# lyndonchan/wsss-analysis

Hardware: AMD Instinct MI355X
Metric: images/sec CAM+CRF pseudo-labels, VOC2012 321x321 (higher is better)
Workload: dtype f16x3; 1 GPU; resnet50 CAM + dense-CRF (M=21, 10 mean-field iters), 321x321, batch 32 images (=64 samples) per GPU, image-sharded; batch_images=32, num_classes=20, parallelism=image-sharded x1, no collective, steps_per_rank=243

## Files before the change

### include/wsscam.h

```cpp
#ifndef WSSCAM_H
#define WSSCAM_H

#include <stddef.h>
#include <stdint.h>

#ifdef __cplusplus
extern "C" {
#endif

#define WSC_VERSION 100

typedef enum wsc_status {
    WSC_OK = 0,
    WSC_ERR_INVALID = -1,
    WSC_ERR_NO_DEVICE = -2,
    WSC_ERR_HIP = -3,
    WSC_ERR_MISSING_KEY = -4,
    WSC_ERR_SHAPE = -5,
    WSC_ERR_NOMEM = -6,
    WSC_ERR_KEY_RANGE = -7,
    WSC_ERR_CAPACITY = -8,
    WSC_ERR_RANGE = -9
} wsc_status;

typedef enum wsc_arch {
    WSC_ARCH_RESNET50_CAM = 0,
    WSC_ARCH_VGG16_CAM = 1,
    WSC_ARCH_M7_CAM = 2,
    WSC_ARCH_RESNET50_IRN = 3,
    WSC_ARCH_VGG16_IRN = 4,
    WSC_ARCH_M7_IRN = 5
} wsc_arch;

typedef enum wsc_precision {
    WSC_PREC_BF16 = 0,
    WSC_PREC_BF16X3 = 1,
    WSC_PREC_F16 = 2,
    WSC_PREC_F16X3 = 3,
    WSC_PREC_F32 = 4
} wsc_precision;

typedef struct wsc_ctx wsc_ctx;
typedef struct wsc_net wsc_net;
typedef enum {
    WSC_OPT_CRF_GAUSS_ON_CHIP = 0,
    WSC_OPT_CRF_FUSED_BLUR = 1,
    WSC_OPT_CRF_BLUR_ON_CHIP = 2,
    WSC_OPT_CRF_RANK_BALLOT = 3,
    WSC_OPT_CRF_EMBED_FULL = 4,
    WSC_OPT_RW_TILED = 5,
    WSC_OPT_STEM_POOL_FUSED = 6,
    WSC_OPT_CONV_WINDOW = 7,
    WSC_OPT_CAM_HEAD_STREAM = 8,
    WSC_OPT_CRF_MSG_IN_UPDATE = 9,
    WSC_OPT_COUNT = 10
} wsc_option;

typedef struct wsc_crf wsc_crf;
typedef struct wsc_crf_v wsc_crf_v;

typedef struct wsc_tensor_desc {
    const char *name;
    const float *data;
    int32_t ndim;
    int64_t shape[4];
} wsc_tensor_desc;


int wsc_version(void);
const char *wsc_last_error(void);

int wsc_ctx_create(int device, void *stream, wsc_ctx **out);
void wsc_ctx_destroy(wsc_ctx *ctx);
int wsc_ctx_set_option(wsc_ctx *ctx, int option, int value);
int wsc_sync(wsc_ctx *ctx);
int wsc_ctx_range_status(wsc_ctx *ctx, int *flag_out, int clear);
int wsc_ctx_wait(wsc_ctx *ctx, wsc_ctx *other);
int wsc_ctx_mark(wsc_ctx *ctx, int slot);
int wsc_ctx_wait_mark(wsc_ctx *ctx, int slot);
int wsc_ctx_wait_for_mark(wsc_ctx *ctx, wsc_ctx *other, int slot);
int wsc_device_info(wsc_ctx *ctx, char *arch_name, size_t arch_name_len, int *num_cus);

int wsc_malloc(wsc_ctx *ctx, size_t bytes, void **dptr_out);
int wsc_free(wsc_ctx *ctx, void *dptr);
int wsc_memcpy_h2d(wsc_ctx *ctx, void *dst_dev, const void *src_host, size_t bytes);
int wsc_memcpy_d2h(wsc_ctx *ctx, void *dst_host, const void *src_dev, size_t bytes);
int wsc_memset(wsc_ctx *ctx, void *dst_dev, int value, size_t bytes);
int wsc_host_alloc(wsc_ctx *ctx, size_t bytes, void **host_out);
int wsc_host_free(wsc_ctx *ctx, void *host);
int wsc_host_write_segments(const char *path, int n, const void *const *ptrs, const size_t *sizes);
int wsc_memcpy_h2d_async(wsc_ctx *ctx, void *dst_dev, const void *src_pinned_host, size_t bytes);
int wsc_memcpy_d2h_async(wsc_ctx *ctx, void *dst_pinned_host, const void *src_dev, size_t bytes);

int wsc_timer_begin(wsc_ctx *ctx);
int wsc_timer_end(wsc_ctx *ctx, float *ms_out);

int wsc_profile_begin(wsc_ctx *ctx);
int wsc_profile_end(wsc_ctx *ctx, int max_classes, int32_t *calls_out, float *total_ms_out, double *work_out,
                    int *n_classes_out);
const char *wsc_profile_class_name(int cls);


int wsc_net_create(wsc_ctx *ctx, int arch, const wsc_tensor_desc *weights, int n_weights,
                   int num_classes, int precision, wsc_net **out);
void wsc_net_destroy(wsc_net *net);
int wsc_net_cam_size(const wsc_net *net, int S, int *h_out);
int wsc_net_feat_channels(const wsc_net *net, int *f_out);

int wsc_net_forward_cam(wsc_ctx *ctx, const wsc_net *net, const float *x_dev, int B, int S,
                        float *cam_dev, float *score_dev);
int wsc_net_cam_size_hw(const wsc_net *net, int H, int W, int *h_out, int *w_out);
int wsc_net_forward_cam_hw(wsc_ctx *ctx, const wsc_net *net, const float *x_dev, int B, int H, int W, float *cam_dev,
                           float *score_dev);

int wsc_net_forward_features(wsc_ctx *ctx, const wsc_net *net, const float *x_dev ,
                             int N, int S, float *feat_dev);

int wsc_net_forward_edge(wsc_ctx *ctx, const wsc_net *net, const float *x_dev, int B, int S, int feat_h, int feat_w,
                         float *edge_dev, float *dp_dev);

int wsc_rw_propagate(wsc_ctx *ctx, const float *x_dev, const float *edge_dev, int K, int h, int w,
                     const int32_t *dirs_host, const int32_t *path_start_host, const int32_t *path_yx_host, int D,
                     float beta, int n_steps, float *rw_dev);
int wsc_rw_propagate_batch(wsc_ctx *ctx, int n_img, const int32_t *K_host, const int32_t *h_host,
                           const int32_t *w_host, const float *x_dev, const float *edge_dev,
                           const int32_t *dirs_host, const int32_t *path_start_host, const int32_t *path_yx_host,
                           int D, float beta, int n_steps, float *rw_dev);

int wsc_net_forward_gradcam(wsc_ctx *ctx, const wsc_net *net, const float *x_dev, int N, int S, int relu,
                            float *cams_dev, float *score_dev);

#define WSC_CONV_GENERIC 0x100
int wsc_conv2d_nchw(wsc_ctx *ctx, const float *x_dev, int N, int Cin, int H, int W, const float *w_host,
                    int Cout, int kh, int kw, int stride, int pad, const float *scale_host,
                    const float *shift_host, const float *residual_dev, int relu, int precision,
                    float *y_dev);


int wsc_cam_postprocess(wsc_ctx *ctx, const float *cam_dev, int B, int C, int h, int w,
                        const int32_t *size_hw_host , const int32_t *keys_host,
                        const int32_t *key_off_host , const int64_t *strided_off_host ,
                        const int64_t *highres_off_host , float *strided_dev, float *highres_dev);

int wsc_cam_eval_confusion(wsc_ctx *ctx, const float *highres_dev, int B, const int32_t *size_hw_host,
                           const int32_t *keys_host, const int32_t *key_off_host,
                           const int64_t *highres_off_host, float bg_thres, const uint8_t *gt_dev, int n_class,
                           int ignore_label, uint8_t *pred_dev, int64_t *confusion_dev);

int wsc_unary_from_maps(wsc_ctx *ctx, const float *maps_dev, int B, int C, int N, float bg_value,
                        float *unary_dev);

int wsc_cam_eval_confusion_nn(wsc_ctx *ctx, const float *maps_dev, int B, const int32_t *src_hw_host ,
                              const int32_t *out_hw_host , const int32_t *keys_host, const int32_t *key_off_host ,
                              const int64_t *maps_off_host , const uint8_t *gt_dev, int n_class, int ignore_label,
                              uint8_t *pred_dev, int64_t *confusion_dev);

int wsc_label_confusion_nn(wsc_ctx *ctx, const int32_t *labels_dev, int B, const int32_t *src_hw_host ,
                           const int32_t *out_hw_host , const int64_t *labels_off_host , const uint8_t *gt_dev,
                           int n_class, int ignore_label, uint8_t *pred_dev, int64_t *confusion_dev);

int wsc_sem_seg_finish(wsc_ctx *ctx, const float *rw_dev, int B, const int64_t *rw_off_host , const int32_t *khw_host ,
                       const int32_t *up_hw_host , const int32_t *out_hw_host , const int32_t *keys_host,
                       const int32_t *key_off_host , int has_bg, float bg_thres, uint8_t *label_dev);

int wsc_cam_unary(wsc_ctx *ctx, const float *cam_dev, int B, int C, int h, int w, int H0, int W0, float bg_value,
                  float *unary_dev);
int wsc_cam_unary_pm(wsc_ctx *ctx, const float *cam_dev, int B, int C, int h, int w, int H0, int W0, float bg_value,
                     float *unary_pm_dev);

int wsc_cam_sum_scales(wsc_ctx *ctx, const float *cam_dev, int n_images, int n_scales, long long map_elems, float *out_dev);

int wsc_msf_input_u8(wsc_ctx *ctx, const uint8_t *images_dev, int B, const int32_t *size_hw_host,
                     const int64_t *offset_host, int S, const float *mean3_host, const float *std3_host,
                     int pre_div255, int pair, float *x_dev);

int wsc_resize_u8(wsc_ctx *ctx, const uint8_t *images_dev, int B, const int32_t *size_hw_host, const int64_t *offset_host,
                  int OH, int OW, uint8_t *out_dev);

int wsc_bilinear_resize(wsc_ctx *ctx, const float *src_dev, int C, int h, int w, float *dst_dev, int H,
                        int W);


int wsc_label_unary_from_cam(wsc_ctx *ctx, const float *highres_dev, int B, int K, int N, float thres, float gt_prob,
                             float *unary_dev, int32_t *labels_dev);
int wsc_ir_label_combine(wsc_ctx *ctx, const int32_t *fg_pred_dev, const int32_t *bg_pred_dev, const int32_t *keys_host,
                         int B, int M, int N, uint8_t *conf_dev);


int wsc_hsn_gradcam_post(wsc_ctx *ctx, const float *cams_nhwc_dev, int B, int h, int w, int C, int S,
                         const float *gate_dev, float *out_dev, int out_channels, int out_first);
int wsc_hsn_voc_background(wsc_ctx *ctx, const float *Hbg_dev, int B, int Cb, int N, float *y_dev, int Ctot);
int wsc_hsn_class_mass(wsc_ctx *ctx, const float *maps_dev, int n_maps, int N, uint32_t *mass_dev);
int wsc_hsn_background(wsc_ctx *ctx, const uint8_t *rgb_dev, int B, int H, int W, int Ho, int Wo, double *bg_dev);
int wsc_cam_adp_modify(wsc_ctx *ctx, const float *cam_dev, int B, int n_sc, int C, int hw, const double *bg_dev, int mode,
                       const int32_t *use_host, int n_use, const int32_t *adipose_host, int n_adip, const int32_t *exc_host,
                       int n_exc, float *out_dev);
int wsc_hsn_cs_gradcam(wsc_ctx *ctx, const float *H_dev, int B, int C_all, int N, const double *bg_dev,
                       const int32_t *src_of_valid_host, int Cv, int bg_ind, int other_ind,
                       const int32_t *exception_inds_host, int n_exc, const int32_t *adipose_src_host, int n_adip,
                       float *cs_dev, float *y_dev, uint32_t *mass_dev);
int wsc_hsn_gather_unary(wsc_ctx *ctx, const float *maps_dev, const int64_t *chan_off_host, int n_chan, int N,
                         float *unary_dev);


int wsc_crf_create(wsc_ctx *ctx, const uint8_t *rgb_dev, int B, int H, int W, float g_sxy,
                   float bi_sxy, float bi_srgb, wsc_crf **out);
void wsc_crf_destroy(wsc_crf *crf);
int wsc_crf_lattice_sizes(wsc_ctx *ctx, const wsc_crf *crf, int32_t *v_gauss_host,
                          int32_t *v_bilat_host);
int wsc_crf_gaussian_on_chip(const wsc_crf *crf, int M);

int wsc_crf_inference(wsc_ctx *ctx, wsc_crf *crf, const float *unary_dev, int M, float g_compat,
                      float bi_compat, int n_iters, float *q_dev, int32_t *argmax_dev);
int wsc_crf_inference_pm(wsc_ctx *ctx, wsc_crf *crf, const float *unary_pm_dev, int M, float g_compat,
                         float bi_compat, int n_iters, float *q_dev, int32_t *argmax_dev);

int wsc_crf_v_create(wsc_ctx *ctx, const uint8_t *const *rgb_dev, const int32_t *hw_host , int B, float g_sxy,
                     float bi_sxy, float bi_srgb, wsc_crf_v **out);
void wsc_crf_v_destroy(wsc_crf_v *crf);
int wsc_crf_v_num_groups(const wsc_crf_v *crf);
int wsc_crf_v_inference(wsc_ctx *ctx, wsc_crf_v *crf, const float *const *unary_dev, const int32_t *M_host, float g_compat,
                        float bi_compat, int n_iters, float *const *q_dev, int32_t *const *argmax_dev);

#ifdef __cplusplus
}
#endif
#endif
```

### wsss-analysis_amd/csrc/common.h

```cpp
#pragma once
#include <hip/hip_runtime.h>
#include <stdint.h>
#include <map>
#include <string>
#include <unordered_map>
#include <vector>

#include "../../include/wsscam.h"

typedef uint16_t bf16_t;

typedef __bf16 bf16x8_t __attribute__((ext_vector_type(8)));
typedef _Float16 f16x8_t __attribute__((ext_vector_type(8)));
typedef float f32x16_t __attribute__((ext_vector_type(16)));
typedef float f32x4_t __attribute__((ext_vector_type(4)));

__host__ __device__ inline bf16_t f32_to_bf16(float f) {
    union { float f; uint32_t u; } v;
    v.f = f;
    uint32_t u = v.u;
    if ((u & 0x7fffffffu) > 0x7f800000u) return (bf16_t)((u >> 16) | 0x40);
    u += 0x7fffu + ((u >> 16) & 1u);
    return (bf16_t)(u >> 16);
}
__host__ __device__ inline float bf16_to_f32(bf16_t h) {
    union { float f; uint32_t u; } v;
    v.u = ((uint32_t)h) << 16;
    return v.f;
}

__host__ __device__ inline uint16_t f32_to_f16(float f) {
#if defined(__HIP_DEVICE_COMPILE__)
    const _Float16 h = (_Float16)fminf(fmaxf(f, -65504.f), 65504.f);
    return __builtin_bit_cast(uint16_t, h);
#else
    union { float f; uint32_t u; } v, magic;
    v.f = f;
    const uint32_t sign = v.u & 0x80000000u;
    v.u ^= sign;
    uint16_t o;
    if (v.u >= ((127u + 16u) << 23)) {
        o = v.u > (255u << 23) ? 0x7e00 : 0x7bff;
    } else if (v.u < (113u << 23)) {
        magic.u = ((127u - 15u) + (23u - 10u) + 1u) << 23;
        v.f += magic.f;
        o = (uint16_t)(v.u - magic.u);
    } else {
        const uint32_t mant_odd = (v.u >> 13) & 1u;
        v.u += ((15u - 127u) << 23) + 0xfffu;
        v.u += mant_odd;
        o = (uint16_t)(v.u >> 13);
        if (o >= 0x7c00) o = 0x7bff;
    }
    return (uint16_t)(o | (sign >> 16));
#endif
}
__host__ __device__ inline float f16_to_f32(uint16_t h) {
#if defined(__HIP_DEVICE_COMPILE__)
    return (float)__builtin_bit_cast(_Float16, h);
#else
    union { float f; uint32_t u; } o, magic;
    magic.u = 113u << 23;
    const uint32_t shifted_exp = 0x7c00u << 13;
    o.u = ((uint32_t)h & 0x7fffu) << 13;
    const uint32_t exp = shifted_exp & o.u;
    o.u += (127u - 15u) << 23;
    if (exp == shifted_exp) o.u += (128u - 16u) << 23;
    else if (exp == 0) { o.u += 1u << 23; o.f -= magic.f; }
    o.u |= ((uint32_t)h & 0x8000u) << 16;
    return o.f;
#endif
}
__host__ __device__ inline uint16_t f32_to_h16(float f, int fmt) { return fmt ? f32_to_f16(f) : f32_to_bf16(f); }
__host__ __device__ inline float h16_to_f32(uint16_t h, int fmt) { return fmt ? f16_to_f32(h) : bf16_to_f32(h); }

void wsc_set_error(const char *fmt, ...);
#define WSC_HIP(expr)                                                                          \
    do {                                                                                       \
        hipError_t _e = (expr);                                                                \
        if (_e != hipSuccess) {                                                                \
            wsc_set_error("%s:%d: %s failed: %s", __FILE__, __LINE__, #expr,                   \
                          hipGetErrorString(_e));                                              \
            return WSC_ERR_HIP;                                                                \
        }                                                                                      \
    } while (0)
#define WSC_CHECK(cond, code, ...)                                                             \
    do {                                                                                       \
        if (!(cond)) {                                                                         \
            wsc_set_error(__VA_ARGS__);                                                        \
            return (code);                                                                     \
        }                                                                                      \
    } while (0)
#define WSC_TRY(expr)                                                                          \
    do {                                                                                       \
        int _s = (expr);                                                                       \
        if (_s != WSC_OK) return _s;                                                           \
    } while (0)

enum WscKernelClass {
    WSC_K_CONV256 = 0,
    WSC_K_CONV128,
    WSC_K_CONV64,
    WSC_K_CONV_SMALLCIN,
    WSC_K_POOL_MISC,
    WSC_K_CAM_TAIL,
    WSC_K_CRF_BUILD,
    WSC_K_GAUSS_MSG,
    WSC_K_BLUR,
    WSC_K_SLICE_UPDATE,
    WSC_K_CRF_MISC,
    WSC_K_COUNT
};
struct WscProfRecord {
    int cls;
    double work;
    hipEvent_t e0, e1;
};

struct WscGaussCache;
void wsc_gauss_cache_destroy(WscGaussCache *cache);
struct wsc_ctx {
    int device = 0;
    hipStream_t stream = nullptr;
    bool own_stream = false;
    int num_cus = 0;
    std::string arch;
    void *ws = nullptr;
    size_t ws_bytes = 0;
    static constexpr int PIN_SLOTS = 8;
    struct PinSlot {
        void *p = nullptr;
        size_t bytes = 0;
        hipEvent_t ev = nullptr;
        bool busy = false;
    };
    PinSlot pin_ring[PIN_SLOTS];
    int pin_next = 0;
    int opt[WSC_OPT_COUNT] = {1, 1, 1, 0, 0, -1, 1, 1, 1, 1};
    void *zero_page = nullptr;
    unsigned *range_host = nullptr, *range_dev = nullptr;
    hipEvent_t ev0 = nullptr, ev1 = nullptr;
    hipEvent_t join_ev = nullptr;
    hipEvent_t marks[8] = {};
    bool mark_set[8] = {};
    hipStream_t aux_stream = nullptr;
    hipEvent_t fork_ev = nullptr, aux_done_ev = nullptr;
    bool profiling = false;
    std::vector<WscProfRecord> prof;
    std::vector<hipEvent_t> prof_pool;
    std::multimap<size_t, void *> free_blocks;
    std::unordered_map<void *, size_t> live_blocks;
    WscGaussCache *gauss_cache = nullptr;
};
int wsc_ctx_workspace(wsc_ctx *ctx, size_t bytes, void **out);
int wsc_ctx_range_check(wsc_ctx *ctx);
__device__ __forceinline__ unsigned half2_at_ceiling(unsigned hw) { return (hw & 0x7fff7fffu) + 0x04010401u; }
struct WscKernelTimer {
    wsc_ctx *ctx;
    int idx = -1;
    WscKernelTimer(wsc_ctx *c, int cls, double work);
    ~WscKernelTimer();
};
int wsc_ctx_cached_alloc(wsc_ctx *ctx, size_t bytes, void **out);
void wsc_ctx_cached_free(wsc_ctx *ctx, void *p);
struct WscCachedGuard {
    wsc_ctx *ctx;
    void *p;
    WscCachedGuard(wsc_ctx *c, void *q) : ctx(c), p(q) {}
    WscCachedGuard(const WscCachedGuard &) = delete;
    WscCachedGuard &operator=(const WscCachedGuard &) = delete;
    void free_now() {
        if (p) wsc_ctx_cached_free(ctx, p);
        p = nullptr;
    }
    ~WscCachedGuard() { free_now(); }
};
int wsc_ctx_upload_small(wsc_ctx *ctx, void *dst_dev, const void *src_host, size_t bytes);
int wsc_set_max_dynamic_lds(wsc_ctx *ctx, const void *fn, int bytes);

constexpr int CONV_FMT_F32 = 2;
inline int conv_fmt(wsc_precision prec) {
    if (prec == WSC_PREC_F32) return CONV_FMT_F32;
    return (prec == WSC_PREC_F16 || prec == WSC_PREC_F16X3) ? 1 : 0;
}
inline size_t conv_elem_bytes(wsc_precision prec) { return prec == WSC_PREC_F32 ? sizeof(float) : sizeof(bf16_t); }
inline int conv_split(wsc_precision prec) { return prec == WSC_PREC_BF16X3 ? 1 : (prec == WSC_PREC_F16X3 ? 2 : 0); }

enum ConvForm {
    CONV_FORM_GENERIC = 0,
    CONV_FORM_SMALL2,
    CONV_FORM_SMALL4,
    CONV_FORM_STEM_ROWS
};
inline bool conv_form_dma(ConvForm f) { return f == CONV_FORM_GENERIC || f == CONV_FORM_STEM_ROWS; }

struct ConvKLayout {
    ConvForm form;
    int kh, kw;
    int kw_steps;
    int kstep;
    int ck;
    bool interleaved;
    int cchunks;
    int ksteps_base;
    int Kbase;
    int Kw;
    int nk;
    int lo_at;
    int index(int ci, int r, int s) const {
        if (form == CONV_FORM_STEM_ROWS) return r * 64 + s * 4 + ci;
        if (form == CONV_FORM_GENERIC) return (((ci / ck) * kh + r) * kw + s) * kstep + ci % ck;
        return r * (form == CONV_FORM_SMALL2 ? 4 : 8) * 4 + s * 4 + ci;
    }
};
inline ConvKLayout conv_k_layout(int kh, int kw, int Cin, ConvForm form, wsc_precision prec) {
    ConvKLayout L;
    const int split = conv_split(prec);
    L.form = form; L.kh = kh; L.kw = kw;
    L.interleaved = split == 2 && conv_form_dma(form);
    L.kstep = prec == WSC_PREC_F32 ? 32 : 64;
    L.ck = (L.interleaved || prec == WSC_PREC_F32) ? 32 : 64;
    L.kw_steps = form == CONV_FORM_STEM_ROWS ? 1 : kw;
    L.cchunks = form == CONV_FORM_GENERIC ? Cin / L.ck : 1;
    if (form == CONV_FORM_GENERIC) L.ksteps_base = kh * kw * L.cchunks;
    else if (form == CONV_FORM_STEM_ROWS) L.ksteps_base = kh;
    else L.ksteps_base = (kh * (form == CONV_FORM_SMALL2 ? 4 : 8) * 4 + L.kstep - 1) / L.kstep;
    L.Kbase = L.ksteps_base * L.kstep;
    const bool segments = split != 0 && !L.interleaved;
    L.Kw = L.Kbase * (segments ? 2 : 1);
    L.nk = L.ksteps_base * (segments ? 3 : 1);
    L.lo_at = L.interleaved ? 32 : L.Kbase;
    return L;
}
inline int conv_cout_pad(int Cout) { return Cout <= 64 ? 64 : ((Cout + 127) / 128) * 128; }
inline int conv_tile_bn(int CoutPad) { return CoutPad % 128 == 0 ? 128 : 64; }
inline void conv_stem_rows_input_dims(int Ho, int Wo, int stride, int kh, int *Hp, int *Wp) {
    *Hp = (Ho - 1) * stride + kh;
    *Wp = (Wo - 1) * stride + 8;
}

struct ConvLaunch {
    const bf16_t *x, *x_lo;
    const bf16_t *w;
    const float *s1, *b1;
    const float *s2, *b2;
    const bf16_t *res, *res_lo;
    bf16_t *y, *y_lo;
    float *y_f32;
    int N, H, W, Cin, Ho, Wo, Cout, CoutPad;
    int kh, kw, stride, pad;
    int relu;
    ConvForm form;
    wsc_precision prec;
    int generic;
    int ldy;
    const bf16_t *x2, *x2_lo;
    int H2, W2, C2, stride2;
};
int conv_igemm_launch(wsc_ctx *ctx, const ConvLaunch &p);
int conv_f32_launch(wsc_ctx *ctx, const ConvLaunch &p);
int launch_cam_head(wsc_ctx *ctx, const bf16_t *x, const bf16_t *x_lo, int M, int K, const bf16_t *w, int Kw, int CoutPad,
                    const float *s1, const float *b1, int C, int relu, float *y);

int launch_nchw_to_nhwc4(wsc_ctx *ctx, const float *x, int N, int H, int W, bf16_t *y, bf16_t *y_lo, int fmt);
void stem_pool_input_dims(int H, int W, int *Hp, int *Wp);
int launch_stem_pool(wsc_ctx *ctx, const bf16_t *x, const bf16_t *x_lo, int N, int H, int W, const bf16_t *w, int Kw, const float *s1,
                     const float *b1, int relu, bf16_t *y, bf16_t *y_lo);
int launch_gather_strided(wsc_ctx *ctx, const bf16_t *x, const bf16_t *x_lo, int N, int H, int W, int C, int stride, int Ho, int Wo,
                          bf16_t *y, bf16_t *y_lo, int ldy);
int launch_nchw_to_nhwc4_pad(wsc_ctx *ctx, const float *x, int N, int H, int W, int Hp, int Wp, int pad, bf16_t *y, bf16_t *y_lo,
                             int fmt);
int launch_maxpool(wsc_ctx *ctx, const bf16_t *x, const bf16_t *x_lo, int N, int H, int W, int C, int k,
                   int stride, int pad, int Ho, int Wo, bf16_t *y, bf16_t *y_lo, int fmt);
int launch_flip_add(wsc_ctx *ctx, const float *head, int B, int h, int w, int C, int Cs, float *cam);
int launch_gap_linear_sigmoid(wsc_ctx *ctx, const bf16_t *feat, const bf16_t *feat_lo, int B, int hw, int F,
                              const float *Wc, const float *bias, int C, float *score, int fmt,
                              int sample_stride);
int launch_bf16_to_f32(wsc_ctx *ctx, const bf16_t *x, const bf16_t *x_lo, size_t n, float *y, int fmt);
int launch_nchw_to_nhwc(wsc_ctx *ctx, const float *x, int N, int C, int HW, bf16_t *y, bf16_t *y_lo, int fmt);
int launch_nhwc_to_nchw(wsc_ctx *ctx, const bf16_t *x, const bf16_t *x_lo, int N, int C, int HW, float *y, int fmt);

int launch_group_norm_stats(wsc_ctx *ctx, const float *x, int N, int H, int W, int C, int G, float eps, void *partial,
                            void *stats);
size_t group_norm_partial_bytes(int N, int H, int W, int G);
int launch_group_norm_apply(wsc_ctx *ctx, const float *x, const void *stats, const float *gamma, const float *beta,
                            int N, int H, int W, int C, int G, int up, int relu, bf16_t *y, bf16_t *y_lo, int Hd, int Wd,
                            int Ctot, int coff, int fmt);
int launch_edge_finish(wsc_ctx *ctx, const float *e, int He, int We, const float *d, int Hd, int Wd, int B, int fh, int fw,
                       float ms0, float ms1, float *edge, float *dp);
```

### wsss-analysis_amd/csrc/crf.hip

```cpp
#include "common.h"

#include <atomic>
#include <cmath>
#include <cstring>
#include <memory>

namespace {

constexpr unsigned long long EMPTY_KEY = 0xFFFFFFFFFFFFFFFFull;
typedef float f32x2_t __attribute__((ext_vector_type(2)));

struct LatticeDev {
    int d = 0;
    int rep = 1;
    int rows = 0;
    int32_t *offset = nullptr;
    float *bary = nullptr;
    float *norm = nullptr;
    int2 *nbr = nullptr;
    int32_t *tslot_start = nullptr;
    int2 *slot_desc = nullptr;
    float *tent_w = nullptr;
    uint8_t *tent_p = nullptr;
    int32_t *row_slot_start = nullptr;
    int n_tiles = 0, n_slots = 0;
    bool sorted_dest = false;
    long long n_pix = 0;
    int M_cur = 0;
    float alpha = 0.f;
    int32_t *tile_rows = nullptr;
    int2 *tile_pstart = nullptr;
    int32_t *tile_list = nullptr;
    int n_tiles_occ = 0;
    int4 *gt_cnt = nullptr;
    int2 *gt_rows = nullptr;
    uint4 *gt_nbr = nullptr;
    uint4 *gt_pix = nullptr;
    int gt_stride = 0;
    std::vector<int32_t> v_per_image;
    int32_t *img_row = nullptr;
    int max_img_rows = 0;
    uint32_t *part_row = nullptr;
    bool bl_ok = false;
    int2 *bl_blk = nullptr;
    int bl_cap = 0;
    mutable std::vector<int2> bl_blk_host;
    mutable int bl_M = -1, bl_nblk = 0;
    mutable size_t bl_lds = 0;
};

constexpr int TILE_W = 16, TILE_H = 16, TILE_PIX = TILE_W * TILE_H;
static_assert(TILE_PIX <= 256, "an entry's pixel index is stored in one byte");
constexpr int SLOT_ENT = 32;
constexpr int SORT_MAX = 2048;
static_assert(TILE_PIX * 6 <= SORT_MAX && SORT_MAX <= 65535, "tile too large for the in-LDS grouping");

struct TileGeom {
    int H, W, ntx, nty, tpi;
};
__host__ __device__ inline TileGeom make_geom(int H, int W) {
    TileGeom g;
    g.H = H; g.W = W;
    g.ntx = (W + TILE_W - 1) / TILE_W;
    g.nty = (H + TILE_H - 1) / TILE_H;
    g.tpi = g.ntx * g.nty;
    return g;
}
struct TileBox {
    int x0, y0, cw, ch;
    int ebase;
};
__host__ __device__ inline TileBox tile_box(const TileGeom &g, int j) {
    const unsigned ty = (unsigned)j / (unsigned)g.ntx, tx = (unsigned)j - ty * (unsigned)g.ntx;
    TileBox b;
    b.x0 = (int)(tx * (unsigned)g.W / (unsigned)g.ntx);
    b.y0 = (int)(ty * (unsigned)g.H / (unsigned)g.nty);
    b.cw = (int)((tx + 1) * (unsigned)g.W / (unsigned)g.ntx) - b.x0;
    b.ch = (int)((ty + 1) * (unsigned)g.H / (unsigned)g.nty) - b.y0;
    b.ebase = b.y0 * g.W + b.x0 * b.ch;
    return b;
}
static_assert(TILE_W <= 26 && TILE_PIX <= 4096, "tile_div_magic range");
__host__ __device__ inline unsigned tile_div_magic(int cw) { return (65536u + (unsigned)cw - 1u) / (unsigned)cw; }

struct CtxBlocks {
    wsc_ctx *ctx;
    std::vector<void *> ptrs;
    explicit CtxBlocks(wsc_ctx *c) : ctx(c) {}
    CtxBlocks(CtxBlocks &&o) noexcept : ctx(o.ctx), ptrs(std::move(o.ptrs)) { o.ptrs.clear(); }
    ~CtxBlocks() { release(); }
    template <class T>
    int alloc(size_t bytes, T **out) {
        void *p = nullptr;
        WSC_TRY(wsc_ctx_cached_alloc(ctx, bytes, &p));
        ptrs.push_back(p);
        *out = static_cast<T *>(p);
        return WSC_OK;
    }
    void take(CtxBlocks &&o) {
        ptrs.insert(ptrs.end(), o.ptrs.begin(), o.ptrs.end());
        o.ptrs.clear();
    }
    void release() {
        for (void *p : ptrs) wsc_ctx_cached_free(ctx, p);
        ptrs.clear();
    }
};

struct GaussEntry {
    int H, W;
    float sxy;
    LatticeDev L;
    CtxBlocks blocks;
    int users = 0;
    unsigned long long last_use = 0;
    bool fuse_pending = true;
};
constexpr int GAUSS_CACHE_MAX = 64;
std::atomic<unsigned long long> g_gauss_use_clock{0};

}

struct wsc_crf {
    wsc_ctx *ctx = nullptr;
    int B = 0, H = 0, W = 0, N = 0;
    LatticeDev lat[2];
    uint4 *pix_rec = nullptr;
    uint32_t *pix_rec_b = nullptr;
    CtxBlocks blocks;
    GaussEntry *gauss = nullptr;
    hipEvent_t use_ev = nullptr;
    bool used_elsewhere = false;
    explicit wsc_crf(wsc_ctx *c) : ctx(c), blocks(c) {}
};

struct WscGaussCache {
    std::vector<std::unique_ptr<GaussEntry>> entries;
};
void wsc_gauss_cache_destroy(WscGaussCache *cache) { delete cache; }

namespace {

__device__ __forceinline__ unsigned long long mix64(unsigned long long x) {
    x ^= x >> 30; x *= 0xbf58476d1ce4e5b9ull;
    x ^= x >> 27; x *= 0x94d049bb133111ebull;
    x ^= x >> 31;
    return x;
}

template <int D>
__device__ __forceinline__ bool pack_key(const int *key, unsigned long long &out) {
    if (D == 2) {
        out = ((unsigned long long)(unsigned)(key[0] + 0x40000000) << 32) | (unsigned)(key[1] + 0x40000000);
        return true;
    }
    unsigned long long k = 0;
    bool ok = true;
#pragma unroll
    for (int i = 0; i < D; ++i) {
        const int v = key[i] + 2048;
        ok = ok && v >= 0 && v < 4096;
        k = (k << 12) | (unsigned long long)(v & 4095);
    }
    out = k;
    return ok;
}
template <int D>
__device__ __forceinline__ void unpack_key(unsigned long long k, int *key) {
    if (D == 2) {
        key[0] = (int)(unsigned)(k >> 32) - 0x40000000;
        key[1] = (int)(unsigned)(k & 0xffffffffu) - 0x40000000;
        return;
    }
#pragma unroll
    for (int i = D - 1; i >= 0; --i) {
        key[i] = (int)(k & 4095) - 2048;
        k >>= 12;
    }
}

constexpr int HASH_MAX_PROBE = 256;
__device__ __forceinline__ int hash_insert(unsigned long long *table, unsigned mask, unsigned long long key) {
    unsigned slot = (unsigned)mix64(key) & mask;
    for (int probe = 0; probe < HASH_MAX_PROBE; ++probe) {
        const unsigned long long prev = atomicCAS(&table[slot], EMPTY_KEY, key);
        if (prev == EMPTY_KEY || prev == key) return (int)slot;
        slot = (slot + 1) & mask;
    }
    return -1;
}
__device__ __forceinline__ int hash_lookup(const unsigned long long *table, unsigned mask, unsigned long long key) {
    unsigned slot = (unsigned)mix64(key) & mask;
    for (;;) {
        const unsigned long long cur = table[slot];
        if (cur == key) return (int)slot;
        if (cur == EMPTY_KEY) return -1;
        slot = (slot + 1) & mask;
    }
}

__device__ __forceinline__ void xcd_range(long long total, long long &begin, long long &end) {
    const int nb = gridDim.x, bid = blockIdx.x;
    const int xcd = bid & 7, q = nb >> 3, r = nb & 7;
    const long long lb = (xcd < r ? (long long)xcd * (q + 1) : (long long)r * (q + 1) + (long long)(xcd - r) * q) + (bid >> 3);
    const long long per = (total + nb - 1) / nb;
    begin = lb * per;
    end = begin + per < total ? begin + per : total;
}

__device__ __forceinline__ int xcd_block_id() {
    const int nb = gridDim.x, bid = blockIdx.x;
    const int xcd = bid & 7, q = nb >> 3, r = nb & 7;
    return (xcd < r ? xcd * (q + 1) : r * (q + 1) + (xcd - r) * q) + (bid >> 3);
}

__device__ __forceinline__ void xcd_range_rep(long long n_local, int rep, int &k, long long &begin, long long &end) {
    const int nb = gridDim.x, bid = blockIdx.x;
    const int xcd = bid & 7, q = nb >> 3, r = nb & 7;
    const int lb = (xcd < r ? xcd * (q + 1) : r * (q + 1) + (xcd - r) * q) + (bid >> 3);
    const int bpr = nb / rep;
    k = lb / bpr;
    const int j = lb - k * bpr;
    const long long per = (n_local + bpr - 1) / bpr;
    begin = (long long)j * per;
    end = begin + per < n_local ? begin + per : n_local;
}

struct EmbedArgs {
    const uint8_t *rgb;
    int B, H, W, N;
    float inv_sxy_den, inv_srgb_den;
    float scale[5];
    unsigned long long *table;
    unsigned cap_mask;
    long long cap;
    float *bary;
    int32_t *first;
    int *err;
};

template <int D>
__device__ __forceinline__ bool embed_pixel(const EmbedArgs &a, long long gp, int x, int y, unsigned long long *pk_out,
                                            float *bary_out) {

    float f[D];
    f[0] = (float)x / a.inv_sxy_den;
    f[1] = (float)y / a.inv_sxy_den;
    if (D == 5) {
        const uint8_t *px = a.rgb + gp * 3;
        f[2] = (float)(int)px[0] / a.inv_srgb_den;
        f[3] = (float)(int)px[1] / a.inv_srgb_den;
        f[4] = (float)(int)px[2] / a.inv_srgb_den;
    }
    float elevated[D + 1], rem0[D + 1];
    int rank[D + 1];
    float sm = 0.f;
#pragma unroll
    for (int j = D; j > 0; --j) {
        const float cf = f[j - 1] * a.scale[j - 1];
        elevated[j] = sm - (float)j * cf;
        sm += cf;
    }
    elevated[0] = sm;

    const float down_factor = 1.0f / (float)(D + 1);
    const float up_factor = (float)(D + 1);
    int sum = 0;
#pragma unroll
    for (int i = 0; i <= D; ++i) {
        const float v = down_factor * elevated[i];
        const float up = ceilf(v) * up_factor;
        const float down = floorf(v) * up_factor;
        int rd2;
        if (up - elevated[i] < elevated[i] - down) rd2 = (int)(short)up;
        else rd2 = (int)(short)down;
        rem0[i] = (float)rd2;
        sum = (int)((float)sum + (float)rd2 * down_factor);
    }
#pragma unroll
    for (int i = 0; i <= D; ++i) rank[i] = 0;
#pragma unroll
    for (int i = 0; i < D; ++i) {
        const float di = elevated[i] - rem0[i];
#pragma unroll
        for (int j = i + 1; j <= D; ++j) {
            if (di < elevated[j] - rem0[j]) rank[i]++;
            else rank[j]++;
        }
    }
#pragma unroll
    for (int i = 0; i <= D; ++i) {
        rank[i] += sum;
        if (rank[i] < 0) {
            rank[i] += D + 1;
            rem0[i] += (float)(D + 1);
        } else if (rank[i] > D) {
            rank[i] -= D + 1;
            rem0[i] -= (float)(D + 1);
        }
    }
    float bary[D + 2];
#pragma unroll
    for (int i = 0; i <= D + 1; ++i) bary[i] = 0.f;
#pragma unroll
    for (int i = 0; i <= D; ++i) {
        const float v = (elevated[i] - rem0[i]) * down_factor;
#pragma unroll
        for (int s = 0; s <= D + 1; ++s) {
            if (s == D - rank[i]) bary[s] += v;
            if (s == D - rank[i] + 1) bary[s] -= v;
        }
    }
    bary[0] = (float)((double)bary[0] + (1.0 + (double)bary[D + 1]));

    bool ok = true;
#pragma unroll
    for (int r = 0; r <= D; ++r) {
        int key[D];
#pragma unroll
        for (int i = 0; i < D; ++i) {
            const int can = rank[i] <= D - r ? r : r - (D + 1);
            key[i] = (int)(short)(rem0[i] + (float)can);
        }
        ok = pack_key<D>(key, pk_out[r]) && ok;
        bary_out[r] = bary[r];
    }
    return ok;
}

__global__ void first_bits_kernel(const int32_t *__restrict__ first, long long cap, int per_img, unsigned *__restrict__ bitmap) {
    const int b = blockIdx.y;
    const int32_t *fi = first + (long long)b * cap;
    for (long long sl = (long long)blockIdx.x * blockDim.x + threadIdx.x; sl < cap; sl += (long long)gridDim.x * blockDim.x) {
        const int f = fi[sl];
        if (f != 0x7fffffff) {
            const long long g = (long long)b * per_img + f;
            atomicOr(&bitmap[g >> 5], 1u << (unsigned)(g & 31));
        }
    }
}
__global__ void popc_words_kernel(const unsigned *__restrict__ bitmap, long long nw, unsigned *__restrict__ cnt) {
    for (long long w = (long long)blockIdx.x * blockDim.x + threadIdx.x; w < nw; w += (long long)gridDim.x * blockDim.x)
        cnt[w] = (unsigned)__popc(bitmap[w]);
}
__device__ __forceinline__ unsigned first_rank(const unsigned *bitmap, const unsigned *wprefix, long long g) {
    return wprefix[g >> 5] + (unsigned)__popc(bitmap[g >> 5] & ((1u << (unsigned)(g & 31)) - 1u));
}
__global__ void image_bounds_kernel(const unsigned *__restrict__ bitmap, const unsigned *__restrict__ wprefix, int per_img, int B,
                                    unsigned *__restrict__ bound) {
    const int b = blockIdx.x * blockDim.x + threadIdx.x;
    if (b < B) bound[b] = first_rank(bitmap, wprefix, (long long)b * per_img);
}
__global__ void image_rows_kernel(const unsigned *__restrict__ bound, int B, int rows, int32_t *__restrict__ img_row) {
    const int b = blockIdx.x * blockDim.x + threadIdx.x;
    if (b < B) img_row[b] = 1 + (int)bound[b];
    if (b == B) img_row[b] = rows;
}
__global__ void assign_rows_kernel(const int32_t *__restrict__ first, const unsigned long long *__restrict__ table, long long cap,
                                   int per_img, const unsigned *__restrict__ bitmap, const unsigned *__restrict__ wprefix,
                                   int32_t *__restrict__ slot2row, unsigned long long *__restrict__ rowkey,
                                   int32_t *__restrict__ rowimg) {
    const int b = blockIdx.y;
    for (long long sl = (long long)blockIdx.x * blockDim.x + threadIdx.x; sl < cap; sl += (long long)gridDim.x * blockDim.x) {
        const long long s_ = (long long)b * cap + sl;
        const int f = first[s_];
        if (f == 0x7fffffff) continue;
        const int row = 1 + (int)first_rank(bitmap, wprefix, (long long)b * per_img + f);
        slot2row[s_] = row;
        rowkey[row] = table[s_];
        rowimg[row] = b;
    }
}

constexpr int SCAN_CHUNK = 4096;

__device__ __forceinline__ unsigned block_exclusive_scan_256(unsigned v, unsigned *lds, unsigned &total) {
    const int lane = threadIdx.x & 63, wv = threadIdx.x >> 6;
    unsigned x = v;
    for (int o = 1; o < 64; o <<= 1) {
        const unsigned y = __shfl_up(x, o, 64);
        if (lane >= o) x += y;
    }
    if (lane == 63) lds[wv] = x;
    __syncthreads();
    unsigned base = 0;
    for (int i = 0; i < wv; ++i) base += lds[i];
    total = lds[0] + lds[1] + lds[2] + lds[3];
    __syncthreads();
    return base + x - v;
}

__global__ __launch_bounds__(256) void scan_reduce_kernel(const unsigned *__restrict__ in, long long n,
                                                          unsigned *__restrict__ sums) {
    __shared__ unsigned lds[4];
    const long long base = (long long)blockIdx.x * SCAN_CHUNK;
    unsigned s = 0;
    for (int i = 0; i < 16; ++i) {
        const long long idx = base + i * 256 + threadIdx.x;
        if (idx < n) s += in[idx];
    }
    for (int o = 32; o > 0; o >>= 1) s += __shfl_down(s, o, 64);
    if ((threadIdx.x & 63) == 0) lds[threadIdx.x >> 6] = s;
    __syncthreads();
    if (threadIdx.x == 0) sums[blockIdx.x] = lds[0] + lds[1] + lds[2] + lds[3];
}

__global__ __launch_bounds__(256) void scan_sums_kernel(unsigned *__restrict__ sums, int m) {
    __shared__ unsigned lds[4];
    unsigned carry = 0;
    for (int base = 0; base < m; base += 256) {
        const int idx = base + threadIdx.x;
        const unsigned v = idx < m ? sums[idx] : 0u;
        unsigned total;
        const unsigned ex = block_exclusive_scan_256(v, lds, total);
        if (idx < m) sums[idx] = carry + ex;
        carry += total;
    }
    if (threadIdx.x == 0) sums[m] = carry;
}

__global__ __launch_bounds__(256) void scan_apply_kernel(const unsigned *__restrict__ in, long long n,
                                                         const unsigned *__restrict__ sums, unsigned *__restrict__ out) {
    __shared__ unsigned lds[4];
    const long long base = (long long)blockIdx.x * SCAN_CHUNK;
    unsigned carry = sums[blockIdx.x];
    unsigned v[16];
    unsigned s = 0;
    const long long t0 = base + (long long)threadIdx.x * 16;
#pragma unroll
    for (int i = 0; i < 16; ++i) {
        v[i] = (t0 + i < n) ? in[t0 + i] : 0u;
        s += v[i];
    }
    unsigned total;
    unsigned ex = carry + block_exclusive_scan_256(s, lds, total);
#pragma unroll
    for (int i = 0; i < 16; ++i) {
        if (t0 + i < n) out[t0 + i] = ex;
        ex += v[i];
    }
}

__global__ __launch_bounds__(256) void scan_apply_fused_kernel(const unsigned *__restrict__ in, long long n,
                                                               unsigned *__restrict__ sums, int nblk, unsigned *__restrict__ out) {
    __shared__ unsigned lds[4];
    __shared__ unsigned red[8];
    const long long base = (long long)blockIdx.x * SCAN_CHUNK;
    const unsigned mine = (int)threadIdx.x < nblk ? sums[threadIdx.x] : 0u;
    unsigned c = (int)threadIdx.x < (int)blockIdx.x ? mine : 0u, tot = mine;
    for (int o = 32; o > 0; o >>= 1) {
        c += __shfl_down(c, o, 64);
        tot += __shfl_down(tot, o, 64);
    }
    if ((threadIdx.x & 63) == 0) {
        red[threadIdx.x >> 6] = c;
        red[4 + (threadIdx.x >> 6)] = tot;
    }
    __syncthreads();
    const unsigned carry = red[0] + red[1] + red[2] + red[3];
    if (blockIdx.x == 0 && threadIdx.x == 0) sums[nblk] = red[4] + red[5] + red[6] + red[7];
    unsigned v[16];
    unsigned s = 0;
    const long long t0 = base + (long long)threadIdx.x * 16;
#pragma unroll
    for (int i = 0; i < 16; ++i) {
        v[i] = (t0 + i < n) ? in[t0 + i] : 0u;
        s += v[i];
    }
    unsigned total;
    unsigned ex = carry + block_exclusive_scan_256(s, lds, total);
#pragma unroll
    for (int i = 0; i < 16; ++i) {
        if (t0 + i < n) out[t0 + i] = ex;
        ex += v[i];
    }
}

int exclusive_scan(wsc_ctx *ctx, const unsigned *in, long long n, unsigned *out, unsigned *sums ) {
    const int nblk = (int)((n + SCAN_CHUNK - 1) / SCAN_CHUNK);
    hipLaunchKernelGGL(scan_reduce_kernel, dim3(nblk), dim3(256), 0, ctx->stream, in, n, sums);
    if (nblk <= 256) {
        hipLaunchKernelGGL(scan_apply_fused_kernel, dim3(nblk), dim3(256), 0, ctx->stream, in, n, sums, nblk, out);
        WSC_HIP(hipGetLastError());
        return WSC_OK;
    }
    hipLaunchKernelGGL(scan_sums_kernel, dim3(1), dim3(256), 0, ctx->stream, sums, nblk);
    hipLaunchKernelGGL(scan_apply_kernel, dim3(nblk), dim3(256), 0, ctx->stream, in, n, sums, out);
    WSC_HIP(hipGetLastError());
    return WSC_OK;
}

template <bool MAXOP, class T = int>
__device__ __forceinline__ void block_scan_lds(T *v, int n, int *wtot ) {
    constexpr int PER = SORT_MAX / 256;
    const int t0 = threadIdx.x * PER;
    int loc[PER];
    int run = 0;
#pragma unroll
    for (int i = 0; i < PER; ++i) {
        const int x = t0 + i < n ? (int)v[t0 + i] : 0;
        run = MAXOP ? max(run, x) : run + x;
        loc[i] = run;
    }
    const int lane = threadIdx.x & 63, wv = threadIdx.x >> 6;
    int x = run;
    for (int o = 1; o < 64; o <<= 1) {
        const int y = __shfl_up(x, o, 64);
        if (lane >= o) x = MAXOP ? max(x, y) : x + y;
    }
    if (lane == 63) wtot[wv] = x;
    __syncthreads();
    int base = 0;
    for (int i = 0; i < wv; ++i) base = MAXOP ? max(base, wtot[i]) : base + wtot[i];
    int prev = __shfl_up(x, 1, 64);
    if (lane == 0) prev = 0;
    const int carry = MAXOP ? max(base, prev) : base + prev;
#pragma unroll
    for (int i = 0; i < PER; ++i)
        if (t0 + i < n) v[t0 + i] = (T)(MAXOP ? max(carry, loc[i]) : carry + loc[i]);
    __syncthreads();
}

__device__ __forceinline__ void tile_slot_flags(const int *srow, int ne, unsigned short *aux, unsigned short *flag, unsigned short *seg,
                                                int *wtot) {
    for (int i = threadIdx.x; i < ne; i += 256) seg[i] = (unsigned short)((i == 0 || srow[i] != srow[i - 1]) ? i : 0);
    __syncthreads();
    block_scan_lds<true>(seg, ne, wtot);
    for (int i = threadIdx.x; i < ne; i += 256) {
        flag[i] = ((i - (int)seg[i]) % SLOT_ENT == 0) ? 1 : 0;
        aux[i] = flag[i];
    }
    __syncthreads();
    block_scan_lds<false>(aux, ne, wtot);
}

constexpr int GROUP_HT_SMALL = 512, GROUP_HT_FULL = SORT_MAX;
constexpr int RANK_MW = (TILE_PIX + 31) / 32;
template <int D, int GROUP_HT>
__device__ __forceinline__ void tile_embed_body(const EmbedArgs &a, const TileGeom &tg, float *__restrict__ tent_w,
                                                uint8_t *__restrict__ tent_p, int32_t *__restrict__ sslot_out,
                                                unsigned *__restrict__ tile_nslots, int force_ballot, int tile,
                                                int32_t *__restrict__ redo_list, unsigned *__restrict__ redo_count) {
    constexpr int RANK_GMAX = (4 * GROUP_HT * 2 + SORT_MAX * 2) / (RANK_MW * 4);
    constexpr bool SMALL = GROUP_HT < GROUP_HT_FULL;
    constexpr int dp1 = D + 1;
    __shared__ unsigned long long table[GROUP_HT];
    __shared__ int start[GROUP_HT];
    __shared__ __attribute__((aligned(16))) unsigned short rank_store[4 * GROUP_HT + SORT_MAX];
    unsigned short(*wcnt)[GROUP_HT] = reinterpret_cast<unsigned short(*)[GROUP_HT]>(rank_store);
    unsigned short *erank = rank_store + 4 * GROUP_HT;
    unsigned *gmask = reinterpret_cast<unsigned *>(rank_store);
    __shared__ unsigned short eslot[SORT_MAX];
    __shared__ unsigned short cid[GROUP_HT];
    __shared__ int wtot[4];
    __shared__ int n_groups_s;
    __shared__ int full_s;
    const int b = tile / tg.tpi, j = tile - b * tg.tpi;
    const TileBox tb = tile_box(tg, j);
    const int N = tg.H * tg.W;
    const int np = tb.cw * tb.ch, ne = np * dp1;
    for (int i = threadIdx.x; i < GROUP_HT; i += 256) {
        table[i] = EMPTY_KEY;
        start[i] = 0x7fffffff;
    }
    for (int i = threadIdx.x; i < (4 * GROUP_HT + SORT_MAX) / 2; i += 256) gmask[i] = 0u;
    if (threadIdx.x == 0) full_s = 0;
    __syncthreads();
    const int t = threadIdx.x;
    const bool have = t < np;
    const int ty = have ? t / tb.cw : 0, tx = have ? t - ty * tb.cw : 0;
    const int y = tb.y0 + ty, x = tb.x0 + tx;
    const int n = y * tg.W + x;
    const long long gp = (long long)b * N + n;
    unsigned long long pk[dp1];
    float bary[dp1];
    if (have) {
        if (!embed_pixel<D>(a, gp, x, y, pk, bary)) atomicOr(a.err, 1);
#pragma unroll
        for (int r = 0; r < dp1; ++r) {
            unsigned sl = (unsigned)(mix64(pk[r]) >> 40) & (GROUP_HT - 1);
            for (int probes = 0;; ++probes) {
                const unsigned long long old = atomicCAS(&table[sl], EMPTY_KEY, pk[r]);
                if (old == EMPTY_KEY || old == pk[r]) break;
                if (SMALL && probes >= GROUP_HT) {
                    full_s = 1;
                    break;
                }
                sl = (sl + 1) & (GROUP_HT - 1);
            }
            eslot[t * dp1 + r] = (unsigned short)sl;
            atomicMin(&start[sl], n * dp1 + r);
        }
    }
    __syncthreads();
    const int lane = threadIdx.x & 63, q = threadIdx.x >> 6;
    {
        constexpr int PER = GROUP_HT / 256;
        int cnt = 0;
#pragma unroll
        for (int k = 0; k < PER; ++k) cnt += table[threadIdx.x * PER + k] != EMPTY_KEY ? 1 : 0;
        int x = cnt;
        for (int o = 1; o < 64; o <<= 1) {
            const int y = __shfl_up(x, o, 64);
            if (lane >= o) x += y;
        }
        if (lane == 63) wtot[q] = x;
        __syncthreads();
        int base = x - cnt;
        for (int i = 0; i < q; ++i) base += wtot[i];
#pragma unroll
        for (int k = 0; k < PER; ++k) {
            const int sl = threadIdx.x * PER + k;
            const bool occ = table[sl] != EMPTY_KEY;
            cid[sl] = (unsigned short)base;
            base += occ ? 1 : 0;
        }
        if (threadIdx.x == 255) n_groups_s = base;
        __syncthreads();
    }
    if (SMALL && (full_s || n_groups_s > GROUP_HT * 3 / 4)) {
        if (threadIdx.x == 0) redo_list[atomicAdd(redo_count, 1u)] = tile;
        return;
    }
    const bool use_mask = !force_ballot && n_groups_s <= RANK_GMAX;
    const int Q = ((ne + 3) / 4 + 63) / 64 * 64;
    if (use_mask) {
        if (have) {
#pragma unroll
            for (int r = 0; r < dp1; ++r)
                atomicOr(&gmask[(unsigned)cid[eslot[t * dp1 + r]] * RANK_MW + (t >> 5)], 1u << (t & 31));
        }
    } else {
        for (int c = q * Q; c < min(ne, (q + 1) * Q); c += 64) {
            const int e = c + lane;
            const bool valid = e < ne;
            const unsigned sl = valid ? eslot[e] : 0u;
            unsigned long long remaining = __ballot(valid);
            unsigned long long mine = 0;
            while (remaining) {
                const int leader = __ffsll((long long)remaining) - 1;
                const bool same = valid && sl == (unsigned)__shfl((int)sl, leader, 64);
                const unsigned long long m = __ballot(same);
                if (same) mine = m;
                remaining &= ~m;
            }
            if (valid) {
                const int leader = __ffsll((long long)mine) - 1;
                int base = 0;
                if (lane == leader) {
                    base = wcnt[q][sl];
                    wcnt[q][sl] = (unsigned short)(base + __popcll(mine));
                }
                base = __shfl(base, leader, 64);
                erank[e] = (unsigned short)(base + __popcll(mine & ((1ull << lane) - 1ull)));
            }
        }
    }
    __syncthreads();
    unsigned long long *gtable = a.table + (long long)b * a.cap;
    int32_t *gfirst = a.first + (long long)b * a.cap;
    int my_slots = 0;
    for (int i = threadIdx.x; i < GROUP_HT; i += 256) {
        int tot = 0, c0 = 0, c1 = 0, c2 = 0;
        if (use_mask) {
            if (table[i] != EMPTY_KEY) {
#pragma unroll
                for (int w = 0; w < RANK_MW; ++w) tot += __popc(gmask[(unsigned)cid[i] * RANK_MW + w]);
            }
        } else {
            c0 = wcnt[0][i]; c1 = wcnt[1][i]; c2 = wcnt[2][i];
            tot = c0 + c1 + c2 + wcnt[3][i];
        }
        if (tot > 0) {
            int gs = hash_insert(gtable, a.cap_mask, table[i]);
            if (gs >= 0) atomicMin(&gfirst[gs], start[i]);
            else {
                atomicOr(a.err, 2);
                gs = 0;
            }
            table[i] = (unsigned long long)(unsigned)gs;
        }
        start[i] = tot;
        if (!use_mask) {
            wcnt[0][i] = 0;
            wcnt[1][i] = (unsigned short)c0;
            wcnt[2][i] = (unsigned short)(c0 + c1);
            wcnt[3][i] = (unsigned short)(c0 + c1 + c2);
        }
        my_slots += (tot + SLOT_ENT - 1) / SLOT_ENT;
    }
    for (int o = 32; o > 0; o >>= 1) my_slots += __shfl_down(my_slots, o, 64);
    __syncthreads();
    if (lane == 0) wtot[q] = my_slots;
    __syncthreads();
    if (threadIdx.x == 0) tile_nslots[tile] = (unsigned)(wtot[0] + wtot[1] + wtot[2] + wtot[3]);
    __syncthreads();
    block_scan_lds<false>(start, GROUP_HT, wtot);
    if (have) {
        const long long ebase = ((long long)b * N + tb.ebase) * dp1;
#pragma unroll
        for (int r = 0; r < dp1; ++r) {
            const int e = t * dp1 + r;
            const int sl = eslot[e];
            const int prev = sl > 0 ? start[sl - 1] : 0;
            int rank;
            if (use_mask) {
                const unsigned *m = gmask + (unsigned)cid[sl] * RANK_MW;
                rank = __popc(m[t >> 5] & ((1u << (t & 31)) - 1u));
                for (int w = 0; w < (t >> 5); ++w) rank += __popc(m[w]);
            } else {
                rank = (int)wcnt[e / Q][sl] + (int)erank[e];
            }
            const int pos = prev + rank;
            const int gs = (int)(unsigned)table[sl];
            tent_w[ebase + pos] = bary[r];
            tent_p[ebase + pos] = (uint8_t)t;
            sslot_out[ebase + pos] = gs | (r << 28);
            a.bary[gp * dp1 + r] = bary[r];
        }
    }
}
template <int D>
__global__ __launch_bounds__(256) void tile_embed_kernel(EmbedArgs a, TileGeom tg, float *__restrict__ tent_w, uint8_t *__restrict__ tent_p,
                                                         int32_t *__restrict__ sslot_out, unsigned *__restrict__ tile_nslots,
                                                         int force_ballot, int32_t *__restrict__ redo_list,
                                                         unsigned *__restrict__ redo_count) {
    tile_embed_body<D, GROUP_HT_SMALL>(a, tg, tent_w, tent_p, sslot_out, tile_nslots, force_ballot, (int)blockIdx.x, redo_list,
                                       redo_count);
}
template <int D>
__global__ __launch_bounds__(256) void tile_embed_full_kernel(EmbedArgs a, TileGeom tg, float *__restrict__ tent_w,
                                                              uint8_t *__restrict__ tent_p, int32_t *__restrict__ sslot_out,
                                                              unsigned *__restrict__ tile_nslots, int force_ballot,
                                                              const int32_t *__restrict__ redo_list,
                                                              const unsigned *__restrict__ redo_count, int n_tiles) {
    const int count = redo_list ? (int)*redo_count : n_tiles;
    for (int i = blockIdx.x; i < count; i += gridDim.x) {
        tile_embed_body<D, GROUP_HT_FULL>(a, tg, tent_w, tent_p, sslot_out, tile_nslots, force_ballot,
                                          redo_list ? redo_list[i] : i, nullptr, nullptr);
        __syncthreads();
    }
}

__global__ __launch_bounds__(256) void tile_slots_kernel(const int32_t *__restrict__ sslot_in, const uint8_t *__restrict__ tent_p,
                                                         int32_t *__restrict__ offset, const int32_t *__restrict__ slot2row,
                                                         long long cap, int dp1, TileGeom tg,
                                                         const int32_t *__restrict__ tslot_start, int2 *__restrict__ slot_desc,
                                                         int32_t *__restrict__ slot_row, unsigned *__restrict__ slot_key,
                                                         unsigned *__restrict__ row_nslots) {
    __shared__ int rows_s[SORT_MAX];
    __shared__ unsigned short aux[SORT_MAX];
    __shared__ unsigned short flag[SORT_MAX];
    __shared__ unsigned short seg[SORT_MAX];
    __shared__ unsigned short pos[SORT_MAX + 2];
    __shared__ int wtot[4];
    const int tile = xcd_block_id();
    const int b = tile / tg.tpi, j = tile - b * tg.tpi;
    const TileBox tb = tile_box(tg, j);
    const int N = tg.H * tg.W;
    const int ne = tb.cw * tb.ch * dp1;
    const long long ebase = ((long long)b * N + tb.ebase) * dp1;
    const unsigned cw_magic = tile_div_magic(tb.cw);
    for (int i = threadIdx.x; i < ne; i += 256) {
        const int ss = sslot_in[ebase + i];
        const int row = slot2row[(long long)b * cap + (ss & 0x0fffffff)];
        rows_s[i] = row;
        const unsigned t = tent_p[ebase + i];
        const unsigned ty = (t * cw_magic) >> 16, tx = t - ty * (unsigned)tb.cw;
        const long long p = (long long)b * N + (long long)(tb.y0 + (int)ty) * tg.W + tb.x0 + (int)tx;
        offset[p * dp1 + (ss >> 28)] = row;
    }
    __syncthreads();
    tile_slot_flags(rows_s, ne, aux, flag, seg, wtot);
    const int ns = aux[ne - 1];
    for (int i = threadIdx.x; i < ne; i += 256)
        if (flag[i]) pos[aux[i] - 1] = (unsigned short)i;
    if (threadIdx.x == 0) pos[ns] = (unsigned short)ne;
    __syncthreads();
    __shared__ int hist[SLOT_ENT + 1], hcur[SLOT_ENT + 1];
    if (threadIdx.x <= SLOT_ENT) { hist[threadIdx.x] = 0; hcur[threadIdx.x] = 0; }
    __syncthreads();
    for (int s = threadIdx.x; s < ns; s += 256) atomicAdd(&hist[pos[s + 1] - pos[s]], 1);
    __syncthreads();
    if (threadIdx.x == 0) {
        int run = 0;
        for (int n = SLOT_ENT; n >= 0; --n) {
            const int c = hist[n];
            hist[n] = run;
            run += c;
        }
    }
    __syncthreads();
    const int s0 = tslot_start[tile];
    for (int s = threadIdx.x; s < ns; s += 256) {
        const int i = pos[s], n = pos[s + 1] - i;
        const int row = rows_s[i];
        const int dst = s0 + hist[n] + atomicAdd(&hcur[n], 1);
        slot_desc[dst] = make_int2(i | (n << 16), 0);
        slot_row[dst] = row;
        if (slot_key) slot_key[dst] = (unsigned)tile * 64u + (unsigned)((i - seg[i]) / SLOT_ENT);
        atomicAdd(&row_nslots[row], 1u);
    }
}

__global__ void slot_dest_kernel(const int32_t *__restrict__ slot_row, int n_slots, const int32_t *__restrict__ row_slot_start,
                                 unsigned *__restrict__ cursor, int2 *__restrict__ slot_desc, uint32_t *__restrict__ part_row) {
    for (int s = blockIdx.x * blockDim.x + threadIdx.x; s < n_slots; s += gridDim.x * blockDim.x) {
        const int row = slot_row[s];
        const int sb = row_slot_start[row];
        const int dst = sb + (int)atomicAdd(&cursor[row], 1u);
        slot_desc[s].y = dst;
        if (part_row) part_row[dst] = (uint32_t)row | ((uint32_t)min(row_slot_start[row + 1] - sb, 255) << 24);
    }
}

__global__ void dest_inverse_kernel(const int2 *__restrict__ slot_desc, int n_slots, int32_t *__restrict__ dest_slot) {
    for (int s = blockIdx.x * blockDim.x + threadIdx.x; s < n_slots; s += gridDim.x * blockDim.x) dest_slot[slot_desc[s].y] = s;
}
__global__ void row_sort_dest_kernel(const unsigned *__restrict__ slot_key, int32_t *__restrict__ dest_slot,
                                     const int32_t *__restrict__ row_slot_start, int rows, int2 *__restrict__ slot_desc) {
    for (int row = blockIdx.x * blockDim.x + threadIdx.x; row < rows; row += gridDim.x * blockDim.x) {
        const int sb = row_slot_start[row], se = row_slot_start[row + 1];
        for (int i = sb + 1; i < se; ++i) {
            const int s = dest_slot[i];
            const unsigned key = slot_key[s];
            int j = i - 1;
            while (j >= sb && slot_key[dest_slot[j]] > key) {
                dest_slot[j + 1] = dest_slot[j];
                --j;
            }
            dest_slot[j + 1] = s;
        }
        for (int i = sb; i < se; ++i) slot_desc[dest_slot[i]].y = i;
    }
}

__global__ __launch_bounds__(256) void tile_scale_entries_kernel(const float *__restrict__ norm, int dp1, TileGeom tg,
                                                                 float *__restrict__ tent_w, const uint8_t *__restrict__ tent_p) {
    const int tile = blockIdx.x;
    const int b = tile / tg.tpi, j = tile - b * tg.tpi;
    const TileBox tb = tile_box(tg, j);
    const int N = tg.H * tg.W;
    const int ne = tb.cw * tb.ch * dp1;
    const long long ebase = ((long long)b * N + tb.ebase) * dp1;
    const unsigned cw_magic = tile_div_magic(tb.cw);
    for (int i = threadIdx.x; i < ne; i += 256) {
        const int t = (int)tent_p[ebase + i];
        const int ty = (int)(((unsigned)t * cw_magic) >> 16), tx = t - ty * tb.cw;
        const long long p = (long long)b * N + (long long)(tb.y0 + ty) * tg.W + tb.x0 + tx;
        tent_w[ebase + i] = tent_w[ebase + i] * norm[p];
    }
}

template <int D>
__global__ void neighbors_kernel(const unsigned long long *__restrict__ rowkey, const int32_t *__restrict__ rowimg,
                                 const unsigned long long *__restrict__ table, const int32_t *__restrict__ slot2row,
                                 long long cap, unsigned cap_mask, int rows, int2 *__restrict__ nbr) {
    const int j = blockIdx.y;
    long long rbeg, rend;
    xcd_range(rows, rbeg, rend);
    for (int row = (int)rbeg + (int)threadIdx.x; row < (int)rend; row += (int)blockDim.x) {
        const long long i = (long long)j * rows + row;
        int *nb = reinterpret_cast<int *>(nbr);
        if (row == 0) {
            nb[2 * i] = 0;
            continue;
        }
        int key[D], k1[D];
        unpack_key<D>(rowkey[row], key);
#pragma unroll
        for (int k = 0; k < D; ++k) k1[k] = key[k] - 1;
        if (j < D) {
#pragma unroll
            for (int k = 0; k < D; ++k)
                if (k == j) k1[k] = key[k] + D;
        }
        const int b = rowimg[row];
        const unsigned long long *tb = table + (long long)b * cap;
        const int32_t *s2r = slot2row + (long long)b * cap;
        unsigned long long p1;
        int r1 = 0;
        if (pack_key<D>(k1, p1)) {
            const int s = hash_lookup(tb, cap_mask, p1);
            if (s >= 0) r1 = s2r[s];
        }
        nb[2 * i] = r1;
        if (r1 > 0) nb[2 * ((long long)j * rows + r1) + 1] = row;
    }
}


constexpr float PFIX_SCALE = 16777216.0f;
constexpr float PFIX_INV = 1.0f / 16777216.0f;
static_assert(SLOT_ENT * 2.5f < 127.0f, "slot partials must fit the 2^24 fixed-point int32");

template <bool PLAIN>
__device__ __forceinline__ f32x4_t combine_slots4(const f32x4_t *__restrict__ part, int sb, int se, unsigned LP, unsigned l) {
    f32x4_t first = part[(unsigned)sb * LP + l];
    if (se - sb == 1) return first;
    if (PLAIN) {
        for (int i = sb + 1; i < se; ++i) {
            const f32x4_t v = part[(unsigned)i * LP + l];
#pragma unroll
            for (int k = 0; k < 4; ++k) first[k] += v[k];
        }
        return first;
    }
    long long acc[4] = {0, 0, 0, 0};
    for (int i = sb; i < se; i += 4) {
        f32x4_t v[4];
#pragma unroll
        for (int u = 0; u < 4; ++u) v[u] = part[(unsigned)min(i + u, se - 1) * LP + l];
#pragma unroll
        for (int u = 0; u < 4; ++u)
            if (i + u < se) {
#pragma unroll
                for (int k = 0; k < 4; ++k) acc[k] += (long long)__float2int_rn(v[u][k] * PFIX_SCALE);
            }
    }
    f32x4_t o = {(float)acc[0] * PFIX_INV, (float)acc[1] * PFIX_INV, (float)acc[2] * PFIX_INV, (float)acc[3] * PFIX_INV};
    return o;
}

__global__ __launch_bounds__(256) void slot_ones_kernel(const int32_t *__restrict__ tslot_start, const int2 *__restrict__ slot_desc,
                                                        const float *__restrict__ tent_w, int dp1, TileGeom tg,
                                                        float *__restrict__ part) {
    const int tile = blockIdx.x;
    const int b = tile / tg.tpi, j = tile - b * tg.tpi;
    const TileBox tb = tile_box(tg, j);
    const long long ebase = ((long long)b * tg.H * tg.W + tb.ebase) * dp1;
    __shared__ float w[TILE_PIX * 6];
    const int ne = tb.cw * tb.ch * dp1;
    {
        constexpr int EN = (TILE_PIX * 6 + 255) / 256;
        float ew[EN];
#pragma unroll
        for (int k = 0; k < EN; ++k) {
            const int i = (int)threadIdx.x + k * 256;
            ew[k] = i < ne ? tent_w[ebase + i] : 0.f;
        }
#pragma unroll
        for (int k = 0; k < EN; ++k) {
            const int i = (int)threadIdx.x + k * 256;
            if (i < ne) w[i] = ew[k];
        }
    }
    __syncthreads();
    for (int s = tslot_start[tile] + threadIdx.x; s < tslot_start[tile + 1]; s += 256) {
        const int2 d = slot_desc[s];
        const int i0 = d.x & 0xffff, n = d.x >> 16;
        float acc = 0.f;
        for (int i = 0; i < n; ++i) acc += w[i0 + i];
        part[d.y] = acc;
    }
}
__global__ void combine1_kernel(const float *__restrict__ part, const int32_t *__restrict__ row_slot_start, int rows,
                                float *__restrict__ val) {
    for (int row = blockIdx.x * blockDim.x + threadIdx.x; row < rows; row += gridDim.x * blockDim.x) {
        long long acc = 0;
        for (int i = row_slot_start[row]; i < row_slot_start[row + 1]; ++i)
            acc += (long long)__float2int_rn(part[i] * PFIX_SCALE);
        val[row] = (float)acc * PFIX_INV;
    }
}

__global__ __launch_bounds__(256) void combine4_kernel(const f32x4_t *__restrict__ part, const int32_t *__restrict__ row_slot_start,
                                                       int LP, int rows_local, int n_slots, int rep, f32x4_t *__restrict__ val) {
    const int rpb = 256 / LP;
    const int tr = threadIdx.x / LP;
    const int l = threadIdx.x - tr * LP;
    if (tr >= rpb) return;
    long long rbeg, rend;
    int rk;
    xcd_range_rep(rows_local, rep, rk, rbeg, rend);
    part += (size_t)rk * n_slots * LP;
    val += (size_t)rk * rows_local * LP;
    for (long long row = rbeg + tr; row < rend; row += rpb) {
        const int sb = row_slot_start[row], se = row_slot_start[row + 1];
        f32x4_t o = {0.f, 0.f, 0.f, 0.f};
        if (se > sb) o = combine_slots4<true>(part, sb, se, (unsigned)LP, (unsigned)l);
        val[(unsigned)row * (unsigned)LP + l] = o;
    }
}

constexpr int CB_ROWS = 32;
__global__ __launch_bounds__(256) void combine4_balanced_kernel(const f32x4_t *__restrict__ part, const int32_t *__restrict__ row_slot_start,
                                                                const uint32_t *__restrict__ part_row, int LP, int rows,
                                                                f32x4_t *__restrict__ val) {
    __shared__ int rss_l[CB_ROWS + 1];
    __shared__ unsigned long long acc[CB_ROWS * 32];
    const int r0 = blockIdx.x * CB_ROWS;
    const int nr = min(CB_ROWS, rows - r0);
    const int P0 = row_slot_start[r0], P1 = row_slot_start[r0 + nr];
    for (int i = threadIdx.x; i <= nr; i += 256) rss_l[i] = row_slot_start[r0 + i];
    for (int i = threadIdx.x; i < CB_ROWS * 32; i += 256) acc[i] = 0ull;
    const int gpb = 256 / LP;
    const int tr = threadIdx.x / LP, l = threadIdx.x - tr * LP;
    constexpr int U = 4;
    f32x4_t v[U];
    uint32_t pr[U];
    auto fetch = [&](int p) {
#pragma unroll
        for (int u = 0; u < U; ++u) {
            const int pp = p + u * gpb;
            v[u] = f32x4_t{0.f, 0.f, 0.f, 0.f};
            pr[u] = 0u;
            if (tr < gpb && pp < P1) {
                v[u] = part[(unsigned)pp * (unsigned)LP + l];
                if (part_row) pr[u] = part_row[pp];
            }
        }
    };
    fetch(P0 + tr);
    __syncthreads();
    if (tr < gpb) {
        for (int p = P0 + tr; p < P1; p += U * gpb) {
            if (p != P0 + tr) fetch(p);
#pragma unroll
            for (int u = 0; u < U; ++u) {
                const int pp = p + u * gpb;
                if (pp < P1) {
                    int lo;
                    bool single;
                    if (part_row) {
                        lo = (int)(pr[u] & 0xffffffu) - r0;
                        single = (pr[u] >> 24) == 1u;
                    } else {
                        lo = 0;
                        int hi = nr;
                        while (hi - lo > 1) {
                            const int mid = (lo + hi) >> 1;
                            if (rss_l[mid] <= pp) lo = mid;
                            else hi = mid;
                        }
                        single = rss_l[lo + 1] - rss_l[lo] == 1;
                    }
                    if (single) {
                        val[(unsigned)(r0 + lo) * (unsigned)LP + l] = v[u];
                    } else {
#pragma unroll
                        for (int k = 0; k < 4; ++k)
                            atomicAdd(&acc[lo * 32 + 4 * l + k], (unsigned long long)(long long)__float2int_rn(v[u][k] * PFIX_SCALE));
                    }
                }
            }
        }
    }
    __syncthreads();
    if (tr < gpb) {
        for (int row = tr; row < nr; row += gpb) {
            const int n = rss_l[row + 1] - rss_l[row];
            if (n == 1) continue;
            f32x4_t o = {0.f, 0.f, 0.f, 0.f};
            if (n > 1) {
#pragma unroll
                for (int k = 0; k < 4; ++k) o[k] = (float)(long long)acc[row * 32 + 4 * l + k] * PFIX_INV;
            }
            val[(unsigned)(r0 + row) * (unsigned)LP + l] = o;
        }
    }
}


__global__ __launch_bounds__(256) void blur1_kernel(const float *__restrict__ in, const int2 *__restrict__ nbr,
                                                    int rows, float *__restrict__ out) {
    for (int row = blockIdx.x * blockDim.x + threadIdx.x; row < rows; row += gridDim.x * blockDim.x) {
        const int2 nb = nbr[row];
        out[row] = row == 0 ? 0.f : in[row] + 0.5f * (in[nb.x] + in[nb.y]);
    }
}

__global__ __launch_bounds__(256) void blur4_kernel(const f32x4_t *__restrict__ in, const int2 *__restrict__ nbr,
                                                    int LP, int rows_local, int rep, f32x4_t *__restrict__ out) {
    const int rpb = 256 / LP;
    const int tr = threadIdx.x / LP;
    const int l = threadIdx.x - tr * LP;
    if (tr >= rpb) return;
    constexpr int U = 4;
    long long rbeg, rend;
    int rk;
    xcd_range_rep(rows_local, rep, rk, rbeg, rend);
    in += (size_t)rk * rows_local * LP;
    out += (size_t)rk * rows_local * LP;
    for (long long row0 = rbeg + tr; row0 < rend; row0 += U * rpb) {
        int2 nb[U];
        f32x4_t c[U], a[U], b[U];
#pragma unroll
        for (int u = 0; u < U; ++u) {
            const long long row = row0 + u * rpb;
            nb[u] = row < rend ? nbr[row] : make_int2(0, 0);
        }
#pragma unroll
        for (int u = 0; u < U; ++u) {
            const long long row = row0 + u * rpb;
            c[u] = in[(unsigned)(row < rend ? row : 0) * (unsigned)LP + l];
            a[u] = in[(unsigned)nb[u].x * (unsigned)LP + l];
            b[u] = in[(unsigned)nb[u].y * (unsigned)LP + l];
        }
#pragma unroll
        for (int u = 0; u < U; ++u) {
            const long long row = row0 + u * rpb;
            if (row < rend) {
                f32x4_t o;
#pragma unroll
                for (int k = 0; k < 4; ++k) o[k] = row == 0 ? 0.f : c[u][k] + 0.5f * (a[u][k] + b[u][k]);
                out[(unsigned)row * (unsigned)LP + l] = o;
            }
        }
    }
}

constexpr int BL_THREADS = 1024;
constexpr int BL_NVAR = 5;
constexpr int BL_VAR[BL_NVAR][2] = {{4, 4}, {4, 10}, {3, 13}, {2, 20}, {1, 26}};
inline int blur_lds_variant(int rows) {
    for (int v = 0; v < BL_NVAR; ++v)
        if (rows <= BL_VAR[v][1] * BL_THREADS && (size_t)(rows + 1) * BL_VAR[v][0] * 4 <= 160 * 1024 && rows < 65535) return v;
    return -1;
}
struct BlurLdsArgs {
    const int2 *nbr;
    const int32_t *img_row;
    const int2 *blk;
    float *val;
    int Mp, M, rows, npass;
};
template <int GW> struct FloatRun { float v[GW]; };
typedef float f32x3u_t __attribute__((ext_vector_type(3), aligned(4)));
template <int GW>
__device__ __forceinline__ FloatRun<GW> load_run(const float *q) {
    FloatRun<GW> r;
    if constexpr (GW == 4) {
        const f32x4_t x = *reinterpret_cast<const f32x4_t *>(q);
        r.v[0] = x[0]; r.v[1] = x[1]; r.v[2] = x[2]; r.v[3] = x[3];
    } else if constexpr (GW == 3) {
        const f32x3u_t x = *reinterpret_cast<const f32x3u_t *>(q);
        r.v[0] = x[0]; r.v[1] = x[1]; r.v[2] = x[2];
    } else if constexpr (GW == 2) {
        const f32x2_t x = *reinterpret_cast<const f32x2_t *>(q);
        r.v[0] = x[0]; r.v[1] = x[1];
    } else {
        r.v[0] = q[0];
    }
    return r;
}
template <int GW>
__device__ __forceinline__ void store_run(float *q, const FloatRun<GW> &r) {
    if constexpr (GW == 4) *reinterpret_cast<f32x4_t *>(q) = f32x4_t{r.v[0], r.v[1], r.v[2], r.v[3]};
    else if constexpr (GW == 3) {
        f32x3u_t x;
        x[0] = r.v[0]; x[1] = r.v[1]; x[2] = r.v[2];
        *reinterpret_cast<f32x3u_t *>(q) = x;
    } else if constexpr (GW == 2) *reinterpret_cast<f32x2_t *>(q) = f32x2_t{r.v[0], r.v[1]};
    else q[0] = r.v[0];
}
template <int GW, int RPT>
__device__ __forceinline__ void blur_lds_body(const BlurLdsArgs &p, float *pl, int img, int grp) {
    const int r0 = p.img_row[img], nr = p.img_row[img + 1] - r0;
    const int stride = nr + 1;
    const int c0 = grp * GW;
    const int tid = (int)threadIdx.x;
    float *vb = p.val + (size_t)r0 * p.Mp + c0;
    unsigned nb[RPT];
    auto load_idx = [&](int pass) {
        const int2 *q = p.nbr + (size_t)pass * p.rows + r0;
        constexpr int CH = RPT < 10 ? RPT : 10;
#pragma unroll
        for (int i0 = 0; i0 < RPT; i0 += CH) {
            int2 raw[CH];
#pragma unroll
            for (int i = 0; i < CH; ++i) {
                const int r = tid + (i0 + i) * BL_THREADS;
                raw[i] = (i0 + i < RPT && r < nr) ? q[r] : make_int2(0, 0);
            }
#pragma unroll
            for (int i = 0; i < CH; ++i)
                if (i0 + i < RPT)
                    nb[i0 + i] = (unsigned)(raw[i].x ? raw[i].x - r0 : nr) | ((unsigned)(raw[i].y ? raw[i].y - r0 : nr) << 16);
        }
    };
    load_idx(0);
#pragma unroll
    for (int i = 0; i < RPT; ++i) {
        const int r = tid + i * BL_THREADS;
        if (r < nr) {
            FloatRun<GW> run;
            if (GW == 3 && c0 + GW > p.Mp) {
#pragma unroll
                for (int g = 0; g < GW; ++g) run.v[g] = c0 + g < p.Mp ? vb[(size_t)r * p.Mp + g] : 0.f;
            } else {
                run = load_run<GW>(vb + (size_t)r * p.Mp);
            }
#pragma unroll
            for (int g = 0; g < GW; ++g) pl[g * stride + r] = c0 + g < p.M ? run.v[g] : 0.f;
        }
    }
    if (tid < GW) pl[tid * stride + nr] = 0.f;
    __syncthreads();
    float o[RPT][GW];
    for (int pass = 0; pass < p.npass; ++pass) {
#pragma unroll
        for (int i = 0; i < RPT; ++i) {
            const int r = tid + i * BL_THREADS;
            const int rc = r < nr ? r : nr;
            const int l1 = (int)(nb[i] & 0xffffu), l2 = (int)(nb[i] >> 16);
#pragma unroll
            for (int g = 0; g < GW; ++g) o[i][g] = pl[g * stride + rc] + 0.5f * (pl[g * stride + l1] + pl[g * stride + l2]);
        }
        if (pass + 1 < p.npass) load_idx(pass + 1);
        else break;
        __syncthreads();
#pragma unroll
        for (int i = 0; i < RPT; ++i) {
            const int r = tid + i * BL_THREADS;
            if (r < nr) {
#pragma unroll
                for (int g = 0; g < GW; ++g) pl[g * stride + r] = o[i][g];
            }
        }
        __syncthreads();
    }
#pragma unroll
    for (int i = 0; i < RPT; ++i) {
        const int r = tid + i * BL_THREADS;
        if (r < nr) {
            if (c0 + GW <= p.M) {
                FloatRun<GW> run;
#pragma unroll
                for (int g = 0; g < GW; ++g) run.v[g] = o[i][g];
                store_run<GW>(vb + (size_t)r * p.Mp, run);
            } else {
#pragma unroll
                for (int g = 0; g < GW; ++g)
                    if (c0 + g < p.M) vb[(size_t)r * p.Mp + g] = o[i][g];
            }
        }
    }
}
__global__ __launch_bounds__(BL_THREADS) void blur_lds_kernel(BlurLdsArgs p) {
    extern __shared__ float pl[];
    const int2 w = p.blk[blockIdx.x];
    if (w.x < 0) return;
    const int img = w.x & 0xffffff;
    switch (w.x >> 24) {
    case 0: blur_lds_body<BL_VAR[0][0], BL_VAR[0][1]>(p, pl, img, w.y); break;
    case 1: blur_lds_body<BL_VAR[1][0], BL_VAR[1][1]>(p, pl, img, w.y); break;
    case 2: blur_lds_body<BL_VAR[2][0], BL_VAR[2][1]>(p, pl, img, w.y); break;
    case 3: blur_lds_body<BL_VAR[3][0], BL_VAR[3][1]>(p, pl, img, w.y); break;
    default: blur_lds_body<BL_VAR[4][0], BL_VAR[4][1]>(p, pl, img, w.y); break;
    }
}

constexpr int GTI = 12, GTJ = 12, GBI = GTI + 4, GBJ = GTJ + 4;
constexpr int GLH = 6;

__global__ void gauss_ij_kernel(const unsigned long long *__restrict__ rowkey, int rows, int2 *__restrict__ ij,
                                int *__restrict__ bbox ) {
    for (int row = 1 + blockIdx.x * blockDim.x + threadIdx.x; row < rows; row += gridDim.x * blockDim.x) {
        int key[2];
        unpack_key<2>(rowkey[row], key);
        const int a = 2 * key[0] + key[1], b = key[0] + 2 * key[1];
        if (a % 3 != 0 || b % 3 != 0) atomicOr(&bbox[4], 1);
        const int i = a / 3, j = b / 3;
        ij[row] = make_int2(i, j);
        atomicMin(&bbox[0], i);
        atomicMin(&bbox[1], j);
        atomicMax(&bbox[2], i);
        atomicMax(&bbox[3], j);
    }
}

__global__ void gauss_tile_fill_kernel(const int2 *__restrict__ ij, int rows, int imin, int jmin, int nti, int ntj,
                                       int32_t *__restrict__ tile_rows, int32_t *__restrict__ occ) {
    for (int row = 1 + blockIdx.x * blockDim.x + threadIdx.x; row < rows; row += gridDim.x * blockDim.x) {
        const int i = ij[row].x - imin, j = ij[row].y - jmin;
        occ[(i / GTI) * ntj + j / GTJ] = 1;
        for (int ti = (i - GTI - 1 >= 0 ? (i - GTI - 1) / GTI : 0); ti <= (i + 2) / GTI && ti < nti; ++ti) {
            const int li = i - ti * GTI + 2;
            if (li < 0 || li >= GBI) continue;
            for (int tj = (j - GTJ - 1 >= 0 ? (j - GTJ - 1) / GTJ : 0); tj <= (j + 2) / GTJ && tj < ntj; ++tj) {
                const int lj = j - tj * GTJ + 2;
                if (lj < 0 || lj >= GBJ) continue;
                tile_rows[((long long)ti * ntj + tj) * (GBI * GBJ) + li * GBJ + lj] = row;
            }
        }
    }
}

__global__ void gauss_tile_pstart_kernel(const int32_t *__restrict__ tile_rows, const int32_t *__restrict__ row_slot_start,
                                         long long total, int2 *__restrict__ tile_pstart) {
    for (long long i = (long long)blockIdx.x * blockDim.x + threadIdx.x; i < total; i += (long long)gridDim.x * blockDim.x) {
        const int row = tile_rows[i];
        tile_pstart[i] = row ? make_int2(row_slot_start[row], row_slot_start[row + 1] - row_slot_start[row]) : make_int2(0, 0);
    }
}

__global__ __launch_bounds__(GBI * GBJ) void blur3_tile_kernel(const f32x4_t *__restrict__ in, const int32_t *__restrict__ tile_rows,
                                                         const int32_t *__restrict__ tile_list, int n_occ, int LP,
                                                         int rows_local, int rep, f32x4_t *__restrict__ out,
                                                         const f32x4_t *__restrict__ part, const int2 *__restrict__ tile_pstart,
                                                         int n_slots) {
    constexpr int P = GBI * GBJ;
    constexpr int PS = P + 1;
    __shared__ f32x4_t b0[GLH * PS];
    const int nb = gridDim.x, bid = blockIdx.x;
    const int xcd = bid & 7, qq = nb >> 3, rr = nb & 7;
    const int lb = (xcd < rr ? xcd * (qq + 1) : rr * (qq + 1) + (xcd - rr) * qq) + (bid >> 3);
    const int k = lb / n_occ, t = lb - k * n_occ;
    if (in) in += (size_t)k * rows_local * LP;
    if (part) part += (size_t)k * n_slots * LP;
    out += (size_t)k * rows_local * LP;
    const int p = threadIdx.x;
    const int li = p / GBJ, lj = p - li * GBJ;
    const long long tbase = (long long)tile_list[t] * P;
    const int row = tile_rows[tbase + p];
    const f32x4_t zero = {0.f, 0.f, 0.f, 0.f};
    if (t == 0 && p < LP) out[p] = zero;
    const bool r0 = row && li >= 1 && li < GBI - 1;
    const bool r1 = r0 && lj >= 1 && lj < GBJ - 1;
    const bool r2 = row && li >= 2 && li < GBI - 2 && lj >= 2 && lj < GBJ - 2;
    int prow[GLH], psb[GLH], pse[GLH];
#pragma unroll
    for (int i = 0; i < GLH; ++i) {
        const int pp = (i * P + p) / GLH;
        const int pli = pp / GBJ, plj = pp - pli * GBJ;
        const int r = tile_rows[tbase + pp];
        psb[i] = 0; pse[i] = 0;
        if (part && r) {
            const int2 ps = tile_pstart[tbase + pp];
            psb[i] = ps.x;
            pse[i] = ps.x + ps.y;
        }
        prow[i] = (r && pli >= 2 && pli < GBI - 2 && plj >= 2 && plj < GBJ - 2) ? r : (r ? -r : 0);
    }
    for (int lbase = 0; lbase < LP; lbase += GLH) {
        if (lbase > 0) __syncthreads();
        {
            f32x4_t v[GLH];
#pragma unroll
            for (int i = 0; i < GLH; ++i) {
                const int idx = i * P + p, pp = idx / GLH, ll = idx - pp * GLH;
                const int r = prow[i] < 0 ? -prow[i] : prow[i];
                v[i] = zero;
                if (r && lbase + ll < LP) {
                    if (part) {
                        if (pse[i] > psb[i]) v[i] = part[(unsigned)psb[i] * (unsigned)LP + lbase + ll];
                    } else {
                        v[i] = in[(unsigned)r * (unsigned)LP + lbase + ll];
                    }
                }
            }
#pragma unroll
            for (int i = 0; i < GLH; ++i) {
                const int idx = i * P + p, pp = idx / GLH, ll = idx - pp * GLH;
                if (part && pse[i] - psb[i] > 1 && lbase + ll < LP)
                    v[i] = combine_slots4<true>(part, psb[i], pse[i], (unsigned)LP, (unsigned)(lbase + ll));
                b0[ll * PS + pp] = v[i];
            }
        }
        __syncthreads();
        f32x4_t o[GLH];
#pragma unroll
        for (int l = 0; l < GLH; ++l) {
            o[l] = zero;
            if (r0) {
                const f32x4_t c = b0[l * PS + p], a = b0[l * PS + p + GBJ], b = b0[l * PS + p - GBJ];
#pragma unroll
                for (int q = 0; q < 4; ++q) o[l][q] = c[q] + 0.5f * (a[q] + b[q]);
            }
        }
        __syncthreads();
#pragma unroll
        for (int l = 0; l < GLH; ++l) b0[l * PS + p] = o[l];
        __syncthreads();
#pragma unroll
        for (int l = 0; l < GLH; ++l) {
            o[l] = zero;
            if (r1) {
                const f32x4_t c = b0[l * PS + p], a = b0[l * PS + p - 1], b = b0[l * PS + p + 1];
#pragma unroll
                for (int q = 0; q < 4; ++q) o[l][q] = c[q] + 0.5f * (a[q] + b[q]);
            }
        }
        __syncthreads();
#pragma unroll
        for (int l = 0; l < GLH; ++l) b0[l * PS + p] = o[l];
        __syncthreads();
        if (r2) {
#pragma unroll
            for (int l = 0; l < GLH; ++l) {
                const f32x4_t c = b0[l * PS + p], a = b0[l * PS + p - GBJ - 1], b = b0[l * PS + p + GBJ + 1];
#pragma unroll
                for (int q = 0; q < 4; ++q) o[l][q] = c[q] + 0.5f * (a[q] + b[q]);
            }
        }
        __syncthreads();
        if (r2) {
#pragma unroll
            for (int l = 0; l < GLH; ++l) b0[l * PS + p] = o[l];
        }
        __syncthreads();
#pragma unroll
        for (int i = 0; i < GLH; ++i) {
            const int idx = i * P + p, pp = idx / GLH, ll = idx - pp * GLH;
            if (prow[i] > 0 && lbase + ll < LP) out[(unsigned)prow[i] * (unsigned)LP + lbase + ll] = b0[ll * PS + pp];
        }
    }
}

__global__ __launch_bounds__(256) void slice_norm_kernel(const int32_t *__restrict__ offset, const float *__restrict__ bary,
                                                          int dp1, float alpha, const float *__restrict__ val, long long npix,
                                                          float *__restrict__ norm, uint32_t *__restrict__ rec) {
    __shared__ uint32_t lrec[256 * 13];
    for (long long p0 = (long long)blockIdx.x * 256; p0 < npix; p0 += (long long)gridDim.x * 256) {
        const long long p = p0 + threadIdx.x;
        if (p < npix) {
            float acc = 0.f;
            for (int r = 0; r < dp1; ++r) {
                const int o = offset[p * dp1 + r];
                const float w = bary[p * dp1 + r];
                acc += w * val[o] * alpha;
                if (rec) {
                    lrec[threadIdx.x * 13 + r] = (uint32_t)o;
                    lrec[threadIdx.x * 13 + 6 + r] = __float_as_uint(w);
                }
            }
            const float nv = (float)(1.0 / sqrt((double)acc + 1e-20));
            norm[p] = nv;
            if (rec) lrec[threadIdx.x * 13 + 12] = __float_as_uint(nv);
        }
        if (rec) {
            __syncthreads();
            const int n13 = (int)min(256ll, npix - p0) * 13;
            for (int i = threadIdx.x; i < n13; i += 256) rec[p0 * 13 + i] = lrec[i];
            __syncthreads();
        }
    }
}

__global__ __launch_bounds__(256) void slice_norm_tile_kernel(const int32_t *__restrict__ offset, const float *__restrict__ bary,
                                                               int dp1, float alpha, const float *__restrict__ val, TileGeom tg,
                                                               float *__restrict__ norm, uint32_t *__restrict__ rec,
                                                               float *__restrict__ tent_w, const uint8_t *__restrict__ tent_p) {
    __shared__ uint32_t lrec[256 * 13];
    __shared__ float lnorm[256];
    const int tile = xcd_block_id();
    const int b = tile / tg.tpi, j = tile - b * tg.tpi;
    const TileBox tb = tile_box(tg, j);
    const int N = tg.H * tg.W;
    const int np = tb.cw * tb.ch;
    const unsigned cw_magic = tile_div_magic(tb.cw);
    const int t = threadIdx.x;
    const int ty = (int)(((unsigned)t * cw_magic) >> 16), tx = t - ty * tb.cw;
    const long long p = (long long)b * N + (long long)(tb.y0 + ty) * tg.W + tb.x0 + tx;
    if (t < np) {
        constexpr int DMAX = 6;
        int o[DMAX];
        float w[DMAX], v[DMAX];
#pragma unroll
        for (int r = 0; r < DMAX; ++r) {
            o[r] = r < dp1 ? offset[p * dp1 + r] : 0;
            w[r] = r < dp1 ? bary[p * dp1 + r] : 0.f;
        }
#pragma unroll
        for (int r = 0; r < DMAX; ++r) v[r] = r < dp1 ? val[o[r]] : 0.f;
        float acc = 0.f;
#pragma unroll
        for (int r = 0; r < DMAX; ++r)
            if (r < dp1) {
                acc += w[r] * v[r] * alpha;
                if (rec) {
                    lrec[t * 13 + r] = (uint32_t)o[r];
                    lrec[t * 13 + 6 + r] = __float_as_uint(w[r]);
                }
            }
        const float nv = (float)(1.0 / sqrt((double)acc + 1e-20));
        norm[p] = nv;
        lnorm[t] = nv;
        if (rec) lrec[t * 13 + 12] = __float_as_uint(nv);
    }
    __syncthreads();
    if (rec) {
        const int rowlen = tb.cw * 13;
        for (int i = t; i < np * 13; i += 256) {
            const int ry = i / rowlen, k = i - ry * rowlen;
            rec[((long long)b * N + (long long)(tb.y0 + ry) * tg.W + tb.x0) * 13 + k] = lrec[i];
        }
    }
    const int ne = np * dp1;
    const long long ebase = ((long long)b * N + tb.ebase) * dp1;
    {
        constexpr int EN = (TILE_PIX * 6 + 255) / 256;
        float ew[EN];
        int ep[EN];
#pragma unroll
        for (int k = 0; k < EN; ++k) {
            const int i = t + k * 256;
            ew[k] = i < ne ? tent_w[ebase + i] : 0.f;
            ep[k] = i < ne ? (int)tent_p[ebase + i] : 0;
        }
#pragma unroll
        for (int k = 0; k < EN; ++k) {
            const int i = t + k * 256;
            if (i < ne) tent_w[ebase + i] = ew[k] * lnorm[ep[k]];
        }
    }
}

__global__ void pack_pixels_kernel(const int32_t *__restrict__ off_g, const float *__restrict__ bary_g,
                                   const float *__restrict__ norm_g, const int32_t *__restrict__ off_b,
                                   const float *__restrict__ bary_b, const float *__restrict__ norm_b, int N,
                                   int g_shared, uint4 *__restrict__ rec) {
    const int b = blockIdx.y;
    for (int i = blockIdx.x * blockDim.x + threadIdx.x; i < N * 5; i += gridDim.x * blockDim.x) {
        const int n = i / 5, piece = i - n * 5;
        const long long p = (long long)b * N + n;
        const long long pg = g_shared ? (long long)n : p;
        uint32_t w[4];
#pragma unroll
        for (int c = 0; c < 4; ++c) {
            const int k = piece * 4 + c;
            uint32_t v;
            if (k < 3) v = (uint32_t)off_g[pg * 3 + k];
            else if (k < 9) v = (uint32_t)off_b[p * 6 + (k - 3)];
            else if (k < 12) v = __float_as_uint(bary_g[pg * 3 + (k - 9)]);
            else if (k < 18) v = __float_as_uint(bary_b[p * 6 + (k - 12)]);
            else if (k == 18) v = __float_as_uint(norm_g[pg]);
            else v = __float_as_uint(norm_b[p]);
            w[c] = v;
        }
        rec[p * 5 + piece] = make_uint4(w[0], w[1], w[2], w[3]);
    }
}

__global__ void pack_pixels_b_kernel(const int32_t *__restrict__ off_b, const float *__restrict__ bary_b,
                                     const float *__restrict__ norm_b, long long npix, uint32_t *__restrict__ rec) {
    for (long long i = (long long)blockIdx.x * blockDim.x + threadIdx.x; i < npix * 13; i += (long long)gridDim.x * blockDim.x) {
        const long long p = i / 13;
        const int k = (int)(i - p * 13);
        rec[i] = k < 6 ? (uint32_t)off_b[p * 6 + k] : (k < 12 ? __float_as_uint(bary_b[p * 6 + (k - 6)]) : __float_as_uint(norm_b[p]));
    }
}

constexpr int GM_THREADS = 512;
struct SplatTab {
    const int32_t *tslot_start;
    const int2 *slot_desc;
    const float *tent_w;
    const uint8_t *tent_p;
    float *part;
    int n_slots;
    int shared;
    int dp1;
// ... 444 lines not shown
        }
        sum = __shfl(sum, seg0, 64);
        const float rs = __builtin_amdgcn_rcpf(sum);
        const f32x4_t o4 = {ex[0] * rs, ex[1] * rs, ex[2] * rs, ex[3] * rs};
        if (ok) {
            if (SPLAT) stage[t * LP + l] = o4;
            if (a.q) *reinterpret_cast<f32x4_t *>(q_b + (__umul24(p, LP16) + l16)) = o4;
        }
        if (!SPLAT && a.argmax != nullptr) {
            float bv = o4[0];
            int bi = 4 * l;
#pragma unroll
            for (int kk = 1; kk < 4; ++kk)
                if (4 * l + kk < a.M && o4[kk] > bv) {
                    bv = o4[kk];
                    bi = 4 * l + kk;
                }
            for (int o = 4; o > 0; o >>= 1) {
                const float ov = __shfl_down(bv, o, 64);
                const int oi = __shfl_down(bi, o, 64);
                if (l + o < LP && ov > bv) {
                    bv = ov;
                    bi = oi;
                }
            }
            if (ok && l == 0) a.argmax[pix0 + p] = bi;
        }
    };
    {
        {
            const f32x4_t u0 = load_u(t_first);
            f32x4_t g3[3], b6[6];
            float w9[9];
            if (SLICE) {
                load_rec(t_first, rq);
                issue_rows(rq, g3, b6, w9);
            }
            unn = u0;
            if (t_first + ppt < np) {
                if (SLICE) load_rec(t_first + ppt, rq);
                unn = load_u(t_first + ppt);
            }
            fold(u0, g3, b6, w9, e01, e23);
        }
        for (int t0 = t_first; t0 < np; t0 += ppt) {
            const bool has_next = t0 + ppt < np;
            f32x4_t vgn[3], vbn[6];
            float wrn[9];
            const f32x4_t un1 = unn;
            if (SLICE && has_next) issue_rows(rq, vgn, vbn, wrn);
            if (t0 + 2 * ppt < np) {
                if (SLICE) load_rec(t0 + 2 * ppt, rq);
                unn = load_u(t0 + 2 * ppt);
            }
            emit(t0);
            if (has_next) fold(un1, vgn, vbn, wrn, e01, e23);
        }
    }
    if (SPLAT) {
        uint2 *lent = reinterpret_cast<uint2 *>(stage + TILE_PIX * LP);
        int2 *ldesc = reinterpret_cast<int2 *>(lent + GATHER_ENT);
        if (DMA) __syncthreads();
        splat_commit<EN_G>(a.sg, np, rg, lent, ldesc, LP);
        SplatRegs<EN_B> rb;
        splat_fetch<EN_B>(a.sb, a.sb.shared ? j : lb, (a.sb.shared ? 0ll : (long long)k * N) + tb.ebase, np, rb);
        __syncthreads();
        tile_gather(a.sg, rg.s_beg, rg.s_end, k, stage, lent, ldesc, LP, l, g, gpw, act);
        splat_commit<EN_B>(a.sb, np, rb, lent, ldesc, LP);
        __syncthreads();
        tile_gather(a.sb, rb.s_beg, rb.s_end, k, stage, lent, ldesc, LP, l, g, gpw, act);
    }
}

struct GaussMsgArgs {
    const int4 *gt_cnt;
    const int2 *gt_rows;
    const uint4 *gt_nbr;
    const uint4 *gt_pix;
    const float *part;
    const float *u;
    float *e;
    int gt_stride, n_slots, shared, LP, B;
    float cag;
    TileGeom tg;
};
template <int NIT, int NPI>
__global__ __launch_bounds__(GM_THREADS) __attribute__((amdgpu_waves_per_eu(4))) void gauss_msg_kernel(GaussMsgArgs a) {
    extern __shared__ f32x4_t gl[];
    const int LP = a.LP, stride = a.gt_stride, tid = (int)threadIdx.x;
    const f32x4_t zero = {0.f, 0.f, 0.f, 0.f};
    const int nb = gridDim.x, bid = blockIdx.x;
    const int xcd = bid & 7, qq = nb >> 3, rr = nb & 7;
    const int lb = (xcd < rr ? xcd * (qq + 1) : rr * (qq + 1) + (xcd - rr) * qq) + (bid >> 3);
    const int k = lb / a.tg.tpi, j = lb - k * a.tg.tpi;
    const TileBox tb = tile_box(a.tg, j);
    const int np = tb.cw * tb.ch;
    const int N = a.tg.H * a.tg.W;
    unsigned *lnb = reinterpret_cast<unsigned *>(gl + (size_t)stride * (size_t)LP);
    const f32x4_t *partg = reinterpret_cast<const f32x4_t *>(a.part) + (a.shared ? (size_t)k * a.n_slots * LP : (size_t)0);
    const int nitems = stride * LP;
    const unsigned lp_magic = (65536u + (unsigned)LP - 1u) / (unsigned)LP;
    const unsigned cw_magic = tile_div_magic(tb.cw);
    const int2 *trow = a.gt_rows + (size_t)j * stride;
    const uint4 *tn = a.gt_nbr + (size_t)j * stride;
    const unsigned gpix0 = (unsigned)tb.y0 * (unsigned)a.tg.W + (unsigned)tb.x0;
    const size_t pix0 = (size_t)k * (size_t)N + gpix0;
    const f32x4_t *u4 = reinterpret_cast<const f32x4_t *>(a.u) + pix0 * LP;
    f32x4_t *e4 = reinterpret_cast<f32x4_t *>(a.e) + pix0 * LP;
    const int4 cnt = a.gt_cnt[j];
    int2 ps[NIT];
#pragma unroll
    for (int it = 0; it < NIT; ++it) {
        const int i = tid + it * GM_THREADS;
        ps[it] = make_int2(0, 0);
        if (i < nitems) ps[it] = trow[((unsigned)i * lp_magic) >> 16];
    }
    uint4 gpx[NPI];
    f32x4_t uu[NPI];
    unsigned poff[NPI];
    auto load_pixels = [&]() {
    #pragma unroll
        for (int it = 0; it < NPI; ++it) {
            const int i = tid + it * GM_THREADS;
            gpx[it] = make_uint4(0, 0, 0, 0);
            uu[it] = zero;
            poff[it] = 0;
            if (i < np * LP) {
                const unsigned t = ((unsigned)i * lp_magic) >> 16, ll = (unsigned)i - t * (unsigned)LP;
                const unsigned ty = (t * cw_magic) >> 16, tx = t - ty * (unsigned)tb.cw;
                const unsigned po = ty * (unsigned)a.tg.W + tx;
                poff[it] = po * (unsigned)LP + ll;
                gpx[it] = a.gt_pix[gpix0 + po];
                uu[it] = u4[poff[it]];
            }
        }
    };
#pragma unroll 2
    for (int v = tid; v < stride; v += GM_THREADS) reinterpret_cast<uint4 *>(lnb)[v] = tn[v];
    {
        f32x4_t val[NIT];
#pragma unroll
        for (int it = 0; it < NIT; ++it) {
            const int i = tid + it * GM_THREADS;
            const unsigned v = ((unsigned)i * lp_magic) >> 16, ll = (unsigned)i - v * (unsigned)LP;
            val[it] = zero;
            if (ps[it].y > 0) val[it] = partg[(unsigned)ps[it].x * (unsigned)LP + ll];
        }
        int maxc = 0;
#pragma unroll
        for (int it = 0; it < NIT; ++it) maxc = max(maxc, ps[it].y);
        for (int c = 1; c < maxc; ++c) {
            f32x4_t more[NIT];
#pragma unroll
            for (int it = 0; it < NIT; ++it) {
                const int i = tid + it * GM_THREADS;
                const unsigned v = ((unsigned)i * lp_magic) >> 16, ll = (unsigned)i - v * (unsigned)LP;
                more[it] = zero;
                if (c < ps[it].y) more[it] = partg[(unsigned)(ps[it].x + c) * (unsigned)LP + ll];
            }
#pragma unroll
            for (int it = 0; it < NIT; ++it)
                if (c < ps[it].y) {
#pragma unroll
                    for (int q = 0; q < 4; ++q) val[it][q] += more[it][q];
                }
        }
#pragma unroll
        for (int it = 0; it < NIT; ++it) {
            const int i = tid + it * GM_THREADS;
            if (i < nitems) gl[i] = val[it];
        }
    }
    __syncthreads();
#pragma unroll
    for (int axis = 0; axis < 3; ++axis) {
        const int nitems = (axis == 0 ? cnt.z : (axis == 1 ? cnt.y : cnt.x)) * LP;
        f32x4_t o[NIT];
#pragma unroll
        for (int it = 0; it < NIT; ++it) {
            const int i = tid + it * GM_THREADS;
            o[it] = zero;
            if (i < nitems) {
                const unsigned v = ((unsigned)i * lp_magic) >> 16, ll = (unsigned)i - v * (unsigned)LP;
                const unsigned w = lnb[v * 4 + axis];
                const f32x4_t c = gl[i], x1 = gl[(w & 0xffffu) * (unsigned)LP + ll], x2 = gl[(w >> 16) * (unsigned)LP + ll];
#pragma unroll
                for (int q = 0; q < 4; ++q) o[it][q] = c[q] + 0.5f * (x1[q] + x2[q]);
            }
        }
        __syncthreads();
#pragma unroll
        for (int it = 0; it < NIT; ++it) {
            const int i = tid + it * GM_THREADS;
            if (i < nitems) gl[i] = o[it];
        }
        __syncthreads();
    }
    load_pixels();
#pragma unroll
    for (int it = 0; it < NPI; ++it) {
        const int i = tid + it * GM_THREADS;
        if (i < np * LP) {
            const unsigned t = ((unsigned)i * lp_magic) >> 16, ll = (unsigned)i - t * (unsigned)LP;
            const uint4 gp = gpx[it];
            f32x2_t o01 = {-uu[it][0], -uu[it][1]}, o23 = {-uu[it][2], -uu[it][3]};
            const float wr[3] = {__uint_as_float(gp.y) * a.cag, __uint_as_float(gp.z) * a.cag, __uint_as_float(gp.w) * a.cag};
#pragma unroll
            for (int r = 0; r < 3; ++r) {
                const f32x4_t row = gl[((gp.x >> (10 * r)) & 1023u) * (unsigned)LP + ll];
                const f32x2_t w2 = {wr[r], wr[r]}, lo = {row[0], row[1]}, hi = {row[2], row[3]};
                o01 = __builtin_elementwise_fma(w2, lo, o01);
                o23 = __builtin_elementwise_fma(w2, hi, o23);
            }
            e4[poff[it]] = f32x4_t{o01[0], o01[1], o23[0], o23[1]};
        }
    }
}

constexpr int TP = 128;

__global__ __launch_bounds__(TP) void init_q_kernel(const float *__restrict__ unary, int M, int Mp, int N,
                                                     float *__restrict__ u, float *__restrict__ q) {
    extern __shared__ float tile[];
    float *tu = tile, *tq = tile + (size_t)M * (TP + 1);
    const int b = blockIdx.y;
    const int n0 = blockIdx.x * TP;
    const int np = min(TP, N - n0);
    const float *src = unary + (long long)b * M * N;
    for (int m = 0; m < M; ++m)
        if ((int)threadIdx.x < np) tu[m * (TP + 1) + threadIdx.x] = src[(long long)m * N + n0 + threadIdx.x];
    __syncthreads();
    if ((int)threadIdx.x < np) {
        float mx = -3.0e38f;
        for (int m = 0; m < M; ++m) mx = fmaxf(mx, -tu[m * (TP + 1) + threadIdx.x]);
        float s = 0.f;
        for (int m = 0; m < M; ++m) {
            const float e = expf(-tu[m * (TP + 1) + threadIdx.x] - mx);
            tq[m * (TP + 1) + threadIdx.x] = e;
            s += e;
        }
        for (int m = 0; m < M; ++m) tq[m * (TP + 1) + threadIdx.x] = tq[m * (TP + 1) + threadIdx.x] / s;
    }
    __syncthreads();
    const long long obase = ((long long)b * N + n0) * Mp;
    for (int i = threadIdx.x; i < np * Mp; i += TP) {
        const int n = i / Mp, m = i - n * Mp;
        u[obase + i] = m < M ? tu[m * (TP + 1) + n] : 0.f;
        if (q) q[obase + i] = m < M ? tq[m * (TP + 1) + n] : 0.f;
    }
}

struct UnaryVJob {
    const float *u;
    int M;
};
__global__ __launch_bounds__(256) void gather_unary_v_kernel(const UnaryVJob *__restrict__ jobs, int Mg, int Mp, int N,
                                                             float *__restrict__ out) {
    const UnaryVJob job = jobs[blockIdx.y];
    const int n = blockIdx.x * blockDim.x + threadIdx.x;
    if (n >= N) return;
    float *dst = out + ((long long)blockIdx.y * N + n) * Mp;
    for (int m0 = 0; m0 < Mp; m0 += 4) {
        f32x4_t v;
#pragma unroll
        for (int k = 0; k < 4; ++k) {
            const int m = m0 + k;
            v[k] = m < job.M ? job.u[(long long)m * N + n] : (m < Mg ? 1.0e30f : 0.f);
        }
        *reinterpret_cast<f32x4_t *>(dst + m0) = v;
    }
}

__global__ __launch_bounds__(TP) void finish_kernel(const float *__restrict__ q, int M, int Mp, int N,
                                                    float *__restrict__ q_out, int32_t *__restrict__ argmax) {
    extern __shared__ float tile[];
    const int b = blockIdx.y;
    const int n0 = blockIdx.x * TP;
    const int np = min(TP, N - n0);
    const long long ibase = ((long long)b * N + n0) * Mp;
    for (int i = threadIdx.x; i < np * Mp; i += TP) {
        const int n = i / Mp, m = i - n * Mp;
        if (m < M) tile[m * (TP + 1) + n] = q[ibase + i];
    }
    __syncthreads();
    if ((int)threadIdx.x < np) {
        if (q_out)
            for (int m = 0; m < M; ++m)
                q_out[((long long)b * M + m) * N + n0 + threadIdx.x] = tile[m * (TP + 1) + threadIdx.x];
        if (argmax) {
            int best = 0;
            float bv = tile[threadIdx.x];
            for (int m = 1; m < M; ++m) {
                const float v = tile[m * (TP + 1) + threadIdx.x];
                if (v > bv) {
                    bv = v;
                    best = m;
                }
            }
            argmax[(long long)b * N + n0 + threadIdx.x] = best;
        }
    }
}

__global__ void fill_tables_kernel(unsigned long long *__restrict__ table, unsigned *__restrict__ first, long long n) {
    for (long long i = (long long)blockIdx.x * blockDim.x + threadIdx.x; i < n; i += (long long)gridDim.x * blockDim.x) {
        table[i] = EMPTY_KEY;
        first[i] = 0x7fffffffu;
    }
}

inline int grid1d(long long total, int per_block = 256, int cap = 256 * 32) {
    long long g = (total + per_block - 1) / per_block;
    if (g > cap) g = cap;
    if (g < 1) g = 1;
    return (int)g;
}

inline int grid_rep(long long total, int per_block, int rep) {
    const int g = grid1d(total, per_block, 256 * 64);
    return g <= rep ? rep : g / rep * rep;
}

void splat_ones(wsc_ctx *ctx, const LatticeDev &L, const TileGeom &tg, float *val, float *part) {
    hipLaunchKernelGGL(slot_ones_kernel, dim3((unsigned)L.n_tiles), dim3(256), 0, ctx->stream, L.tslot_start, L.slot_desc,
                       L.tent_w, L.d + 1, tg, part);
    hipLaunchKernelGGL(combine1_kernel, dim3(grid1d(L.rows)), dim3(256), 0, ctx->stream, part, L.row_slot_start, L.rows, val);
}

void combine4(wsc_ctx *ctx, hipStream_t st, const LatticeDev &L, const float *part, int LP, float *val) {
    WscKernelTimer timer(ctx, WSC_K_BLUR, ((double)L.n_slots + L.rows) * L.rep * L.M_cur * 4);
    if (L.sorted_dest)
        hipLaunchKernelGGL(combine4_kernel, dim3(grid_rep((long long)L.rows * L.rep, 256 / LP, L.rep)), dim3(256), 0,
                           st, (const f32x4_t *)part, L.row_slot_start, LP, L.rows, L.n_slots, L.rep, (f32x4_t *)val);
    else
        hipLaunchKernelGGL(combine4_balanced_kernel, dim3((unsigned)((L.rows + CB_ROWS - 1) / CB_ROWS)), dim3(256), 0, st,
                           (const f32x4_t *)part, L.row_slot_start, (const uint32_t *)L.part_row, LP, L.rows, (f32x4_t *)val);
}

float *blur_all1(wsc_ctx *ctx, const LatticeDev &L, float *a, float *b) {
    for (int j = 0; j <= L.d; ++j) {
        hipLaunchKernelGGL(blur1_kernel, dim3(grid1d(L.rows)), dim3(256), 0, ctx->stream, a,
                           L.nbr + (long long)j * L.rows, L.rows, b);
        float *t = a; a = b; b = t;
    }
    return a;
}

int blur_lds_prepare(wsc_ctx *ctx, const LatticeDev &L, int M) {
    if (L.rep != 1 || !L.img_row || !L.bl_ok) return WSC_OK;
    const int B = (int)L.v_per_image.size();
    if (L.bl_M != M) {
        std::vector<std::vector<int2>> q(8);
        size_t lds = 0;
        for (int b = 0; b < B; ++b) {
            const int v = blur_lds_variant(L.v_per_image[b]), gw = BL_VAR[v][0];
            lds = std::max(lds, (size_t)(L.v_per_image[b] + 1) * gw * 4);
            for (int g = 0; g * gw < M; ++g) q[b & 7].push_back(make_int2(b | (v << 24), g));
        }
        size_t len = 0;
        for (int x = 0; x < 8; ++x) len = std::max(len, q[x].size());
        std::vector<int2> &h = L.bl_blk_host;
        h.assign(len * 8, make_int2(-1, 0));
        for (int x = 0; x < 8; ++x)
            for (size_t i = 0; i < q[x].size(); ++i) h[i * 8 + x] = q[x][i];
        L.bl_M = -1;
        if ((int)h.size() > L.bl_cap) return WSC_OK;
        WSC_TRY(wsc_ctx_upload_small(ctx, L.bl_blk, h.data(), sizeof(int2) * h.size()));
        L.bl_nblk = (int)h.size();
        L.bl_lds = lds;
        L.bl_M = M;
    }
    return WSC_OK;
}
bool blur_lds(wsc_ctx *ctx, hipStream_t st, const LatticeDev &L, int LP, float *val) {
    const int M = L.M_cur;
    if (!ctx->opt[WSC_OPT_CRF_BLUR_ON_CHIP] || L.rep != 1 || !L.img_row || !L.bl_ok || L.bl_M != M) return false;
    if (L.bl_nblk == 0) return true;
    if (wsc_set_max_dynamic_lds(ctx, reinterpret_cast<const void *>(blur_lds_kernel), 160 * 1024) != WSC_OK) return false;
    BlurLdsArgs ba;
    ba.nbr = L.nbr; ba.img_row = L.img_row; ba.blk = L.bl_blk; ba.val = val; ba.Mp = 4 * LP; ba.M = M; ba.rows = L.rows;
    ba.npass = L.d + 1;
    WscKernelTimer timer(ctx, WSC_K_BLUR, 2.0 * (L.d + 1) * L.rows * M * 4);
    hipLaunchKernelGGL(blur_lds_kernel, dim3((unsigned)L.bl_nblk), dim3(BL_THREADS), L.bl_lds, st, ba);
    return true;
}

float *combine_blur_all4(wsc_ctx *ctx, hipStream_t st, const LatticeDev &L, int LP, const float *part, float *a, float *b) {
    const bool fused_off = !ctx->opt[WSC_OPT_CRF_FUSED_BLUR];
    if (L.d == 2 && L.tile_rows && L.tile_pstart && L.n_tiles_occ > 0 && !fused_off) {
        WscKernelTimer timer(ctx, WSC_K_BLUR, ((double)L.n_slots + L.rows) * L.rep * L.M_cur * 4);
        hipLaunchKernelGGL(blur3_tile_kernel, dim3((unsigned)(L.n_tiles_occ * L.rep)), dim3(GBI * GBJ), 0, st,
                           (const f32x4_t *)nullptr, L.tile_rows, L.tile_list, L.n_tiles_occ, LP, L.rows, L.rep, (f32x4_t *)b,
                           (const f32x4_t *)part, L.tile_pstart, L.n_slots);
        return b;
    }
    combine4(ctx, st, L, part, LP, a);
    if (blur_lds(ctx, st, L, LP, a)) return a;
    for (int j = 0; j <= L.d; ++j) {
        WscKernelTimer timer(ctx, WSC_K_BLUR, 2.0 * L.rows * L.rep * L.M_cur * 4);
        hipLaunchKernelGGL(blur4_kernel, dim3(grid_rep((long long)L.rows * L.rep, (256 / LP) * 4, L.rep)), dim3(256),
                           0, st, (const f32x4_t *)a, L.nbr + (long long)j * L.rows, LP, L.rows, L.rep,
                           (f32x4_t *)b);
        float *t = a; a = b; b = t;
    }
    return a;
}

constexpr int GT_MAX_LOCAL = 1022;
int gauss_fuse_tables(wsc_ctx *ctx, const TileGeom &tg, LatticeDev &L, CtxBlocks &own) {
    const int N = tg.H * tg.W, rows = L.rows, W = tg.W;
    std::vector<int32_t> off((size_t)N * 3), rss((size_t)rows + 1);
    std::vector<float> bary((size_t)N * 3), norm((size_t)N);
    std::vector<int2> nbr((size_t)3 * rows);
    WSC_HIP(hipMemcpyAsync(off.data(), L.offset, sizeof(int32_t) * off.size(), hipMemcpyDeviceToHost, ctx->stream));
    WSC_HIP(hipMemcpyAsync(bary.data(), L.bary, sizeof(float) * bary.size(), hipMemcpyDeviceToHost, ctx->stream));
    WSC_HIP(hipMemcpyAsync(norm.data(), L.norm, sizeof(float) * norm.size(), hipMemcpyDeviceToHost, ctx->stream));
    WSC_HIP(hipMemcpyAsync(rss.data(), L.row_slot_start, sizeof(int32_t) * rss.size(), hipMemcpyDeviceToHost, ctx->stream));
    WSC_HIP(hipMemcpyAsync(nbr.data(), L.nbr, sizeof(int2) * nbr.size(), hipMemcpyDeviceToHost, ctx->stream));
    WSC_HIP(hipStreamSynchronize(ctx->stream));
    std::vector<int> loc((size_t)rows, -1);
    std::vector<std::vector<int>> sets((size_t)tg.tpi);
    std::vector<int4> cnt((size_t)tg.tpi);
    int nvmax = 0;
    for (int j = 0; j < tg.tpi; ++j) {
        const TileBox tb = tile_box(tg, j);
        std::vector<int> &list = sets[j];
        auto add = [&](int R) {
            if (R > 0 && R < rows && loc[R] < 0) {
                loc[R] = (int)list.size();
                list.push_back(R);
            }
        };
        for (int ty = 0; ty < tb.ch; ++ty)
            for (int tx = 0; tx < tb.cw; ++tx) {
                const size_t n = (size_t)(tb.y0 + ty) * W + tb.x0 + tx;
                for (int r = 0; r < 3; ++r) add(off[n * 3 + r]);
            }
        int4 &c = cnt[j];
        c.x = (int)list.size();
        for (int axis = 2; axis >= 0; --axis) {
            const size_t cur = list.size();
            for (size_t i = 0; i < cur; ++i) {
                const int2 nb = nbr[(size_t)axis * rows + list[i]];
                add(nb.x);
                add(nb.y);
            }
            if (axis == 2) c.y = (int)list.size();
            if (axis == 1) c.z = (int)list.size();
        }
        c.w = (int)list.size();
        for (int R : list) loc[R] = -1;
        if ((int)list.size() > nvmax) nvmax = (int)list.size();
    }
    if (nvmax > GT_MAX_LOCAL || nvmax == 0) return WSC_OK;
    const int stride = nvmax + 1, zr = stride - 1;
    std::vector<int2> trows((size_t)tg.tpi * stride, make_int2(0, 0));
    std::vector<uint4> tnbr((size_t)tg.tpi * stride, make_uint4((unsigned)zr | ((unsigned)zr << 16), (unsigned)zr | ((unsigned)zr << 16),
                                                                (unsigned)zr | ((unsigned)zr << 16), 0u));
    std::vector<uint4> pix((size_t)N);
    for (int j = 0; j < tg.tpi; ++j) {
        const TileBox tb = tile_box(tg, j);
        const std::vector<int> &list = sets[j];
        const int nv = (int)list.size();
        for (int v = 0; v < nv; ++v) loc[list[v]] = v;
        auto lid = [&](int R) { return (R > 0 && R < rows && loc[R] >= 0) ? loc[R] : zr; };
        for (int v = 0; v < nv; ++v) {
            const int R = list[v];
            trows[(size_t)j * stride + v] = make_int2(rss[R], rss[R + 1] - rss[R]);
            unsigned w[3];
            for (int axis = 0; axis < 3; ++axis) {
                const int2 nb = nbr[(size_t)axis * rows + R];
                w[axis] = (unsigned)lid(nb.x) | ((unsigned)lid(nb.y) << 16);
            }
            tnbr[(size_t)j * stride + v] = make_uint4(w[0], w[1], w[2], 0u);
        }
        for (int ty = 0; ty < tb.ch; ++ty)
            for (int tx = 0; tx < tb.cw; ++tx) {
                const size_t n = (size_t)(tb.y0 + ty) * W + tb.x0 + tx;
                unsigned ids = 0;
                uint32_t bw[3];
                for (int r = 0; r < 3; ++r) {
                    ids |= (unsigned)lid(off[n * 3 + r]) << (10 * r);
                    const float bn = bary[n * 3 + r] * norm[n];
                    memcpy(&bw[r], &bn, sizeof(float));
                }
                pix[n] = make_uint4(ids, bw[0], bw[1], bw[2]);
            }
        for (int R : list) loc[R] = -1;
    }
    WSC_TRY(own.alloc(sizeof(int4) * cnt.size(), &L.gt_cnt));
    WSC_HIP(hipMemcpyAsync(L.gt_cnt, cnt.data(), sizeof(int4) * cnt.size(), hipMemcpyHostToDevice, ctx->stream));
    WSC_TRY(own.alloc(sizeof(int2) * trows.size(), &L.gt_rows));
    WSC_TRY(own.alloc(sizeof(uint4) * tnbr.size(), &L.gt_nbr));
    WSC_TRY(own.alloc(sizeof(uint4) * pix.size(), &L.gt_pix));
    WSC_HIP(hipMemcpyAsync(L.gt_rows, trows.data(), sizeof(int2) * trows.size(), hipMemcpyHostToDevice, ctx->stream));
    WSC_HIP(hipMemcpyAsync(L.gt_nbr, tnbr.data(), sizeof(uint4) * tnbr.size(), hipMemcpyHostToDevice, ctx->stream));
    WSC_HIP(hipMemcpyAsync(L.gt_pix, pix.data(), sizeof(uint4) * pix.size(), hipMemcpyHostToDevice, ctx->stream));
    WSC_HIP(hipStreamSynchronize(ctx->stream));
    L.gt_stride = stride;
    return WSC_OK;
}

constexpr int WSC_RETRY_FULL_TABLE = 1;

template <int D>
int build_lattice(wsc_crf *crf, LatticeDev &L, CtxBlocks &own, const uint8_t *rgb_dev, float sxy, float srgb, bool shared,
                  bool full_table) {
    wsc_ctx *ctx = crf->ctx;
    const int B = shared ? 1 : crf->B, N = crf->N, dp1 = D + 1;
    L.rep = shared ? crf->B : 1;
    const long long npix = (long long)B * N;
    const long long total = npix * dp1;
    WSC_CHECK(total < (1ll << 31), WSC_ERR_CAPACITY, "CRF batch too large: %lld lattice entries", total);
    L.d = D;
    L.n_pix = npix;
    L.alpha = 1.0f / (1.0f + powf(2.0f, -(float)D));
    long long cap = 1;
    const long long want = full_table ? 2ll * N * dp1 : (long long)N * dp1 / 8;
    while (cap < want || cap < 1024) cap <<= 1;
    WSC_CHECK(B * cap < (1ll << 31), WSC_ERR_CAPACITY, "CRF batch too large for the hash tables");
    WSC_CHECK(cap <= (1ll << 28), WSC_ERR_CAPACITY, "CRF image too large: hash slots do not fit 28 bits");

    CtxBlocks tmp(ctx);
    unsigned long long *table;
    int32_t *first, *slot2row, *rowimg;
    unsigned *bitmap, *wcount, *wprefix, *sums, *bound_dev;
    unsigned long long *rowkey;
    int *err;
    WSC_TRY(tmp.alloc(sizeof(unsigned long long) * B * cap, &table));
    WSC_TRY(tmp.alloc(sizeof(int32_t) * B * cap, &first));
    WSC_TRY(tmp.alloc(sizeof(int32_t) * B * cap, &slot2row));
    const long long nw = (total + 31) / 32 + 1;
    WSC_TRY(tmp.alloc(sizeof(unsigned) * nw, &bitmap));
    WSC_TRY(tmp.alloc(sizeof(unsigned) * nw, &wcount));
    WSC_TRY(tmp.alloc(sizeof(unsigned) * (nw + 1), &wprefix));
    WSC_TRY(tmp.alloc(sizeof(unsigned) * (size_t)(B + 1), &bound_dev));
    const int nblk = (int)((nw + SCAN_CHUNK - 1) / SCAN_CHUNK);
    WSC_TRY(tmp.alloc(sizeof(unsigned) * (nblk + 2), &sums));
    const TileGeom tg0 = make_geom(crf->H, crf->W);
    const int n_tiles0 = B * tg0.tpi;
    unsigned *zblk;
    WSC_TRY(tmp.alloc(sizeof(unsigned) * (size_t)(n_tiles0 + 1 + 4), &zblk));
    err = reinterpret_cast<int *>(zblk);
    WSC_TRY(own.alloc(sizeof(int32_t) * total, &L.offset));
    WSC_TRY(own.alloc(sizeof(float) * total, &L.bary));
    WSC_TRY(own.alloc(sizeof(float) * npix, &L.norm));
    WSC_TRY(own.alloc(sizeof(float) * total, &L.tent_w));
    WSC_TRY(own.alloc(sizeof(uint8_t) * total, &L.tent_p));

    hipLaunchKernelGGL(fill_tables_kernel, dim3(grid1d(B * cap)), dim3(256), 0, ctx->stream, table, (unsigned *)first,
                       (long long)B * cap);
    WSC_HIP(hipMemsetAsync(zblk, 0, sizeof(unsigned) * (size_t)(n_tiles0 + 1 + 4), ctx->stream));

    EmbedArgs ea;
    ea.rgb = rgb_dev; ea.B = B; ea.H = crf->H; ea.W = crf->W; ea.N = N;
    ea.inv_sxy_den = sxy; ea.inv_srgb_den = srgb;
    {
        const float inv_std_dev = (float)(std::sqrt(2.0 / 3.0) * (D + 1));
        for (int i = 0; i < 5; ++i)
            ea.scale[i] = i < D ? (float)(1.0 / std::sqrt((double)((i + 2) * (i + 1))) * inv_std_dev) : 0.f;
    }
    ea.table = table; ea.cap_mask = (unsigned)(cap - 1); ea.cap = cap;
    ea.bary = L.bary; ea.first = first; ea.err = err;
    const TileGeom tg = make_geom(crf->H, crf->W);
    L.n_tiles = B * tg.tpi;
    int32_t *sslot;
    unsigned *tile_nslots;
    WSC_TRY(tmp.alloc(sizeof(int32_t) * total, &sslot));
    tile_nslots = zblk + 4;
    {
        const int fb = ctx->opt[WSC_OPT_CRF_RANK_BALLOT] ? 1 : 0;
        if (ctx->opt[WSC_OPT_CRF_EMBED_FULL]) {
            hipLaunchKernelGGL(tile_embed_full_kernel<D>, dim3((unsigned)L.n_tiles), dim3(256), 0, ctx->stream, ea, tg, L.tent_w,
                               L.tent_p, sslot, tile_nslots, fb, (const int32_t *)nullptr, (const unsigned *)nullptr, L.n_tiles);
        } else {
            int32_t *redo_list;
            unsigned *redo_count;
            WSC_TRY(tmp.alloc(sizeof(int32_t) * (size_t)L.n_tiles, &redo_list));
            redo_count = zblk + 1;
            hipLaunchKernelGGL(tile_embed_kernel<D>, dim3((unsigned)L.n_tiles), dim3(256), 0, ctx->stream, ea, tg, L.tent_w, L.tent_p,
                               sslot, tile_nslots, fb, redo_list, redo_count);
            hipLaunchKernelGGL(tile_embed_full_kernel<D>, dim3((unsigned)std::min(L.n_tiles, 3 * ctx->num_cus)), dim3(256), 0, ctx->stream, ea,
                               tg, L.tent_w, L.tent_p, sslot, tile_nslots, fb, (const int32_t *)redo_list,
                               (const unsigned *)redo_count, L.n_tiles);
        }
    }
    const int per_img = N * dp1;
    const dim3 grid_tab((unsigned)grid1d(cap, 256, B >= 32 ? 256 : 8192 / (B > 0 ? B : 1)), (unsigned)B);
    WSC_HIP(hipMemsetAsync(bitmap, 0, sizeof(unsigned) * nw, ctx->stream));
    hipLaunchKernelGGL(first_bits_kernel, grid_tab, dim3(256), 0, ctx->stream, first, cap, per_img, bitmap);
    hipLaunchKernelGGL(popc_words_kernel, dim3(grid1d(nw)), dim3(256), 0, ctx->stream, bitmap, nw, wcount);
    WSC_TRY(exclusive_scan(ctx, wcount, nw, wprefix, sums));
    hipLaunchKernelGGL(image_bounds_kernel, dim3((unsigned)((B + 63) / 64)), dim3(64), 0, ctx->stream, bitmap, wprefix, per_img, B,
                       bound_dev);
    int herr = 0;
    unsigned vtot = 0;
    WSC_HIP(hipMemcpyAsync(&vtot, sums + nblk, sizeof(unsigned), hipMemcpyDeviceToHost, ctx->stream));
    WSC_HIP(hipMemcpyAsync(&herr, err, sizeof(int), hipMemcpyDeviceToHost, ctx->stream));
    std::vector<unsigned> bound(B, 0);
    WSC_HIP(hipMemcpyAsync(bound.data(), bound_dev, sizeof(unsigned) * (size_t)B, hipMemcpyDeviceToHost, ctx->stream));
    WSC_HIP(hipStreamSynchronize(ctx->stream));
    WSC_CHECK((herr & 1) == 0, WSC_ERR_KEY_RANGE,
              "CRF lattice coordinate outside the packed-key range (sxy=%g srgb=%g too small for this image size)",
              (double)sxy, (double)srgb);
    if (herr & 2) {
        WSC_CHECK(!full_table, WSC_ERR_CAPACITY, "CRF lattice hash table overflow at worst-case size");
        return WSC_RETRY_FULL_TABLE;
    }
    L.rows = (int)vtot + 1;
    L.v_per_image.resize(crf->B);
    if (shared)
        for (int b = 0; b < crf->B; ++b) L.v_per_image[b] = (int)vtot;
    else
        for (int b = 0; b < B; ++b) L.v_per_image[b] = (int)((b + 1 < B ? bound[b + 1] : vtot) - bound[b]);
    if (!shared) {
        WSC_TRY(own.alloc(sizeof(int32_t) * (size_t)(B + 1), &L.img_row));
        hipLaunchKernelGGL(image_rows_kernel, dim3((unsigned)(B / 64 + 1)), dim3(64), 0, ctx->stream, bound_dev, B, (int)vtot + 1,
                           L.img_row);
        L.max_img_rows = 0;
        for (int b = 0; b < B; ++b) L.max_img_rows = std::max(L.max_img_rows, (int)L.v_per_image[b]);
        L.bl_ok = B < (1 << 24);
        for (int b = 0; b < B; ++b)
            if (blur_lds_variant(L.v_per_image[b]) < 0) L.bl_ok = false;
        if (L.bl_ok) {
            L.bl_cap = 8 * ((B + 7) / 8) * 32;
            WSC_TRY(own.alloc(sizeof(int2) * (size_t)L.bl_cap, &L.bl_blk));
        }
    }

    WSC_TRY(tmp.alloc(sizeof(unsigned long long) * L.rows, &rowkey));
    WSC_TRY(tmp.alloc(sizeof(int32_t) * L.rows, &rowimg));
    WSC_TRY(own.alloc(sizeof(int2) * (size_t)dp1 * L.rows, &L.nbr));

    hipLaunchKernelGGL(assign_rows_kernel, grid_tab, dim3(256), 0, ctx->stream, first, table, cap, per_img, bitmap, wprefix, slot2row,
                       rowkey, rowimg);
    {
        int32_t *slot_row;
        unsigned *sums2, *row_nslots, *cursor, *sums3;
        const int nb2 = (L.n_tiles + 1 + SCAN_CHUNK - 1) / SCAN_CHUNK, nb3 = (L.rows + 1 + SCAN_CHUNK - 1) / SCAN_CHUNK;
        WSC_TRY(tmp.alloc(sizeof(unsigned) * (nb2 + 2), &sums2));
        WSC_TRY(tmp.alloc(sizeof(unsigned) * 2 * (size_t)(L.rows + 1), &row_nslots));
        cursor = row_nslots + (L.rows + 1);
        WSC_TRY(tmp.alloc(sizeof(unsigned) * (nb3 + 2), &sums3));
        WSC_TRY(own.alloc(sizeof(int32_t) * (L.n_tiles + 2), &L.tslot_start));
        WSC_TRY(own.alloc(sizeof(int32_t) * (L.rows + 2), &L.row_slot_start));
        WSC_HIP(hipMemsetAsync(row_nslots, 0, sizeof(unsigned) * 2 * (size_t)(L.rows + 1), ctx->stream));
        WSC_TRY(exclusive_scan(ctx, tile_nslots, L.n_tiles + 1, (unsigned *)L.tslot_start, sums2));
        unsigned ns = 0;
        WSC_HIP(hipMemcpyAsync(&ns, sums2 + nb2, sizeof(unsigned), hipMemcpyDeviceToHost, ctx->stream));
        WSC_HIP(hipStreamSynchronize(ctx->stream));
        L.n_slots = (int)ns;
        WSC_TRY(own.alloc(sizeof(int2) * (size_t)(L.n_slots + 1), &L.slot_desc));
        WSC_TRY(tmp.alloc(sizeof(int32_t) * (size_t)(L.n_slots + 1), &slot_row));
        unsigned *slot_key = nullptr;
        int32_t *dest_slot = nullptr;
        if (D == 2) {
            WSC_TRY(tmp.alloc(sizeof(unsigned) * (size_t)(L.n_slots + 1), &slot_key));
            WSC_TRY(tmp.alloc(sizeof(int32_t) * (size_t)(L.n_slots + 1), &dest_slot));
        }
        hipLaunchKernelGGL(tile_slots_kernel, dim3((unsigned)L.n_tiles), dim3(256), 0, ctx->stream, sslot, L.tent_p, L.offset, slot2row,
                           cap, dp1, tg,
                           L.tslot_start, L.slot_desc, slot_row, slot_key, row_nslots);
        WSC_TRY(exclusive_scan(ctx, row_nslots, L.rows + 1, (unsigned *)L.row_slot_start, sums3));
        if (!shared) WSC_TRY(own.alloc(sizeof(uint32_t) * (size_t)(L.n_slots + 1), &L.part_row));
        hipLaunchKernelGGL(slot_dest_kernel, dim3(grid1d(L.n_slots)), dim3(256), 0, ctx->stream, slot_row, L.n_slots,
                           L.row_slot_start, cursor, L.slot_desc, L.part_row);
        if (D == 2) {
            hipLaunchKernelGGL(dest_inverse_kernel, dim3(grid1d(L.n_slots)), dim3(256), 0, ctx->stream, L.slot_desc, L.n_slots,
                               dest_slot);
            hipLaunchKernelGGL(row_sort_dest_kernel, dim3(grid1d(L.rows)), dim3(256), 0, ctx->stream, slot_key, dest_slot,
                               L.row_slot_start, L.rows, L.slot_desc);
            L.sorted_dest = true;
        }
    }
    WSC_HIP(hipMemsetAsync(L.nbr, 0, sizeof(int2) * (size_t)dp1 * L.rows, ctx->stream));
    hipLaunchKernelGGL(neighbors_kernel<D>, dim3((unsigned)grid1d(L.rows, 256, 4096), (unsigned)dp1), dim3(256), 0, ctx->stream, rowkey,
                       rowimg, table, slot2row, cap, (unsigned)(cap - 1), L.rows, L.nbr);
    WSC_HIP(hipGetLastError());
    if (D == 2) {
        int2 *ij;
        int *bbox;
        WSC_TRY(tmp.alloc(sizeof(int2) * L.rows, &ij));
        WSC_TRY(tmp.alloc(sizeof(int) * 5, &bbox));
        const int init[5] = {0x7fffffff, 0x7fffffff, -0x7fffffff, -0x7fffffff, 0};
        WSC_TRY(wsc_ctx_upload_small(ctx, bbox, init, sizeof(init)));
        hipLaunchKernelGGL(gauss_ij_kernel, dim3(grid1d(L.rows)), dim3(256), 0, ctx->stream, rowkey, L.rows, ij, bbox);
        int hb[5] = {0, 0, -1, -1, 1};
        WSC_HIP(hipMemcpyAsync(hb, bbox, sizeof(hb), hipMemcpyDeviceToHost, ctx->stream));
        WSC_HIP(hipStreamSynchronize(ctx->stream));
        const long long nti = hb[2] >= hb[0] ? ((long long)hb[2] - hb[0]) / GTI + 1 : 0;
        const long long ntj = hb[3] >= hb[1] ? ((long long)hb[3] - hb[1]) / GTJ + 1 : 0;
        if (hb[4] == 0 && nti > 0 && ntj > 0 && nti * ntj <= 4ll * L.rows + 64) {
            const long long nt = nti * ntj;
            int32_t *occ;
            WSC_TRY(tmp.alloc(sizeof(int32_t) * nt, &occ));
            WSC_TRY(own.alloc(sizeof(int32_t) * nt * GBI * GBJ, &L.tile_rows));
            WSC_HIP(hipMemsetAsync(L.tile_rows, 0, sizeof(int32_t) * nt * GBI * GBJ, ctx->stream));
            WSC_HIP(hipMemsetAsync(occ, 0, sizeof(int32_t) * nt, ctx->stream));
            hipLaunchKernelGGL(gauss_tile_fill_kernel, dim3(grid1d(L.rows)), dim3(256), 0, ctx->stream, ij, L.rows, hb[0],
                               hb[1], (int)nti, (int)ntj, L.tile_rows, occ);
            std::vector<int32_t> hocc(nt), list;
            WSC_HIP(hipMemcpyAsync(hocc.data(), occ, sizeof(int32_t) * nt, hipMemcpyDeviceToHost, ctx->stream));
            WSC_HIP(hipStreamSynchronize(ctx->stream));
            for (long long t = 0; t < nt; ++t)
                if (hocc[t]) list.push_back((int32_t)t);
            L.n_tiles_occ = (int)list.size();
            if (L.n_tiles_occ > 0) {
                WSC_TRY(own.alloc(sizeof(int32_t) * list.size(), &L.tile_list));
                WSC_HIP(hipMemcpyAsync(L.tile_list, list.data(), sizeof(int32_t) * list.size(), hipMemcpyHostToDevice,
                                       ctx->stream));
                WSC_HIP(hipStreamSynchronize(ctx->stream));
                WSC_TRY(own.alloc(sizeof(int2) * nt * GBI * GBJ, &L.tile_pstart));
                hipLaunchKernelGGL(gauss_tile_pstart_kernel, dim3(grid1d(nt * GBI * GBJ)), dim3(256), 0, ctx->stream,
                                   L.tile_rows, L.row_slot_start, nt * GBI * GBJ, L.tile_pstart);
            }
        }
    }
    float *va, *vb, *vp;
    WSC_TRY(tmp.alloc(sizeof(float) * L.rows, &va));
    WSC_TRY(tmp.alloc(sizeof(float) * L.rows, &vb));
    WSC_TRY(tmp.alloc(sizeof(float) * (size_t)(L.n_slots + 1), &vp));
    splat_ones(ctx, L, make_geom(crf->H, crf->W), va, vp);
    float *res = blur_all1(ctx, L, va, vb);
    uint32_t *rec_b = nullptr;
    if (D == 5 && !shared && crf->lat[0].gt_rows && !crf->pix_rec_b) WSC_TRY(own.alloc(sizeof(uint32_t) * 13 * (size_t)npix, &rec_b));
    if (!shared && D == 5) {
        hipLaunchKernelGGL(slice_norm_tile_kernel, dim3((unsigned)L.n_tiles), dim3(256), 0, ctx->stream, L.offset, L.bary, dp1,
                           L.alpha, res, make_geom(crf->H, crf->W), L.norm, rec_b, L.tent_w, L.tent_p);
    } else {
        hipLaunchKernelGGL(slice_norm_kernel, dim3(grid1d(npix)), dim3(256), 0, ctx->stream, L.offset, L.bary, dp1,
                           L.alpha, res, npix, L.norm, rec_b);
        hipLaunchKernelGGL(tile_scale_entries_kernel, dim3((unsigned)L.n_tiles), dim3(256), 0, ctx->stream, L.norm, dp1,
                           make_geom(crf->H, crf->W), L.tent_w, L.tent_p);
    }
    WSC_HIP(hipGetLastError());
    if (rec_b) crf->pix_rec_b = rec_b;
    return WSC_OK;
}

size_t update_splat_lds(int LP) { return sizeof(f32x4_t) * TILE_PIX * LP + sizeof(uint2) * GATHER_ENT + sizeof(int2) * GATHER_SB; }
size_t gauss_msg_lds(int LP, int gt_stride) { return ((size_t)LP * sizeof(f32x4_t) + sizeof(uint4)) * (size_t)gt_stride; }
size_t update_fg_lds(int LP, int gt_stride) { return update_splat_lds(LP) + gauss_msg_lds(LP, gt_stride); }
bool update_gf_ok(const wsc_ctx *ctx, const LatticeDev &G, int LP) {
    if (!ctx->opt[WSC_OPT_CRF_GAUSS_ON_CHIP]) return false;
    if (!G.gt_rows || G.rep < 1 || G.gt_stride <= 0) return false;
    if ((long long)G.gt_stride * LP > 6ll * GM_THREADS || (long long)G.gt_stride * LP >= 8192) return false;
    return gauss_msg_lds(LP, G.gt_stride) <= 64 * 1024;
}
bool update_fg_ok(const wsc_ctx *ctx, const LatticeDev &G, int LP) {
    if (!ctx->opt[WSC_OPT_CRF_MSG_IN_UPDATE] || !update_gf_ok(ctx, G, LP)) return false;
    return update_fg_lds(LP, G.gt_stride) <= 80 * 1024;
}
bool gauss_msg_small(int gt_stride, int LP) { return (long long)gt_stride * LP <= 4ll * GM_THREADS && LP <= 6; }

int launch_gauss_msg(wsc_ctx *ctx, hipStream_t st, const GaussMsgArgs &g, double bytes) {
    WscKernelTimer timer(ctx, WSC_K_GAUSS_MSG, bytes);
    const auto kernel = gauss_msg_small(g.gt_stride, g.LP) ? gauss_msg_kernel<4, 3> : gauss_msg_kernel<6, 4>;
    hipLaunchKernelGGL(kernel, dim3((unsigned)(g.B * g.tg.tpi)), dim3(GM_THREADS), gauss_msg_lds(g.LP, g.gt_stride), st, g);
    WSC_HIP(hipGetLastError());
    return WSC_OK;
}

typedef void (*UpdateKernel)(UpdateArgs);
template <bool SLICE, bool GF, int FG>
UpdateKernel update_kernel(bool splat) { return splat ? update_splat_kernel<SLICE, true, GF, FG> : update_splat_kernel<SLICE, false, GF, FG>; }
struct UpdateVariant { UpdateKernel kernel; int threads; size_t lds; };
UpdateVariant update_variant(bool slice, bool splat, bool gf, bool fg, bool small, int LP, int gt_stride) {
    if (fg) return {small ? update_kernel<true, true, 4>(splat) : update_kernel<true, true, 6>(splat), GM_THREADS, update_fg_lds(LP, gt_stride)};
    if (slice && gf) return {update_kernel<true, true, 0>(splat), 256, update_splat_lds(LP)};
    return {slice ? update_kernel<true, false, 0>(splat) : update_kernel<false, false, 0>(splat), 256, splat ? update_splat_lds(LP) : 0};
}
int update_fg_lds_limit(wsc_ctx *ctx, int LP, int gt_stride) {
    if (update_fg_lds(LP, gt_stride) <= 48 * 1024) return WSC_OK;
    for (const bool small : {true, false})
        for (const bool splat : {true, false}) {
            const UpdateKernel k = update_variant(true, splat, true, true, small, LP, gt_stride).kernel;
            WSC_TRY(wsc_set_max_dynamic_lds(ctx, reinterpret_cast<const void *>(k), 96 * 1024));
        }
    return WSC_OK;
}
int launch_update(wsc_ctx *ctx, const UpdateArgs &a, bool slice, bool splat, bool gf, bool fg = false, double fg_bytes = 0.0) {
    const double npix = (double)a.B * a.tg.H * a.tg.W;
    const double by = npix * (2.0 * a.M * 4 + (slice ? (gf ? 6 * 8 + 1.0 * a.M * 4 : 9 * 8 + 2.0 * a.M * 4) : 0.0) +
                              (splat ? 9 * 8 + 2.0 * a.M * 4 : 0.0));
    WscKernelTimer timer(ctx, WSC_K_SLICE_UPDATE, by + (fg ? fg_bytes : 0.0));
    const UpdateVariant v = update_variant(slice, splat, gf, fg, gauss_msg_small(a.gt_stride, a.LP), a.LP, a.gt_stride);
    hipLaunchKernelGGL(v.kernel, dim3((unsigned)(a.B * a.tg.tpi)), dim3(v.threads), v.lds, ctx->stream, a);
    WSC_HIP(hipGetLastError());
    return WSC_OK;
}

SplatTab splat_tab(const LatticeDev &L, float *part) {
    return SplatTab{L.tslot_start, L.slot_desc, L.tent_w, L.tent_p, part, L.n_slots, L.rep > 1 ? 1 : 0, L.d + 1};
}
UpdateArgs update_args(const wsc_crf *crf, int M, float g_compat, float bi_compat, const float *u, float *partg, float *partb) {
    const LatticeDev &G = crf->lat[0], &Bl = crf->lat[1];
    UpdateArgs a;
    a.pix_rec = crf->pix_rec; a.pix_rec_b = crf->pix_rec_b; a.val_g = nullptr; a.val_b = nullptr;
    a.u = u; a.q = nullptr; a.argmax = nullptr;
    a.alpha_g = G.alpha; a.alpha_b = Bl.alpha; a.compat_g = g_compat; a.compat_b = bi_compat;
    a.M = M; a.LP = (M + 3) / 4; a.B = crf->B; a.tg = make_geom(crf->H, crf->W);
    a.g_pix = (unsigned)G.n_pix; a.g_rows = G.rep > 1 ? (unsigned)G.rows : 0u;
    a.sg = splat_tab(G, partg); a.sb = splat_tab(Bl, partb);
    a.gt_cnt = G.gt_cnt; a.gt_rows = G.gt_rows; a.gt_nbr = G.gt_nbr; a.gt_pix = G.gt_pix; a.gt_stride = G.gt_stride;
    a.part_g_in = nullptr;
    return a;
}
GaussMsgArgs gauss_msg_args(const wsc_crf *crf, int M, float g_compat, const float *part, const float *u, float *e) {
    const LatticeDev &G = crf->lat[0];
    return GaussMsgArgs{G.gt_cnt, G.gt_rows, G.gt_nbr, G.gt_pix, part, u, e, G.gt_stride, G.n_slots, G.rep > 1 ? 1 : 0,
                        (M + 3) / 4, crf->B, g_compat * G.alpha, make_geom(crf->H, crf->W)};
}

int order_after_build(const wsc_crf *crf, hipStream_t st) {
    wsc_ctx *bctx = crf->ctx;
    if (st != bctx->stream) {
        WSC_HIP(hipEventRecord(bctx->join_ev, bctx->stream));
        WSC_HIP(hipStreamWaitEvent(st, bctx->join_ev, 0));
    }
    return WSC_OK;
}
int crf_full_records(wsc_crf *crf, hipStream_t st) {
    if (crf->pix_rec) return WSC_OK;
    WSC_TRY(crf->blocks.alloc(sizeof(uint4) * 5 * (size_t)crf->B * crf->N, &crf->pix_rec));
    WSC_TRY(order_after_build(crf, st));
    hipLaunchKernelGGL(pack_pixels_kernel, dim3((unsigned)grid1d((long long)crf->N * 5, 256, 2048), (unsigned)crf->B), dim3(256), 0, st,
                       crf->lat[0].offset, crf->lat[0].bary, crf->lat[0].norm, crf->lat[1].offset, crf->lat[1].bary,
                       crf->lat[1].norm, crf->N, crf->lat[0].rep > 1 ? 1 : 0, crf->pix_rec);
    WSC_HIP(hipGetLastError());
    return WSC_OK;
}
int crf_bilateral_records(wsc_crf *crf, hipStream_t st) {
    if (crf->pix_rec_b) return WSC_OK;
    WSC_TRY(crf->blocks.alloc(sizeof(uint32_t) * 13 * (size_t)crf->B * crf->N, &crf->pix_rec_b));
    WSC_TRY(order_after_build(crf, st));
    hipLaunchKernelGGL(pack_pixels_b_kernel, dim3((unsigned)grid1d((long long)crf->B * crf->N * 13, 256, 8192)), dim3(256), 0, st,
                       crf->lat[1].offset, crf->lat[1].bary, crf->lat[1].norm, (long long)crf->B * crf->N, crf->pix_rec_b);
    WSC_HIP(hipGetLastError());
    return WSC_OK;
}

int gauss_lattice(wsc_crf *crf, const uint8_t *rgb_dev, float sxy) {
    wsc_ctx *ctx = crf->ctx;
    if (!ctx->gauss_cache) ctx->gauss_cache = new WscGaussCache();
    std::vector<std::unique_ptr<GaussEntry>> &cache = ctx->gauss_cache->entries;
    GaussEntry *hit = nullptr;
    auto lru = cache.end();
    for (auto it = cache.begin(); it != cache.end(); ++it) {
        GaussEntry &g = **it;
        if (g.H == crf->H && g.W == crf->W && g.sxy == sxy) hit = &g;
        if (g.users == 0 && (lru == cache.end() || g.last_use < (*lru)->last_use)) lru = it;
    }
    if (!hit && (int)cache.size() >= GAUSS_CACHE_MAX && lru != cache.end()) cache.erase(lru);
    if (!hit) {
        CtxBlocks own(ctx);
        WSC_TRY(build_lattice<2>(crf, crf->lat[0], own, rgb_dev, sxy, 1.f, true, true));
        if ((int)cache.size() >= GAUSS_CACHE_MAX) {
            crf->blocks.take(std::move(own));
            return WSC_OK;
        }
        cache.emplace_back(new GaussEntry{crf->H, crf->W, sxy, crf->lat[0], std::move(own)});
        hit = cache.back().get();
    } else {
        if (hit->fuse_pending) {
            hit->fuse_pending = false;
            if (gauss_fuse_tables(ctx, make_geom(crf->H, crf->W), hit->L, hit->blocks) != WSC_OK) {
                hit->L.gt_cnt = nullptr; hit->L.gt_rows = nullptr; hit->L.gt_nbr = nullptr; hit->L.gt_pix = nullptr; hit->L.gt_stride = 0;
            }
        }
        crf->lat[0] = hit->L;
    }
    hit->users += 1;
    hit->last_use = ++g_gauss_use_clock;
    crf->gauss = hit;
    return WSC_OK;
}

int bilateral_lattice(wsc_crf *crf, const uint8_t *rgb_dev, float sxy, float srgb) {
    CtxBlocks own(crf->ctx);
    int st = build_lattice<5>(crf, crf->lat[1], own, rgb_dev, sxy, srgb, false, false);
    if (st == WSC_RETRY_FULL_TABLE) {
        own.release();
        crf->lat[1] = LatticeDev();
        st = build_lattice<5>(crf, crf->lat[1], own, rgb_dev, sxy, srgb, false, true);
    }
    if (st == WSC_OK) crf->blocks.take(std::move(own));
    return st;
}

}

extern "C" {

int wsc_crf_create(wsc_ctx *ctx, const uint8_t *rgb_dev, int B, int H, int W, float g_sxy, float bi_sxy,
                   float bi_srgb, wsc_crf **out) {
    WSC_CHECK(ctx && rgb_dev && out, WSC_ERR_INVALID, "wsc_crf_create: null argument");
    WSC_CHECK(B > 0 && H > 0 && W > 0, WSC_ERR_INVALID, "wsc_crf_create: B=%d H=%d W=%d", B, H, W);
    WSC_CHECK(g_sxy > 0.f && bi_sxy > 0.f && bi_srgb > 0.f, WSC_ERR_INVALID,
              "wsc_crf_create: kernel widths must be positive");
    WSC_HIP(hipSetDevice(ctx->device));
    wsc_crf *crf = new wsc_crf(ctx);
    crf->B = B; crf->H = H; crf->W = W; crf->N = H * W;
    WscKernelTimer timer(ctx, WSC_K_CRF_BUILD, (double)B * H * W * (3.0 * 16 + 6.0 * 16));
    int st = gauss_lattice(crf, rgb_dev, g_sxy);
    crf->lat[0].rep = B;
    crf->lat[0].v_per_image.assign(B, crf->lat[0].rows - 1);
    if (st == WSC_OK) st = bilateral_lattice(crf, rgb_dev, bi_sxy, bi_srgb);
    if (st == WSC_OK && !(crf->lat[0].gt_rows && update_gf_ok(ctx, crf->lat[0], 8))) st = crf_full_records(crf, ctx->stream);
    if (st == WSC_OK && crf->lat[0].gt_rows) st = crf_bilateral_records(crf, ctx->stream);
    if (st != WSC_OK) {
        wsc_crf_destroy(crf);
        return st;
    }
    *out = crf;
    return WSC_OK;
}

void wsc_crf_destroy(wsc_crf *crf) {
    if (!crf) return;
    if (crf->used_elsewhere && crf->use_ev) (void)hipStreamWaitEvent(crf->ctx->stream, crf->use_ev, 0);
    if (crf->gauss) crf->gauss->users -= 1;
    crf->blocks.release();
    if (crf->use_ev) (void)hipEventDestroy(crf->use_ev);
    delete crf;
}

int wsc_crf_lattice_sizes(wsc_ctx *ctx, const wsc_crf *crf, int32_t *v_gauss_host, int32_t *v_bilat_host) {
    WSC_CHECK(ctx && crf, WSC_ERR_INVALID, "wsc_crf_lattice_sizes: null argument");
    for (int b = 0; b < crf->B; ++b) {
        if (v_gauss_host) v_gauss_host[b] = crf->lat[0].v_per_image[b];
        if (v_bilat_host) v_bilat_host[b] = crf->lat[1].v_per_image[b];
    }
    return WSC_OK;
}

int wsc_crf_gaussian_on_chip(const wsc_crf *crf, int M) {
    if (!crf || M < 1 || M > 32) return 0;
    return update_gf_ok(crf->ctx, crf->lat[0], (M + 3) / 4) ? 1 : 0;
}

static int crf_inference_impl(wsc_ctx *ctx, wsc_crf *crf, const float *unary_dev, bool pixel_major, int M, float g_compat,
                              float bi_compat, int n_iters, float *q_dev, int32_t *argmax_dev);

int wsc_crf_inference(wsc_ctx *ctx, wsc_crf *crf, const float *unary_dev, int M, float g_compat, float bi_compat,
                      int n_iters, float *q_dev, int32_t *argmax_dev) {
    return crf_inference_impl(ctx, crf, unary_dev, false, M, g_compat, bi_compat, n_iters, q_dev, argmax_dev);
}

int wsc_crf_inference_pm(wsc_ctx *ctx, wsc_crf *crf, const float *unary_pm_dev, int M, float g_compat, float bi_compat,
                         int n_iters, float *q_dev, int32_t *argmax_dev) {
    return crf_inference_impl(ctx, crf, unary_pm_dev, true, M, g_compat, bi_compat, n_iters, q_dev, argmax_dev);
}

static int crf_inference_impl(wsc_ctx *ctx, wsc_crf *crf, const float *unary_dev, bool pixel_major, int M, float g_compat,
                              float bi_compat, int n_iters, float *q_dev, int32_t *argmax_dev) {
    WSC_CHECK(ctx && crf && unary_dev, WSC_ERR_INVALID, "wsc_crf_inference: null argument");
    WSC_CHECK(M >= 1 && M <= 32, WSC_ERR_INVALID, "wsc_crf_inference: M=%d outside [1,32]", M);
    WSC_CHECK(n_iters >= 0, WSC_ERR_INVALID, "wsc_crf_inference: n_iters=%d", n_iters);
    WSC_HIP(hipSetDevice(ctx->device));
    const int B = crf->B, N = crf->N;
    const long long npix = (long long)B * N;
    const LatticeDev &G = crf->lat[0], &Bl = crf->lat[1];
    const int LP = (M + 3) / 4, Mp = 4 * LP;
    const long long g_rows = (long long)G.rows * G.rep, g_slots = (long long)G.n_slots * G.rep;
    WSC_CHECK(npix * Mp < (1ll << 30) && g_rows * Mp < (1ll << 30) && (long long)Bl.rows * Mp < (1ll << 30) &&
                  g_slots * Mp < (1ll << 30) && (long long)Bl.n_slots * Mp < (1ll << 30) && npix * 80 < (1ll << 32),
              WSC_ERR_CAPACITY, "CRF batch too large for 32-bit byte offsets (B*N*Mp = %lld elements; split the batch)", npix * Mp);
    WSC_CHECK(N < (1 << 24) && G.rows < (1 << 24) && Bl.rows < (1 << 24), WSC_ERR_CAPACITY,
              "CRF image / lattice too large for 24-bit row arithmetic (N = %d, rows = %d / %d)", N, G.rows, Bl.rows);
    auto al = [](size_t v) { return (v + 255) / 256 * 256; };
    const size_t qb = al(sizeof(float) * npix * Mp);
    const size_t pg = al(sizeof(float) * (size_t)g_slots * Mp), pb = al(sizeof(float) * (size_t)Bl.n_slots * Mp);
    const size_t vg = al(sizeof(float) * (size_t)g_rows * Mp), vb = al(sizeof(float) * (size_t)Bl.rows * Mp);
    void *ws;
    WSC_TRY(wsc_ctx_workspace(ctx, 2 * qb + 2 * vg + 2 * vb + 2 * pg + pb, &ws));
    char *p = (char *)ws;
    float *u = (float *)p; p += qb;
    float *q = (float *)p; p += qb;
    float *vg0 = (float *)p; p += vg;
    float *vg1 = (float *)p; p += vg;
    float *vb0 = (float *)p; p += vb;
    float *vb1 = (float *)p; p += vb;
    float *partg = (float *)p; p += pg;
    float *partg2 = (float *)p; p += pg;
    float *partb = (float *)p; p += pb;

    crf->lat[0].M_cur = M;
    crf->lat[1].M_cur = M;
    if (n_iters > 0) WSC_TRY(blur_lds_prepare(ctx, crf->lat[1], M));
    const dim3 tgrid((N + TP - 1) / TP, B);
    if (!pixel_major) {
        WscKernelTimer timer(ctx, WSC_K_CRF_MISC, (double)npix * M * 12);
        hipLaunchKernelGGL(init_q_kernel, tgrid, dim3(TP), 2 * (size_t)M * (TP + 1) * sizeof(float), ctx->stream,
                           unary_dev, M, Mp, N, u, n_iters == 0 ? q : (float *)nullptr);
    } else {
        u = const_cast<float *>(unary_dev);
    }
    const bool lds_blur = Bl.bl_ok && Bl.img_row && ctx->opt[WSC_OPT_CRF_BLUR_ON_CHIP];
    const bool no_fork = lds_blur || ctx->profiling;
    if (!no_fork && !ctx->aux_stream) {
        WSC_HIP(hipStreamCreateWithFlags(&ctx->aux_stream, hipStreamNonBlocking));
        WSC_HIP(hipEventCreateWithFlags(&ctx->fork_ev, hipEventDisableTiming));
        WSC_HIP(hipEventCreateWithFlags(&ctx->aux_done_ev, hipEventDisableTiming));
    }
    const bool gf = update_gf_ok(ctx, G, LP);
    const bool fg = gf && update_fg_ok(ctx, G, LP) && update_fg_lds_limit(ctx, LP, G.gt_stride) == WSC_OK;
    if (n_iters > 0) WSC_TRY(gf ? crf_bilateral_records(crf, ctx->stream) : crf_full_records(crf, ctx->stream));
    UpdateArgs a = update_args(crf, M, g_compat, bi_compat, u, partg, partb);
    const GaussMsgArgs gm = gauss_msg_args(crf, M, g_compat, partg, u, q);
    const double gf_bytes = 2.0 * 3.0 * (double)(G.rows - 1) * G.rep * M * 4 + (double)npix * (3 * 8 + 1.0 * M * 4);
    if (n_iters == 0 && pixel_major) {
        a.q = q;
        WSC_TRY(launch_update(ctx, a, false, false, false));
    }
    for (int it = 0; it <= n_iters && n_iters > 0; ++it) {
        const bool last = it == n_iters;
        const bool labels_only = last && q_dev == nullptr && argmax_dev != nullptr;
        a.q = last && !labels_only ? q : nullptr;
        a.argmax = labels_only ? argmax_dev : nullptr;
        a.u = (gf && !fg && it > 0) ? q : u;
        if (fg) {
            a.part_g_in = (it & 1) ? partg : partg2;
            a.sg.part = (it & 1) ? partg2 : partg;
        }
        WSC_TRY(launch_update(ctx, a, it > 0, !last, gf, fg && it > 0, gf_bytes));
        if (last) break;
// ... 151 lines not shown
```

### wsss-analysis_amd/wsscam/_lib.py

```python
import ctypes
import os
import re
import threading

import numpy as np

_HERE = os.path.dirname(os.path.abspath(__file__))
LIB_PATH = os.path.join(_HERE, "libwsscam.so")
HEADER_PATH = os.path.normpath(os.path.join(_HERE, "..", "..", "include", "wsscam.h"))

WSC_OK = 0
WSC_ERR_INVALID = -1
WSC_ERR_NO_DEVICE = -2
WSC_ERR_HIP = -3
WSC_ERR_MISSING_KEY = -4
WSC_ERR_SHAPE = -5
WSC_ERR_NOMEM = -6
WSC_ERR_KEY_RANGE = -7
WSC_ERR_CAPACITY = -8
WSC_ERR_RANGE = -9

ARCH_RESNET50_CAM = 0
ARCH_VGG16_CAM = 1
ARCH_M7_CAM = 2
ARCH_RESNET50_IRN = 3
ARCH_VGG16_IRN = 4
ARCH_M7_IRN = 5

PREC_BF16 = 0
PREC_BF16X3 = 1
PREC_F16 = 2
PREC_F16X3 = 3
PREC_F32 = 4
OPT_CRF_GAUSS_ON_CHIP, OPT_CRF_FUSED_BLUR, OPT_CRF_BLUR_ON_CHIP, OPT_CRF_RANK_BALLOT, OPT_CRF_EMBED_FULL, OPT_RW_TILED, \
    OPT_STEM_POOL_FUSED, OPT_CONV_WINDOW, OPT_CAM_HEAD_STREAM, OPT_CRF_MSG_IN_UPDATE = range(10)
OPT_DEFAULTS = {OPT_CRF_GAUSS_ON_CHIP: 1, OPT_CRF_FUSED_BLUR: 1, OPT_CRF_BLUR_ON_CHIP: 1, OPT_CRF_RANK_BALLOT: 0,
                OPT_CRF_EMBED_FULL: 0, OPT_RW_TILED: -1, OPT_STEM_POOL_FUSED: 1, OPT_CONV_WINDOW: 1, OPT_CAM_HEAD_STREAM: 1,
                OPT_CRF_MSG_IN_UPDATE: 1}
CONV_GENERIC = 0x100


class WscError(RuntimeError):
    def __init__(self, status, message):
        super().__init__("libwsscam error %d: %s" % (status, message))
        self.status = status


class TensorDesc(ctypes.Structure):
    _fields_ = [
        ("name", ctypes.c_char_p),
        ("data", ctypes.POINTER(ctypes.c_float)),
        ("ndim", ctypes.c_int32),
        ("shape", ctypes.c_int64 * 4),
    ]


_lib = None

_vp = ctypes.c_void_p
_i = ctypes.c_int
_f = ctypes.c_float
_sz = ctypes.c_size_t

_SIGNATURES = {
    "wsc_version": (_i, []),
    "wsc_last_error": (ctypes.c_char_p, []),
    "wsc_ctx_create": (_i, [_i, _vp, ctypes.POINTER(_vp)]),
    "wsc_ctx_destroy": (None, [_vp]),
    "wsc_sync": (_i, [_vp]),
    "wsc_ctx_range_status": (_i, [_vp, ctypes.POINTER(_i), _i]),
    "wsc_ctx_wait": (_i, [_vp, _vp]),
    "wsc_ctx_mark": (_i, [_vp, _i]),
    "wsc_ctx_wait_mark": (_i, [_vp, _i]),
    "wsc_ctx_wait_for_mark": (_i, [_vp, _vp, _i]),
    "wsc_device_info": (_i, [_vp, ctypes.c_char_p, _sz, ctypes.POINTER(_i)]),
    "wsc_malloc": (_i, [_vp, _sz, ctypes.POINTER(_vp)]),
    "wsc_free": (_i, [_vp, _vp]),
    "wsc_memcpy_h2d": (_i, [_vp, _vp, _vp, _sz]),
    "wsc_memcpy_d2h": (_i, [_vp, _vp, _vp, _sz]),
    "wsc_memset": (_i, [_vp, _vp, _i, _sz]),
    "wsc_ctx_set_option": (_i, [_vp, _i, _i]),
    "wsc_host_alloc": (_i, [_vp, _sz, ctypes.POINTER(_vp)]),
    "wsc_host_free": (_i, [_vp, _vp]),
    "wsc_host_write_segments": (_i, [ctypes.c_char_p, _i, ctypes.POINTER(_vp), ctypes.POINTER(_sz)]),
    "wsc_memcpy_h2d_async": (_i, [_vp, _vp, _vp, _sz]),
    "wsc_memcpy_d2h_async": (_i, [_vp, _vp, _vp, _sz]),
    "wsc_profile_begin": (_i, [_vp]),
    "wsc_profile_end": (_i, [_vp, _i, _vp, _vp, _vp, ctypes.POINTER(_i)]),
    "wsc_profile_class_name": (ctypes.c_char_p, [_i]),
    "wsc_timer_begin": (_i, [_vp]),
    "wsc_timer_end": (_i, [_vp, ctypes.POINTER(_f)]),
    "wsc_net_create": (_i, [_vp, _i, ctypes.POINTER(TensorDesc), _i, _i, _i, ctypes.POINTER(_vp)]),
    "wsc_net_destroy": (None, [_vp]),
    "wsc_net_cam_size": (_i, [_vp, _i, ctypes.POINTER(_i)]),
    "wsc_net_feat_channels": (_i, [_vp, ctypes.POINTER(_i)]),
    "wsc_net_forward_cam": (_i, [_vp, _vp, _vp, _i, _i, _vp, _vp]),
    "wsc_net_forward_gradcam": (_i, [_vp, _vp, _vp, _i, _i, _i, _vp, _vp]),
    "wsc_net_forward_features": (_i, [_vp, _vp, _vp, _i, _i, _vp]),
    "wsc_net_cam_size_hw": (_i, [_vp, _i, _i, ctypes.POINTER(_i), ctypes.POINTER(_i)]),
    "wsc_net_forward_cam_hw": (_i, [_vp, _vp, _vp, _i, _i, _i, _vp, _vp]),
    "wsc_net_forward_edge": (_i, [_vp, _vp, _vp, _i, _i, _i, _i, _vp, _vp]),
    "wsc_rw_propagate": (_i, [_vp, _vp, _vp, _i, _i, _i, _vp, _vp, _vp, _i, _f, _i, _vp]),
    "wsc_rw_propagate_batch": (_i, [_vp, _i, _vp, _vp, _vp, _vp, _vp, _vp, _vp, _vp, _i, _f, _i, _vp]),
    "wsc_conv2d_nchw": (_i, [_vp, _vp, _i, _i, _i, _i, _vp, _i, _i, _i, _i, _i, _vp, _vp, _vp, _i, _i, _vp]),
    "wsc_cam_postprocess": (_i, [_vp, _vp, _i, _i, _i, _i, _vp, _vp, _vp, _vp, _vp, _vp, _vp]),
    "wsc_cam_eval_confusion": (_i, [_vp, _vp, _i, _vp, _vp, _vp, _vp, _f, _vp, _i, _i, _vp, _vp]),
    "wsc_unary_from_maps": (_i, [_vp, _vp, _i, _i, _i, _f, _vp]),
    "wsc_cam_unary": (_i, [_vp, _vp, _i, _i, _i, _i, _i, _i, _f, _vp]),
    "wsc_cam_unary_pm": (_i, [_vp, _vp, _i, _i, _i, _i, _i, _i, _f, _vp]),
    "wsc_cam_sum_scales": (_i, [_vp, _vp, _i, _i, ctypes.c_longlong, _vp]),
    "wsc_cam_eval_confusion_nn": (_i, [_vp, _vp, _i, _vp, _vp, _vp, _vp, _vp, _vp, _i, _i, _vp, _vp]),
    "wsc_label_confusion_nn": (_i, [_vp, _vp, _i, _vp, _vp, _vp, _vp, _i, _i, _vp, _vp]),
    "wsc_sem_seg_finish": (_i, [_vp, _vp, _i, _vp, _vp, _vp, _vp, _vp, _vp, _i, _f, _vp]),
    "wsc_bilinear_resize": (_i, [_vp, _vp, _i, _i, _i, _vp, _i, _i]),
    "wsc_msf_input_u8": (_i, [_vp, _vp, _i, _vp, _vp, _i, _vp, _vp, _i, _i, _vp]),
    "wsc_resize_u8": (_i, [_vp, _vp, _i, _vp, _vp, _i, _i, _vp]),
    "wsc_label_unary_from_cam": (_i, [_vp, _vp, _i, _i, _i, _f, _f, _vp, _vp]),
    "wsc_ir_label_combine": (_i, [_vp, _vp, _vp, _vp, _i, _i, _i, _vp]),
    "wsc_hsn_gradcam_post": (_i, [_vp, _vp, _i, _i, _i, _i, _i, _vp, _vp, _i, _i]),
    "wsc_hsn_voc_background": (_i, [_vp, _vp, _i, _i, _i, _vp, _i]),
    "wsc_hsn_class_mass": (_i, [_vp, _vp, _i, _i, _vp]),
    "wsc_hsn_background": (_i, [_vp, _vp, _i, _i, _i, _i, _i, _vp]),
    "wsc_cam_adp_modify": (_i, [_vp, _vp, _i, _i, _i, _i, _vp, _i, _vp, _i, _vp, _i, _vp, _i, _vp]),
    "wsc_hsn_cs_gradcam": (_i, [_vp, _vp, _i, _i, _i, _vp, _vp, _i, _i, _i, _vp, _i, _vp, _i, _vp, _vp, _vp]),
    "wsc_hsn_gather_unary": (_i, [_vp, _vp, _vp, _i, _i, _vp]),
    "wsc_crf_create": (_i, [_vp, _vp, _i, _i, _i, _f, _f, _f, ctypes.POINTER(_vp)]),
    "wsc_crf_destroy": (None, [_vp]),
    "wsc_crf_lattice_sizes": (_i, [_vp, _vp, _vp, _vp]),
    "wsc_crf_gaussian_on_chip": (_i, [_vp, _i]),
    "wsc_crf_inference": (_i, [_vp, _vp, _vp, _i, _f, _f, _i, _vp, _vp]),
    "wsc_crf_inference_pm": (_i, [_vp, _vp, _vp, _i, _f, _f, _i, _vp, _vp]),
    "wsc_crf_v_create": (_i, [_vp, _vp, _vp, _i, _f, _f, _f, ctypes.POINTER(_vp)]),
    "wsc_crf_v_destroy": (None, [_vp]),
    "wsc_crf_v_num_groups": (_i, [_vp]),
    "wsc_crf_v_inference": (_i, [_vp, _vp, _vp, _vp, _f, _f, _i, _vp, _vp]),
}


def header_symbols():
    with open(HEADER_PATH) as fh:
        text = fh.read()
    text = re.sub(r"/\*.*?\*/", "", text, flags=re.S)
    return sorted(set(re.findall(r"\b(wsc_[a-z0-9_]+)\s*\(", text)))


def load():
    global _lib
    if _lib is not None:
        return _lib
    if not os.path.exists(LIB_PATH):
        raise WscError(WSC_ERR_NO_DEVICE,
                       "libwsscam.so not built at %s -- run `python __graft_entry__.py` (there is no "
                       "CPU fallback for the product path)" % LIB_PATH)
    lib = ctypes.CDLL(LIB_PATH)
    for name, (res, args) in _SIGNATURES.items():
        fn = getattr(lib, name)
        fn.restype = res
        fn.argtypes = args
    _lib = lib
    return lib


def check_exports():
    lib = load()
    declared = header_symbols()
    missing = [s for s in declared if not hasattr(lib, s)]
    unbound = [s for s in declared if s not in _SIGNATURES]
    if missing or unbound:
        raise WscError(WSC_ERR_INVALID, "missing exports %s / unbound %s" % (missing, unbound))
    return declared


def check(status):
    if status != WSC_OK:
        raise WscError(status, load().wsc_last_error().decode("utf-8", "replace"))


def _ptr(x):
    if x is None:
        return None
    if isinstance(x, DeviceBuffer):
        return x.ptr
    if isinstance(x, np.ndarray):
        assert x.flags["C_CONTIGUOUS"]
        return x.ctypes.data
    if isinstance(x, int):
        return x
    if hasattr(x, "data_ptr"):
        return x.data_ptr()
    raise TypeError("cannot take a pointer of %r" % type(x))


class StackChain:

    SLOT = 7

    def __init__(self):
        self._lock = threading.Lock()
        self._last = None

    def run(self, ctx, enqueue):
        with self._lock:
            prev = self._last
            if prev is not None and prev is not ctx:
                ctx.wait_for_mark(prev, self.SLOT)
            try:
                return enqueue()
            finally:
                ctx.mark(self.SLOT)
                self._last = ctx


class Context:

    def __init__(self, device=0, stream=None):
        lib = load()
        h = _vp()
        check(lib.wsc_ctx_create(int(device), stream, ctypes.byref(h)))
        self.h = h
        self.device = device
        self._lib = lib
        self._options = {}

    def close(self):
        if getattr(self, "h", None):
            pool = self.__dict__.pop("_pool", None)
            if pool:
                for lst in pool.values():
                    for buf in lst:
                        self._lib.wsc_free(self.h, buf.ptr)
                        buf.ptr = None
            self._lib.wsc_ctx_destroy(self.h)
            self.h = None

    def __del__(self):
        try:
            self.close()
        except Exception:
            pass

    def sync(self):
        check(self._lib.wsc_sync(self.h))

    def range_status(self, clear=False):
        f = _i(0)
        check(self._lib.wsc_ctx_range_status(self.h, ctypes.byref(f), 1 if clear else 0))
        return int(f.value)

    def mark(self, slot):
        check(self._lib.wsc_ctx_mark(self.h, int(slot)))

    def wait_mark(self, slot):
        check(self._lib.wsc_ctx_wait_mark(self.h, int(slot)))

    def wait_for_mark(self, other, slot):
        check(self._lib.wsc_ctx_wait_for_mark(self.h, other.h, int(slot)))

    def wait_for(self, other):
        check(self._lib.wsc_ctx_wait(self.h, other.h))

    def device_info(self):
        buf = ctypes.create_string_buffer(128)
        n = _i()
        check(self._lib.wsc_device_info(self.h, buf, 128, ctypes.byref(n)))
        return buf.value.decode(), n.value

    def alloc(self, nbytes, pooled=False):
        nbytes = int(nbytes)
        if pooled:
            size = 1 << max(16, (max(nbytes, 1) - 1).bit_length())
            pool = self.__dict__.setdefault("_pool", {})
            lst = pool.get(size)
            if lst:
                buf = lst.pop()
                buf.nbytes = nbytes
                return buf
            buf = DeviceBuffer(self, size)
            buf.nbytes, buf._pool_size = nbytes, size
            return buf
        return DeviceBuffer(self, nbytes)

    def to_device(self, arr, pooled=False):
        arr = np.ascontiguousarray(arr)
        buf = self.alloc(arr.nbytes, pooled=pooled)
        check(self._lib.wsc_memcpy_h2d(self.h, buf.ptr, arr.ctypes.data, arr.nbytes))
        self.sync()
        return buf

    def to_host(self, buf, shape, dtype, offset_bytes=0):
        out = np.empty(shape, dtype=dtype)
        check(self._lib.wsc_memcpy_d2h(self.h, out.ctypes.data, _ptr(buf) + offset_bytes, out.nbytes))
        return out

    def host_alloc(self, nbytes):
        return PinnedBuffer(self, int(nbytes))

    def h2d_async(self, dst_dev, pinned, nbytes, dst_offset=0, src_offset=0):
        check(self._lib.wsc_memcpy_h2d_async(self.h, _ptr(dst_dev) + dst_offset, pinned.ptr + src_offset, int(nbytes)))

    def d2h_async(self, pinned, src_dev, nbytes, dst_offset=0, src_offset=0):
        check(self._lib.wsc_memcpy_d2h_async(self.h, pinned.ptr + dst_offset, _ptr(src_dev) + src_offset, int(nbytes)))

    def set_option(self, option, value):
        check(self._lib.wsc_ctx_set_option(self.h, int(option), int(value)))
        self._options[int(option)] = int(value)

    def get_option(self, option):
        return self._options.get(int(option), OPT_DEFAULTS[int(option)])

    def option(self, option, value):
        import contextlib

        @contextlib.contextmanager
        def _cm():
            before = self.get_option(option)
            self.set_option(option, value)
            try:
                yield self
            finally:
                self.set_option(option, before)

        return _cm()

    def profile_begin(self):
        check(self._lib.wsc_profile_begin(self.h))

    def profile_end(self):
        n = 16
        calls = np.zeros(n, np.int32)
        ms = np.zeros(n, np.float32)
        work = np.zeros(n, np.float64)
        k = _i()
        check(self._lib.wsc_profile_end(self.h, n, calls.ctypes.data, ms.ctypes.data, work.ctypes.data, ctypes.byref(k)))
        return {self._lib.wsc_profile_class_name(i).decode(): (int(calls[i]), float(ms[i]), float(work[i]))
                for i in range(k.value) if calls[i] > 0}

    def timer_begin(self):
        check(self._lib.wsc_timer_begin(self.h))

    def timer_end(self):
        ms = _f()
# ... 463 lines not shown
```

Baseline: 2644 images/s.

## Add lean CRF path: planar combine output, fused popc scan, fewer memsets

Adds a default-on CRF_LEAN option that trims lattice-build and blur launches. It folds the bitmap and row-count zeroing into existing kernels, fuses popcount into the scan, and adds a single-block scan for small arrays. It also fuses splat-ones with the normalisation blur in LDS. Combine now writes directly into per-image column-group planes that the LDS blur reads contiguously, which removes a strided gather. The cost is more template variants and added complexity, including a per-row plane descriptor array.

```diff
diff --git a/include/wsscam.h b/include/wsscam.h
--- a/include/wsscam.h
+++ b/include/wsscam.h
@@ -53,7 +53,8 @@
     WSC_OPT_CONV_WINDOW = 7,
     WSC_OPT_CAM_HEAD_STREAM = 8,
     WSC_OPT_CRF_MSG_IN_UPDATE = 9,
-    WSC_OPT_COUNT = 10
+    WSC_OPT_CRF_LEAN = 10,
+    WSC_OPT_COUNT = 11
 } wsc_option;
 
 typedef struct wsc_crf wsc_crf;
diff --git a/wsss-analysis_amd/csrc/common.h b/wsss-analysis_amd/csrc/common.h
--- a/wsss-analysis_amd/csrc/common.h
+++ b/wsss-analysis_amd/csrc/common.h
@@ -136,7 +136,7 @@
     };
     PinSlot pin_ring[PIN_SLOTS];
     int pin_next = 0;
-    int opt[WSC_OPT_COUNT] = {1, 1, 1, 0, 0, -1, 1, 1, 1, 1};
+    int opt[WSC_OPT_COUNT] = {1, 1, 1, 0, 0, -1, 1, 1, 1, 1, 1};
     void *zero_page = nullptr;
     unsigned *range_host = nullptr, *range_dev = nullptr;
     hipEvent_t ev0 = nullptr, ev1 = nullptr;
diff --git a/wsss-analysis_amd/csrc/crf.hip b/wsss-analysis_amd/csrc/crf.hip
--- a/wsss-analysis_amd/csrc/crf.hip
+++ b/wsss-analysis_amd/csrc/crf.hip
@@ -41,6 +41,7 @@
     int32_t *img_row = nullptr;
     int max_img_rows = 0;
     uint32_t *part_row = nullptr;
+    int2 *row_plane = nullptr;
     bool bl_ok = false;
     int2 *bl_blk = nullptr;
     int bl_cap = 0;
@@ -328,6 +329,26 @@
     return ok;
 }
 
+constexpr int BL_THREADS = 1024;
+constexpr int BL_NVAR = 5;
+constexpr int BL_VAR[BL_NVAR][2] = {{4, 4}, {4, 10}, {3, 13}, {2, 20}, {1, 26}};
+__host__ __device__ inline bool blur_lds_fits(int rows, int gw, int rpt) {
+    return rows <= rpt * BL_THREADS && (size_t)(rows + 1) * gw * 4 <= 160 * 1024 && rows < 65535;
+}
+inline int blur_lds_variant(int rows) {
+    for (int v = 0; v < BL_NVAR; ++v)
+        if (blur_lds_fits(rows, BL_VAR[v][0], BL_VAR[v][1])) return v;
+    return -1;
+}
+__device__ __forceinline__ int blur_lds_gw(int rows) {
+    if (blur_lds_fits(rows, BL_VAR[0][0], BL_VAR[0][1])) return BL_VAR[0][0];
+    if (blur_lds_fits(rows, BL_VAR[1][0], BL_VAR[1][1])) return BL_VAR[1][0];
+    if (blur_lds_fits(rows, BL_VAR[2][0], BL_VAR[2][1])) return BL_VAR[2][0];
+    if (blur_lds_fits(rows, BL_VAR[3][0], BL_VAR[3][1])) return BL_VAR[3][0];
+    if (blur_lds_fits(rows, BL_VAR[4][0], BL_VAR[4][1])) return BL_VAR[4][0];
+    return 0;
+}
+
 __global__ void first_bits_kernel(const int32_t *__restrict__ first, long long cap, int per_img, unsigned *__restrict__ bitmap) {
     const int b = blockIdx.y;
     const int32_t *fi = first + (long long)b * cap;
@@ -359,8 +380,19 @@
 __global__ void assign_rows_kernel(const int32_t *__restrict__ first, const unsigned long long *__restrict__ table, long long cap,
                                    int per_img, const unsigned *__restrict__ bitmap, const unsigned *__restrict__ wprefix,
                                    int32_t *__restrict__ slot2row, unsigned long long *__restrict__ rowkey,
-                                   int32_t *__restrict__ rowimg) {
+                                   int32_t *__restrict__ rowimg, unsigned *__restrict__ zero, long long nz,
+                                   const int32_t *__restrict__ img_row, int2 *__restrict__ row_plane) {
     const int b = blockIdx.y;
+    int2 plane = make_int2(0, 0);
+    if (row_plane) {
+        const int ir0 = img_row[b], inr = img_row[b + 1] - ir0;
+        plane = make_int2(ir0, inr | (blur_lds_gw(inr) << 24));
+        if (blockIdx.x == 0 && b == 0 && threadIdx.x == 0) row_plane[0] = make_int2(0, 0);
+    }
+    if (zero) {
+        const long long nthr = (long long)gridDim.x * gridDim.y * blockDim.x;
+        for (long long i = ((long long)blockIdx.y * gridDim.x + blockIdx.x) * blockDim.x + threadIdx.x; i < nz; i += nthr) zero[i] = 0u;
+    }
     for (long long sl = (long long)blockIdx.x * blockDim.x + threadIdx.x; sl < cap; sl += (long long)gridDim.x * blockDim.x) {
         const long long s_ = (long long)b * cap + sl;
         const int f = first[s_];
@@ -369,10 +401,15 @@
         slot2row[s_] = row;
         rowkey[row] = table[s_];
         rowimg[row] = b;
+        if (row_plane) row_plane[row] = plane;
     }
 }
 
 constexpr int SCAN_CHUNK = 4096;
+template <bool POPC>
+__device__ __forceinline__ unsigned scan_in(const unsigned *__restrict__ in, long long idx) {
+    return POPC ? (unsigned)__popc(in[idx]) : in[idx];
+}
 
 __device__ __forceinline__ unsigned block_exclusive_scan_256(unsigned v, unsigned *lds, unsigned &total) {
     const int lane = threadIdx.x & 63, wv = threadIdx.x >> 6;
@@ -390,6 +427,7 @@
     return base + x - v;
 }
 
+template <bool POPC>
 __global__ __launch_bounds__(256) void scan_reduce_kernel(const unsigned *__restrict__ in, long long n,
                                                           unsigned *__restrict__ sums) {
     __shared__ unsigned lds[4];
@@ -397,7 +435,7 @@
     unsigned s = 0;
     for (int i = 0; i < 16; ++i) {
         const long long idx = base + i * 256 + threadIdx.x;
-        if (idx < n) s += in[idx];
+        if (idx < n) s += scan_in<POPC>(in, idx);
     }
     for (int o = 32; o > 0; o >>= 1) s += __shfl_down(s, o, 64);
     if ((threadIdx.x & 63) == 0) lds[threadIdx.x >> 6] = s;
@@ -419,6 +457,7 @@
     if (threadIdx.x == 0) sums[m] = carry;
 }
 
+template <bool POPC>
 __global__ __launch_bounds__(256) void scan_apply_kernel(const unsigned *__restrict__ in, long long n,
                                                          const unsigned *__restrict__ sums, unsigned *__restrict__ out) {
     __shared__ unsigned lds[4];
@@ -429,7 +468,7 @@
     const long long t0 = base + (long long)threadIdx.x * 16;
 #pragma unroll
     for (int i = 0; i < 16; ++i) {
-        v[i] = (t0 + i < n) ? in[t0 + i] : 0u;
+        v[i] = (t0 + i < n) ? scan_in<POPC>(in, t0 + i) : 0u;
         s += v[i];
     }
     unsigned total;
@@ -441,6 +480,7 @@
     }
 }
 
+template <bool POPC>
 __global__ __launch_bounds__(256) void scan_apply_fused_kernel(const unsigned *__restrict__ in, long long n,
                                                                unsigned *__restrict__ sums, int nblk, unsigned *__restrict__ out) {
     __shared__ unsigned lds[4];
@@ -464,7 +504,7 @@
     const long long t0 = base + (long long)threadIdx.x * 16;
 #pragma unroll
     for (int i = 0; i < 16; ++i) {
-        v[i] = (t0 + i < n) ? in[t0 + i] : 0u;
+        v[i] = (t0 + i < n) ? scan_in<POPC>(in, t0 + i) : 0u;
         s += v[i];
     }
     unsigned total;
@@ -476,16 +516,56 @@
     }
 }
 
-int exclusive_scan(wsc_ctx *ctx, const unsigned *in, long long n, unsigned *out, unsigned *sums ) {
+constexpr int SCAN_ONE = 1024 * 16;
+__global__ __launch_bounds__(1024) void scan_one_block_kernel(const unsigned *__restrict__ in, int n, unsigned *__restrict__ sums,
+                                                              int nblk, unsigned *__restrict__ out) {
+    __shared__ unsigned wtot[16];
+    const int lane = threadIdx.x & 63, wv = threadIdx.x >> 6;
+    const int t0 = (int)threadIdx.x * 16;
+    unsigned v[16];
+    unsigned s = 0;
+#pragma unroll
+    for (int i = 0; i < 16; ++i) {
+        v[i] = (t0 + i < n) ? in[t0 + i] : 0u;
+        s += v[i];
+    }
+    unsigned x = s;
+    for (int o = 1; o < 64; o <<= 1) {
+        const unsigned y = __shfl_up(x, o, 64);
+        if (lane >= o) x += y;
+    }
+    if (lane == 63) wtot[wv] = x;
+    __syncthreads();
+    unsigned base = 0, total = 0;
+    for (int i = 0; i < 16; ++i) {
+        if (i < wv) base += wtot[i];
+        total += wtot[i];
+    }
+    if (threadIdx.x == 0) sums[nblk] = total;
+    unsigned ex = base + x - s;
+#pragma unroll
+    for (int i = 0; i < 16; ++i) {
+        if (t0 + i < n) out[t0 + i] = ex;
+        ex += v[i];
+    }
+}
+
+template <bool POPC = false>
+int exclusive_scan(wsc_ctx *ctx, const unsigned *in, long long n, unsigned *out, unsigned *sums , bool one_block = false) {
     const int nblk = (int)((n + SCAN_CHUNK - 1) / SCAN_CHUNK);
-    hipLaunchKernelGGL(scan_reduce_kernel, dim3(nblk), dim3(256), 0, ctx->stream, in, n, sums);
-    if (nblk <= 256) {
-        hipLaunchKernelGGL(scan_apply_fused_kernel, dim3(nblk), dim3(256), 0, ctx->stream, in, n, sums, nblk, out);
+    if (!POPC && one_block && n <= SCAN_ONE) {
+        hipLaunchKernelGGL(scan_one_block_kernel, dim3(1), dim3(1024), 0, ctx->stream, in, (int)n, sums, nblk, out);
         WSC_HIP(hipGetLastError());
         return WSC_OK;
     }
+    hipLaunchKernelGGL(scan_reduce_kernel<POPC>, dim3(nblk), dim3(256), 0, ctx->stream, in, n, sums);
+    if (nblk <= 256) {
+        hipLaunchKernelGGL(scan_apply_fused_kernel<POPC>, dim3(nblk), dim3(256), 0, ctx->stream, in, n, sums, nblk, out);
+        WSC_HIP(hipGetLastError());
+        return WSC_OK;
+    }
     hipLaunchKernelGGL(scan_sums_kernel, dim3(1), dim3(256), 0, ctx->stream, sums, nblk);
-    hipLaunchKernelGGL(scan_apply_kernel, dim3(nblk), dim3(256), 0, ctx->stream, in, n, sums, out);
+    hipLaunchKernelGGL(scan_apply_kernel<POPC>, dim3(nblk), dim3(256), 0, ctx->stream, in, n, sums, out);
     WSC_HIP(hipGetLastError());
     return WSC_OK;
 }
@@ -984,18 +1064,42 @@
 }
 
 constexpr int CB_ROWS = 32;
+__device__ __forceinline__ size_t blur_plane_at(int ir0, int inr, int Mp, int c0) { return (size_t)ir0 * Mp + (size_t)inr * c0; }
+template <bool PLANAR>
 __global__ __launch_bounds__(256) void combine4_balanced_kernel(const f32x4_t *__restrict__ part, const int32_t *__restrict__ row_slot_start,
                                                                 const uint32_t *__restrict__ part_row, int LP, int rows,
-                                                                f32x4_t *__restrict__ val) {
+                                                                f32x4_t *__restrict__ val, const int2 *__restrict__ row_plane,
+                                                                float *__restrict__ pval) {
     __shared__ int rss_l[CB_ROWS + 1];
+    __shared__ int2 rpl_l[PLANAR ? CB_ROWS : 1];
     __shared__ unsigned long long acc[CB_ROWS * 32];
     const int r0 = blockIdx.x * CB_ROWS;
     const int nr = min(CB_ROWS, rows - r0);
     const int P0 = row_slot_start[r0], P1 = row_slot_start[r0 + nr];
     for (int i = threadIdx.x; i <= nr; i += 256) rss_l[i] = row_slot_start[r0 + i];
+    if (PLANAR)
+        for (int i = threadIdx.x; i < nr; i += 256) rpl_l[i] = row_plane[r0 + i];
     for (int i = threadIdx.x; i < CB_ROWS * 32; i += 256) acc[i] = 0ull;
     const int gpb = 256 / LP;
     const int tr = threadIdx.x / LP, l = threadIdx.x - tr * LP;
+    auto put = [&](int lo, const f32x4_t &o) {
+        if (PLANAR) {
+            const int2 rp = rpl_l[lo];
+            const int gw = rp.y >> 24;
+            if (gw) {
+                const int ir0 = rp.x, inr = rp.y & 0xffffff, Mp = 4 * LP;
+#pragma unroll
+                for (int k = 0; k < 4; ++k) {
+                    const int c = 4 * l + k;
+                    const int g = gw == 4 ? c >> 2 : gw == 3 ? (c * 86) >> 8 : gw == 2 ? c >> 1 : c;
+                    const int c0 = g * gw, w = min(gw, Mp - c0);
+                    pval[blur_plane_at(ir0, inr, Mp, c0) + (size_t)(r0 + lo - ir0) * w + (c - c0)] = o[k];
+                }
+                return;
+            }
+        }
+        val[(unsigned)(r0 + lo) * (unsigned)LP + l] = o;
+    };
     constexpr int U = 4;
     f32x4_t v[U];
     uint32_t pr[U];
@@ -1036,7 +1140,7 @@
                         single = rss_l[lo + 1] - rss_l[lo] == 1;
                     }
                     if (single) {
-                        val[(unsigned)(r0 + lo) * (unsigned)LP + l] = v[u];
+                        put(lo, v[u]);
                     } else {
 #pragma unroll
                         for (int k = 0; k < 4; ++k)
@@ -1056,7 +1160,7 @@
 #pragma unroll
                 for (int k = 0; k < 4; ++k) o[k] = (float)(long long)acc[row * 32 + 4 * l + k] * PFIX_INV;
             }
-            val[(unsigned)(r0 + row) * (unsigned)LP + l] = o;
+            put(row, o);
         }
     }
 }
@@ -1110,21 +1214,16 @@
     }
 }
 
-constexpr int BL_THREADS = 1024;
-constexpr int BL_NVAR = 5;
-constexpr int BL_VAR[BL_NVAR][2] = {{4, 4}, {4, 10}, {3, 13}, {2, 20}, {1, 26}};
-inline int blur_lds_variant(int rows) {
-    for (int v = 0; v < BL_NVAR; ++v)
-        if (rows <= BL_VAR[v][1] * BL_THREADS && (size_t)(rows + 1) * BL_VAR[v][0] * 4 <= 160 * 1024 && rows < 65535) return v;
-    return -1;
-}
 struct BlurLdsArgs {
     const int2 *nbr;
     const int32_t *img_row;
     const int2 *blk;
     float *val;
+    const float *src;
+    const int32_t *rss;
     int Mp, M, rows, npass;
 };
+enum { BL_SRC_ROWS = 0, BL_SRC_PLANES = 1, BL_SRC_ONES = 2 };
 template <int GW> struct FloatRun { float v[GW]; };
 typedef float f32x3u_t __attribute__((ext_vector_type(3), aligned(4)));
 template <int GW>
@@ -1154,7 +1253,7 @@
     } else if constexpr (GW == 2) *reinterpret_cast<f32x2_t *>(q) = f32x2_t{r.v[0], r.v[1]};
     else q[0] = r.v[0];
 }
-template <int GW, int RPT>
+template <int GW, int RPT, int SRC>
 __device__ __forceinline__ void blur_lds_body(const BlurLdsArgs &p, float *pl, int img, int grp) {
     const int r0 = p.img_row[img], nr = p.img_row[img + 1] - r0;
     const int stride = nr + 1;
@@ -1179,20 +1278,74 @@
                     nb[i0 + i] = (unsigned)(raw[i].x ? raw[i].x - r0 : nr) | ((unsigned)(raw[i].y ? raw[i].y - r0 : nr) << 16);
         }
     };
-    load_idx(0);
-#pragma unroll
-    for (int i = 0; i < RPT; ++i) {
-        const int r = tid + i * BL_THREADS;
-        if (r < nr) {
-            FloatRun<GW> run;
-            if (GW == 3 && c0 + GW > p.Mp) {
-#pragma unroll
-                for (int g = 0; g < GW; ++g) run.v[g] = c0 + g < p.Mp ? vb[(size_t)r * p.Mp + g] : 0.f;
-            } else {
-                run = load_run<GW>(vb + (size_t)r * p.Mp);
-            }
-#pragma unroll
-            for (int g = 0; g < GW; ++g) pl[g * stride + r] = c0 + g < p.M ? run.v[g] : 0.f;
+    if constexpr (SRC != BL_SRC_ONES) load_idx(0);
+    if constexpr (SRC == BL_SRC_ONES) {
+        static_assert(GW == 1, "one value per row");
+        constexpr int CH = RPT < 8 ? RPT : 8;
+        const int32_t *rs = p.rss + r0;
+#pragma unroll 1
+        for (int i0 = 0; i0 < RPT; i0 += CH) {
+            int sb[CH], n[CH];
+            long long acc[CH];
+            int nmax = 0;
+#pragma unroll
+            for (int i = 0; i < CH; ++i) {
+                const int r = tid + (i0 + i) * BL_THREADS;
+                sb[i] = 0; n[i] = 0; acc[i] = 0;
+                if (i0 + i < RPT && r < nr) {
+                    sb[i] = rs[r];
+                    n[i] = rs[r + 1] - sb[i];
+                }
+                nmax = max(nmax, n[i]);
+            }
+            for (int k = 0; k < nmax; ++k) {
+                float v[CH];
+#pragma unroll
+                for (int i = 0; i < CH; ++i) v[i] = k < n[i] ? p.src[sb[i] + k] : 0.f;
+#pragma unroll
+                for (int i = 0; i < CH; ++i)
+                    if (k < n[i]) acc[i] += (long long)__float2int_rn(v[i] * PFIX_SCALE);
+            }
+#pragma unroll
+            for (int i = 0; i < CH; ++i) {
+                const int r = tid + (i0 + i) * BL_THREADS;
+                if (i0 + i < RPT && r < nr) pl[r] = (float)acc[i] * PFIX_INV;
+            }
+        }
+        load_idx(0);
+    } else if constexpr (SRC == BL_SRC_PLANES) {
+        const int w = min(GW, p.Mp - c0);
+        const float *q = p.src + blur_plane_at(r0, nr, p.Mp, c0);
+#pragma unroll
+        for (int i = 0; i < RPT; ++i) {
+            const int r = tid + i * BL_THREADS;
+            if (r < nr) {
+                FloatRun<GW> run;
+                if (w < GW) {
+#pragma unroll
+                    for (int g = 0; g < GW; ++g) run.v[g] = g < w ? q[(size_t)r * w + g] : 0.f;
+                } else {
+                    run = load_run<GW>(q + (size_t)r * GW);
+                }
+#pragma unroll
+                for (int g = 0; g < GW; ++g) pl[g * stride + r] = c0 + g < p.M ? run.v[g] : 0.f;
+            }
+        }
+    } else {
+#pragma unroll
+        for (int i = 0; i < RPT; ++i) {
+            const int r = tid + i * BL_THREADS;
+            if (r < nr) {
+                FloatRun<GW> run;
+                if (GW == 3 && c0 + GW > p.Mp) {
+#pragma unroll
+                    for (int g = 0; g < GW; ++g) run.v[g] = c0 + g < p.Mp ? vb[(size_t)r * p.Mp + g] : 0.f;
+                } else {
+                    run = load_run<GW>(vb + (size_t)r * p.Mp);
+                }
+#pragma unroll
+                for (int g = 0; g < GW; ++g) pl[g * stride + r] = c0 + g < p.M ? run.v[g] : 0.f;
+            }
         }
     }
     if (tid < GW) pl[tid * stride + nr] = 0.f;
@@ -1237,18 +1390,35 @@
         }
     }
 }
+template <bool PLANAR>
 __global__ __launch_bounds__(BL_THREADS) void blur_lds_kernel(BlurLdsArgs p) {
     extern __shared__ float pl[];
     const int2 w = p.blk[blockIdx.x];
     if (w.x < 0) return;
     const int img = w.x & 0xffffff;
+    constexpr int SRC = PLANAR ? BL_SRC_PLANES : BL_SRC_ROWS;
+    static_assert(BL_NVAR == 5, "one case per variant here and in blur_lds_gw");
     switch (w.x >> 24) {
-    case 0: blur_lds_body<BL_VAR[0][0], BL_VAR[0][1]>(p, pl, img, w.y); break;
-    case 1: blur_lds_body<BL_VAR[1][0], BL_VAR[1][1]>(p, pl, img, w.y); break;
-    case 2: blur_lds_body<BL_VAR[2][0], BL_VAR[2][1]>(p, pl, img, w.y); break;
-    case 3: blur_lds_body<BL_VAR[3][0], BL_VAR[3][1]>(p, pl, img, w.y); break;
-    default: blur_lds_body<BL_VAR[4][0], BL_VAR[4][1]>(p, pl, img, w.y); break;
-    }
+    case 0: blur_lds_body<BL_VAR[0][0], BL_VAR[0][1], SRC>(p, pl, img, w.y); break;
+    case 1: blur_lds_body<BL_VAR[1][0], BL_VAR[1][1], SRC>(p, pl, img, w.y); break;
+    case 2: blur_lds_body<BL_VAR[2][0], BL_VAR[2][1], SRC>(p, pl, img, w.y); break;
+    case 3: blur_lds_body<BL_VAR[3][0], BL_VAR[3][1], SRC>(p, pl, img, w.y); break;
+    default: blur_lds_body<BL_VAR[4][0], BL_VAR[4][1], SRC>(p, pl, img, w.y); break;
+    }
+}
+
+constexpr int NB_NVAR = 3;
+constexpr int NB_RPT[NB_NVAR] = {4, 12, BL_VAR[BL_NVAR - 1][1]};
+static_assert(BL_VAR[BL_NVAR - 1][0] == 1, "the last variant holds one class per workgroup");
+inline bool norm_blur_fits(int rows) { return blur_lds_fits(rows, 1, NB_RPT[NB_NVAR - 1]); }
+__global__ __launch_bounds__(BL_THREADS) void norm_blur_lds_kernel(BlurLdsArgs p) {
+    extern __shared__ float pl[];
+    const int img = blockIdx.x;
+    const int nr = p.img_row[img + 1] - p.img_row[img];
+    if (img == 0 && threadIdx.x == 0) p.val[0] = 0.f;
+    if (nr <= NB_RPT[0] * BL_THREADS) blur_lds_body<1, NB_RPT[0], BL_SRC_ONES>(p, pl, img, 0);
+    else if (nr <= NB_RPT[1] * BL_THREADS) blur_lds_body<1, NB_RPT[1], BL_SRC_ONES>(p, pl, img, 0);
+    else blur_lds_body<1, NB_RPT[2], BL_SRC_ONES>(p, pl, img, 0);
 }
 
 constexpr int GTI = 12, GTJ = 12, GBI = GTI + 4, GBJ = GTJ + 4;
@@ -2299,11 +2469,17 @@
     }
 }
 
-__global__ void fill_tables_kernel(unsigned long long *__restrict__ table, unsigned *__restrict__ first, long long n) {
-    for (long long i = (long long)blockIdx.x * blockDim.x + threadIdx.x; i < n; i += (long long)gridDim.x * blockDim.x) {
+__global__ void fill_tables_kernel(unsigned long long *__restrict__ table, unsigned *__restrict__ first, long long n,
+                                   unsigned *__restrict__ z0, long long n0, unsigned *__restrict__ z1, long long n1) {
+    const long long t = (long long)blockIdx.x * blockDim.x + threadIdx.x, nthr = (long long)gridDim.x * blockDim.x;
+    for (long long i = t; i < n; i += nthr) {
         table[i] = EMPTY_KEY;
         first[i] = 0x7fffffffu;
     }
+    if (z0)
+        for (long long i = t; i < n0; i += nthr) z0[i] = 0u;
+    if (z1)
+        for (long long i = t; i < n1; i += nthr) z1[i] = 0u;
 }
 
 inline int grid1d(long long total, int per_block = 256, int cap = 256 * 32) {
@@ -2323,15 +2499,32 @@
                        L.tent_w, L.d + 1, tg, part);
     hipLaunchKernelGGL(combine1_kernel, dim3(grid1d(L.rows)), dim3(256), 0, ctx->stream, part, L.row_slot_start, L.rows, val);
 }
-
-void combine4(wsc_ctx *ctx, hipStream_t st, const LatticeDev &L, const float *part, int LP, float *val) {
+bool splat_blur_ones_lds(wsc_ctx *ctx, const LatticeDev &L, const TileGeom &tg, float *val, float *part) {
+    if (L.rep != 1 || !L.img_row || L.v_per_image.empty()) return false;
+    for (const int32_t v : L.v_per_image)
+        if (!norm_blur_fits(v)) return false;
+    if (wsc_set_max_dynamic_lds(ctx, reinterpret_cast<const void *>(norm_blur_lds_kernel), 160 * 1024) != WSC_OK) return false;
+    hipLaunchKernelGGL(slot_ones_kernel, dim3((unsigned)L.n_tiles), dim3(256), 0, ctx->stream, L.tslot_start, L.slot_desc,
+                       L.tent_w, L.d + 1, tg, part);
+    BlurLdsArgs ba;
+    ba.nbr = L.nbr; ba.img_row = L.img_row; ba.blk = nullptr; ba.val = val; ba.Mp = 1; ba.M = 1; ba.rows = L.rows;
+    ba.npass = L.d + 1;
+    ba.src = part; ba.rss = L.row_slot_start;
+    hipLaunchKernelGGL(norm_blur_lds_kernel, dim3((unsigned)L.v_per_image.size()), dim3(BL_THREADS),
+                       sizeof(float) * (size_t)(L.max_img_rows + 1), ctx->stream, ba);
+    return true;
+}
+
+void combine4(wsc_ctx *ctx, hipStream_t st, const LatticeDev &L, const float *part, int LP, float *val, float *planes = nullptr) {
     WscKernelTimer timer(ctx, WSC_K_BLUR, ((double)L.n_slots + L.rows) * L.rep * L.M_cur * 4);
     if (L.sorted_dest)
         hipLaunchKernelGGL(combine4_kernel, dim3(grid_rep((long long)L.rows * L.rep, 256 / LP, L.rep)), dim3(256), 0,
                            st, (const f32x4_t *)part, L.row_slot_start, LP, L.rows, L.n_slots, L.rep, (f32x4_t *)val);
     else
-        hipLaunchKernelGGL(combine4_balanced_kernel, dim3((unsigned)((L.rows + CB_ROWS - 1) / CB_ROWS)), dim3(256), 0, st,
-                           (const f32x4_t *)part, L.row_slot_start, (const uint32_t *)L.part_row, LP, L.rows, (f32x4_t *)val);
+        hipLaunchKernelGGL(planes ? combine4_balanced_kernel<true> : combine4_balanced_kernel<false>,
+                           dim3((unsigned)((L.rows + CB_ROWS - 1) / CB_ROWS)), dim3(256), 0, st, (const f32x4_t *)part,
+                           L.row_slot_start, (const uint32_t *)L.part_row, LP, L.rows, (f32x4_t *)val,
+                           (const int2 *)L.row_plane, planes);
 }
 
 float *blur_all1(wsc_ctx *ctx, const LatticeDev &L, float *a, float *b) {
@@ -2369,17 +2562,22 @@
     }
     return WSC_OK;
 }
-bool blur_lds(wsc_ctx *ctx, hipStream_t st, const LatticeDev &L, int LP, float *val) {
+bool blur_lds_ok(wsc_ctx *ctx, const LatticeDev &L) {
+    if (!ctx->opt[WSC_OPT_CRF_BLUR_ON_CHIP] || L.rep != 1 || !L.img_row || !L.bl_ok || L.bl_M != L.M_cur) return false;
+    if (L.bl_nblk == 0) return true;
+    return wsc_set_max_dynamic_lds(ctx, reinterpret_cast<const void *>(blur_lds_kernel<false>), 160 * 1024) == WSC_OK &&
+           wsc_set_max_dynamic_lds(ctx, reinterpret_cast<const void *>(blur_lds_kernel<true>), 160 * 1024) == WSC_OK;
+}
+void blur_lds(wsc_ctx *ctx, hipStream_t st, const LatticeDev &L, int LP, float *val, const float *planes) {
+    if (L.bl_nblk == 0) return;
     const int M = L.M_cur;
-    if (!ctx->opt[WSC_OPT_CRF_BLUR_ON_CHIP] || L.rep != 1 || !L.img_row || !L.bl_ok || L.bl_M != M) return false;
-    if (L.bl_nblk == 0) return true;
-    if (wsc_set_max_dynamic_lds(ctx, reinterpret_cast<const void *>(blur_lds_kernel), 160 * 1024) != WSC_OK) return false;
     BlurLdsArgs ba;
     ba.nbr = L.nbr; ba.img_row = L.img_row; ba.blk = L.bl_blk; ba.val = val; ba.Mp = 4 * LP; ba.M = M; ba.rows = L.rows;
     ba.npass = L.d + 1;
+    ba.src = planes; ba.rss = nullptr;
     WscKernelTimer timer(ctx, WSC_K_BLUR, 2.0 * (L.d + 1) * L.rows * M * 4);
-    hipLaunchKernelGGL(blur_lds_kernel, dim3((unsigned)L.bl_nblk), dim3(BL_THREADS), L.bl_lds, st, ba);
-    return true;
+    hipLaunchKernelGGL(planes ? blur_lds_kernel<true> : blur_lds_kernel<false>, dim3((unsigned)L.bl_nblk), dim3(BL_THREADS),
+                       L.bl_lds, st, ba);
 }
 
 float *combine_blur_all4(wsc_ctx *ctx, hipStream_t st, const LatticeDev &L, int LP, const float *part, float *a, float *b) {
@@ -2391,8 +2589,13 @@
                            (const f32x4_t *)part, L.tile_pstart, L.n_slots);
         return b;
     }
+    if (blur_lds_ok(ctx, L)) {
+        float *planes = ctx->opt[WSC_OPT_CRF_LEAN] && L.row_plane && L.bl_nblk > 0 ? b : nullptr;
+        combine4(ctx, st, L, part, LP, a, planes);
+        blur_lds(ctx, st, L, LP, a, planes);
+        return a;
+    }
     combine4(ctx, st, L, part, LP, a);
-    if (blur_lds(ctx, st, L, LP, a)) return a;
     for (int j = 0; j <= L.d; ++j) {
         WscKernelTimer timer(ctx, WSC_K_BLUR, 2.0 * L.rows * L.rep * L.M_cur * 4);
         hipLaunchKernelGGL(blur4_kernel, dim3(grid_rep((long long)L.rows * L.rep, (256 / LP) * 4, L.rep)), dim3(256),
@@ -2504,6 +2707,7 @@
 int build_lattice(wsc_crf *crf, LatticeDev &L, CtxBlocks &own, const uint8_t *rgb_dev, float sxy, float srgb, bool shared,
                   bool full_table) {
     wsc_ctx *ctx = crf->ctx;
+    const bool lean = ctx->opt[WSC_OPT_CRF_LEAN] != 0;
     const int B = shared ? 1 : crf->B, N = crf->N, dp1 = D + 1;
     L.rep = shared ? crf->B : 1;
     const long long npix = (long long)B * N;
@@ -2529,7 +2733,8 @@
     WSC_TRY(tmp.alloc(sizeof(int32_t) * B * cap, &slot2row));
     const long long nw = (total + 31) / 32 + 1;
     WSC_TRY(tmp.alloc(sizeof(unsigned) * nw, &bitmap));
-    WSC_TRY(tmp.alloc(sizeof(unsigned) * nw, &wcount));
+    wcount = nullptr;
+    if (!lean) WSC_TRY(tmp.alloc(sizeof(unsigned) * nw, &wcount));
     WSC_TRY(tmp.alloc(sizeof(unsigned) * (nw + 1), &wprefix));
     WSC_TRY(tmp.alloc(sizeof(unsigned) * (size_t)(B + 1), &bound_dev));
     const int nblk = (int)((nw + SCAN_CHUNK - 1) / SCAN_CHUNK);
@@ -2545,9 +2750,10 @@
     WSC_TRY(own.alloc(sizeof(float) * total, &L.tent_w));
     WSC_TRY(own.alloc(sizeof(uint8_t) * total, &L.tent_p));
 
+    const long long nzblk = n_tiles0 + 1 + 4;
     hipLaunchKernelGGL(fill_tables_kernel, dim3(grid1d(B * cap)), dim3(256), 0, ctx->stream, table, (unsigned *)first,
-                       (long long)B * cap);
-    WSC_HIP(hipMemsetAsync(zblk, 0, sizeof(unsigned) * (size_t)(n_tiles0 + 1 + 4), ctx->stream));
+                       (long long)B * cap, lean ? bitmap : nullptr, nw, lean ? zblk : nullptr, nzblk);
+    if (!lean) WSC_HIP(hipMemsetAsync(zblk, 0, sizeof(unsigned) * (size_t)nzblk, ctx->stream));
 
     EmbedArgs ea;
     ea.rgb = rgb_dev; ea.B = B; ea.H = crf->H; ea.W = crf->W; ea.N = N;
@@ -2584,10 +2790,14 @@
     }
     const int per_img = N * dp1;
     const dim3 grid_tab((unsigned)grid1d(cap, 256, B >= 32 ? 256 : 8192 / (B > 0 ? B : 1)), (unsigned)B);
-    WSC_HIP(hipMemsetAsync(bitmap, 0, sizeof(unsigned) * nw, ctx->stream));
+    if (!lean) WSC_HIP(hipMemsetAsync(bitmap, 0, sizeof(unsigned) * nw, ctx->stream));
     hipLaunchKernelGGL(first_bits_kernel, grid_tab, dim3(256), 0, ctx->stream, first, cap, per_img, bitmap);
-    hipLaunchKernelGGL(popc_words_kernel, dim3(grid1d(nw)), dim3(256), 0, ctx->stream, bitmap, nw, wcount);
-    WSC_TRY(exclusive_scan(ctx, wcount, nw, wprefix, sums));
+    if (lean) {
+        WSC_TRY(exclusive_scan<true>(ctx, bitmap, nw, wprefix, sums));
+    } else {
+        hipLaunchKernelGGL(popc_words_kernel, dim3(grid1d(nw)), dim3(256), 0, ctx->stream, bitmap, nw, wcount);
+        WSC_TRY(exclusive_scan(ctx, wcount, nw, wprefix, sums));
+    }
     hipLaunchKernelGGL(image_bounds_kernel, dim3((unsigned)((B + 63) / 64)), dim3(64), 0, ctx->stream, bitmap, wprefix, per_img, B,
                        bound_dev);
     int herr = 0;
@@ -2628,21 +2838,23 @@
     WSC_TRY(tmp.alloc(sizeof(unsigned long long) * L.rows, &rowkey));
     WSC_TRY(tmp.alloc(sizeof(int32_t) * L.rows, &rowimg));
     WSC_TRY(own.alloc(sizeof(int2) * (size_t)dp1 * L.rows, &L.nbr));
-
+    if (lean && !shared && L.bl_ok) WSC_TRY(own.alloc(sizeof(int2) * (size_t)L.rows, &L.row_plane));
+
+    unsigned *row_nslots, *cursor;
+    WSC_TRY(tmp.alloc(sizeof(unsigned) * 2 * (size_t)(L.rows + 1), &row_nslots));
+    cursor = row_nslots + (L.rows + 1);
     hipLaunchKernelGGL(assign_rows_kernel, grid_tab, dim3(256), 0, ctx->stream, first, table, cap, per_img, bitmap, wprefix, slot2row,
-                       rowkey, rowimg);
+                       rowkey, rowimg, lean ? row_nslots : nullptr, 2ll * (L.rows + 1), (const int32_t *)L.img_row, L.row_plane);
     {
         int32_t *slot_row;
-        unsigned *sums2, *row_nslots, *cursor, *sums3;
+        unsigned *sums2, *sums3;
         const int nb2 = (L.n_tiles + 1 + SCAN_CHUNK - 1) / SCAN_CHUNK, nb3 = (L.rows + 1 + SCAN_CHUNK - 1) / SCAN_CHUNK;
         WSC_TRY(tmp.alloc(sizeof(unsigned) * (nb2 + 2), &sums2));
-        WSC_TRY(tmp.alloc(sizeof(unsigned) * 2 * (size_t)(L.rows + 1), &row_nslots));
-        cursor = row_nslots + (L.rows + 1);
         WSC_TRY(tmp.alloc(sizeof(unsigned) * (nb3 + 2), &sums3));
         WSC_TRY(own.alloc(sizeof(int32_t) * (L.n_tiles + 2), &L.tslot_start));
         WSC_TRY(own.alloc(sizeof(int32_t) * (L.rows + 2), &L.row_slot_start));
-        WSC_HIP(hipMemsetAsync(row_nslots, 0, sizeof(unsigned) * 2 * (size_t)(L.rows + 1), ctx->stream));
-        WSC_TRY(exclusive_scan(ctx, tile_nslots, L.n_tiles + 1, (unsigned *)L.tslot_start, sums2));
+        if (!lean) WSC_HIP(hipMemsetAsync(row_nslots, 0, sizeof(unsigned) * 2 * (size_t)(L.rows + 1), ctx->stream));
+        WSC_TRY(exclusive_scan(ctx, tile_nslots, L.n_tiles + 1, (unsigned *)L.tslot_start, sums2, lean));
         unsigned ns = 0;
         WSC_HIP(hipMemcpyAsync(&ns, sums2 + nb2, sizeof(unsigned), hipMemcpyDeviceToHost, ctx->stream));
         WSC_HIP(hipStreamSynchronize(ctx->stream));
@@ -2658,7 +2870,7 @@
         hipLaunchKernelGGL(tile_slots_kernel, dim3((unsigned)L.n_tiles), dim3(256), 0, ctx->stream, sslot, L.tent_p, L.offset, slot2row,
                            cap, dp1, tg,
                            L.tslot_start, L.slot_desc, slot_row, slot_key, row_nslots);
-        WSC_TRY(exclusive_scan(ctx, row_nslots, L.rows + 1, (unsigned *)L.row_slot_start, sums3));
+        WSC_TRY(exclusive_scan(ctx, row_nslots, L.rows + 1, (unsigned *)L.row_slot_start, sums3, lean));
         if (!shared) WSC_TRY(own.alloc(sizeof(uint32_t) * (size_t)(L.n_slots + 1), &L.part_row));
         hipLaunchKernelGGL(slot_dest_kernel, dim3(grid1d(L.n_slots)), dim3(256), 0, ctx->stream, slot_row, L.n_slots,
                            L.row_slot_start, cursor, L.slot_desc, L.part_row);
@@ -2717,8 +2929,11 @@
     WSC_TRY(tmp.alloc(sizeof(float) * L.rows, &va));
     WSC_TRY(tmp.alloc(sizeof(float) * L.rows, &vb));
     WSC_TRY(tmp.alloc(sizeof(float) * (size_t)(L.n_slots + 1), &vp));
-    splat_ones(ctx, L, make_geom(crf->H, crf->W), va, vp);
-    float *res = blur_all1(ctx, L, va, vb);
+    float *res = va;
+    if (!(lean && !shared && D == 5 && splat_blur_ones_lds(ctx, L, make_geom(crf->H, crf->W), va, vp))) {
+        splat_ones(ctx, L, make_geom(crf->H, crf->W), va, vp);
+        res = blur_all1(ctx, L, va, vb);
+    }
     uint32_t *rec_b = nullptr;
     if (D == 5 && !shared && crf->lat[0].gt_rows && !crf->pix_rec_b) WSC_TRY(own.alloc(sizeof(uint32_t) * 13 * (size_t)npix, &rec_b));
     if (!shared && D == 5) {
diff --git a/wsss-analysis_amd/wsscam/_lib.py b/wsss-analysis_amd/wsscam/_lib.py
--- a/wsss-analysis_amd/wsscam/_lib.py
+++ b/wsss-analysis_amd/wsscam/_lib.py
@@ -33,10 +33,10 @@
 PREC_F16X3 = 3
 PREC_F32 = 4
 OPT_CRF_GAUSS_ON_CHIP, OPT_CRF_FUSED_BLUR, OPT_CRF_BLUR_ON_CHIP, OPT_CRF_RANK_BALLOT, OPT_CRF_EMBED_FULL, OPT_RW_TILED, \
-    OPT_STEM_POOL_FUSED, OPT_CONV_WINDOW, OPT_CAM_HEAD_STREAM, OPT_CRF_MSG_IN_UPDATE = range(10)
+    OPT_STEM_POOL_FUSED, OPT_CONV_WINDOW, OPT_CAM_HEAD_STREAM, OPT_CRF_MSG_IN_UPDATE, OPT_CRF_LEAN = range(11)
 OPT_DEFAULTS = {OPT_CRF_GAUSS_ON_CHIP: 1, OPT_CRF_FUSED_BLUR: 1, OPT_CRF_BLUR_ON_CHIP: 1, OPT_CRF_RANK_BALLOT: 0,
                 OPT_CRF_EMBED_FULL: 0, OPT_RW_TILED: -1, OPT_STEM_POOL_FUSED: 1, OPT_CONV_WINDOW: 1, OPT_CAM_HEAD_STREAM: 1,
-                OPT_CRF_MSG_IN_UPDATE: 1}
+                OPT_CRF_MSG_IN_UPDATE: 1, OPT_CRF_LEAN: 1}
 CONV_GENERIC = 0x100
 
 
```

After: 2637 images/s. About the same (-0.3%).
